# salesforce/LayoutDETR

Hardware: AMD Instinct MI355X
Metric: images/sec G+D fwd-bwd, 256x256 bg x9 elems (higher is better)
Workload: dtype f32

## Files before the change

include/ldetr_hip.h:

```cpp
#ifndef LDETR_HIP_H
#define LDETR_HIP_H

#include <stdint.h>

#ifdef __cplusplus
extern "C" {
#endif

const char* ldetr_last_error(void);
int ldetr_abi_version(void);

int ldetr_debug_trace_tiles(int64_t* buffer);

int ldetr_set_split_bf16(int tiles);

int ldetr_engine_launch_counts(int64_t* f32_pipe, int64_t* bf16_split_pipe);

int ldetr_set_workspace(void* ptr, int64_t bytes);

typedef struct ldetr_tensor4 {
    int N, C, H, W;
    int64_t sn, sc, sh, sw;
} ldetr_tensor4;

typedef struct ldetr_epilogue {
    float alpha;
    const float* col_scale;
    const float* col_bias;
    const float* samp_scale;
    int64_t samp_ld;
    const float* residual;
    int64_t ldr;
    int act;
    float act_alpha;
    float act_gain;
    const float* mask_src;
    int64_t ldm;
    int mask_mode;
    float out_scale;
    float p_drop;
    uint64_t seed;
    const uint64_t* seed_ptr;
    int accumulate;
    float* a_rowsum;
} ldetr_epilogue;

int ldetr_bias_act_f32(const float* x, const float* b, const float* xref, const float* yref, const float* dy, float* y,
                       int64_t sizeX, int sizeB, int64_t stepB, int grad, int act, float alpha, float gain, float clamp,
                       void* stream);

int ldetr_upfirdn2d_f32(const float* x, const float* f, float* y, int N, int C, int inH, int inW,
                        const int64_t* x_strides_nchw, int fh, int fw, int64_t f_stride_h, int64_t f_stride_w,
                        int upx, int upy, int downx, int downy, int padx0, int padx1, int pady0, int pady1, int flip,
                        float gain, int outH, int outW, const int64_t* y_strides_nchw,
                        const float* act_bias, int has_act, float act_alpha, float act_gain, void* stream);

int ldetr_gemm_f32(const float* A, int64_t lda, int ta, const float* B, int64_t ldb, int tb, float* C, int64_t ldc,
                   int M, int N, int K, int splitk, const ldetr_epilogue* ep, int pix_per_sample, void* stream);

typedef struct ldetr_gemm_desc {
    const float* A; int64_t lda; int ta;
    const float* B; int64_t ldb; int tb;
    float* C; int64_t ldc;
    int M, N, K, splitk;
    const ldetr_epilogue* ep;
    int pix_per_sample;
} ldetr_gemm_desc;
int ldetr_gemm_pair_f32(const ldetr_gemm_desc* g0, const ldetr_gemm_desc* g1, void* stream);
int ldetr_gemm_pair_is_single_launch(const ldetr_gemm_desc* g0, const ldetr_gemm_desc* g1);

int ldetr_conv2d_fwd_f32(const float* x, const ldetr_tensor4* xt, const float* w, int Cout, int KH, int KW, int stride,
                         int pad, float* y, int64_t ldy, int OH, int OW, const float* in_scale, int64_t in_scale_ld,
                         const ldetr_epilogue* ep, void* stream);
int ldetr_conv2d_bwd_data_f32(const float* dy, const ldetr_tensor4* dyt, const float* w, int Cin, int KH, int KW,
                              int stride, int pad, float* dx, int64_t lddx, int IH, int IW, const float* dy_scale,
                              int64_t dy_scale_ld, const ldetr_epilogue* ep, void* stream);
int ldetr_conv2d_bwd_weight_f32(const float* x, const ldetr_tensor4* xt, const float* dy, const ldetr_tensor4* dyt,
                                float* dw, int KH, int KW, int stride, int pad, int splitk, const float* x_scale,
                                int64_t x_scale_ld, const float* dy_scale, int64_t dy_scale_ld, int accumulate, void* stream);

int ldetr_conv_transpose2d_fwd_f32(const float* x, const ldetr_tensor4* xt, const float* w, int Cout, int KH, int KW,
                                   int stride, int pad, float* y, int64_t ldy, int OH, int OW, const float* in_scale,
                                   int64_t in_scale_ld, const ldetr_epilogue* ep, void* stream);
int ldetr_conv_transpose2d_bwd_data_f32(const float* dy, const ldetr_tensor4* dyt, const float* w, int Cin, int KH,
                                        int KW, int stride, int pad, float* dx, int64_t lddx, int IH, int IW,
                                        const float* dy_scale, int64_t dy_scale_ld, const ldetr_epilogue* ep,
                                        void* stream);
int ldetr_conv_transpose2d_bwd_weight_f32(const float* x, const ldetr_tensor4* xt, const float* dy,
                                          const ldetr_tensor4* dyt, float* dw, int KH, int KW, int stride, int pad,
                                          int splitk, const float* x_scale, int64_t x_scale_ld, const float* dy_scale,
                                          int64_t dy_scale_ld, int accumulate, void* stream);

int ldetr_attention_fwd_f32(const float* q, int64_t ldq, const float* k, int64_t ldk, const float* v, int64_t ldv,
                            const unsigned char* key_padding_mask, float* out, int64_t ldo, float* lse, int B, int H,
                            int Lq, int Lk, int head_dim, float scale, float p_drop, uint64_t seed, const uint64_t* seed_ptr,
                            int causal, void* stream);
int ldetr_attention_bwd_f32(const float* q, int64_t ldq, const float* k, int64_t ldk, const float* v, int64_t ldv,
                            const unsigned char* key_padding_mask, const float* out, int64_t ldo, const float* lse,
                            const float* dout, int64_t lddo, float* dq, int64_t lddq, float* dk, int64_t lddk,
                            float* dv, int64_t lddv, int B, int H, int Lq, int Lk, int head_dim, float scale,
                            float p_drop, uint64_t seed, const uint64_t* seed_ptr, int causal, void* stream);

int ldetr_torgb_bwd_finish_f32(const float* dws, const float* s, const float* w, int B, int C, float* dw, float* ds, void* stream);

int ldetr_loss_combine_fwd_f32(const float* const* x, const float* w, const int* n, const int* fn, const int* red, int K, int ld,
                               float* vals, float* sums, float* total, void* stream);
int ldetr_loss_combine_bwd_f32(const float* const* x, const float* w, const int* n, const int* fn, const int* red, int K, int ld,
                               const float* g, float* grads, void* stream);
int ldetr_masked_mse_fwd_f32(const float* a, const float* b, const uint8_t* valid, int64_t rows, int D, int bdiv, float* out2, void* stream);
int ldetr_masked_mse_bwd_f32(const float* a, const float* b, const uint8_t* valid, int64_t rows, int D, int bdiv, const float* out2,
                             const float* g, float* da, void* stream);

typedef struct ldetr_ln_args {
    const float* x; const float* r; const float* gamma; const float* beta;
    float* y; float* z; float* mean; float* rstd;
    const float* dy; float* dx; float* dr; float* dgamma; float* dbeta;
    int64_t rows; int D; float eps, p_drop; uint64_t seed; const uint64_t* seed_ptr;
    const float* pos; int64_t pos_rows; float* ypos; const float* dy2;
    int r_parts; int64_t r_part_stride; const float* r_bias;
    const float* dy_parts; int dy_nparts; int64_t dy_part_stride;
} ldetr_ln_args;
int ldetr_layernorm_fwd_group_f32(const ldetr_ln_args* a, int n, void* stream);
int ldetr_layernorm_bwd_group_f32(const ldetr_ln_args* a, int n, void* stream);
int ldetr_sum_parts_f32(const float* base, const float* parts, int n_parts, int64_t part_stride, float* out, int64_t n, void* stream);

typedef struct ldetr_ffn_args {
    const float* x; int64_t ldx;
    const float* w1; const float* b1;
    const float* w2;
    float* h;
    float* ypart;
    int M, F;
    float p_drop; uint64_t seed; const uint64_t* seed_ptr;
    const float* dy;
    float* dxpart;
    float* dh;
} ldetr_ffn_args;
int ldetr_ffn_fwd_group_f32(const ldetr_ffn_args* a, int n, void* stream);
int ldetr_ffn_bwd_group_f32(const ldetr_ffn_args* a, int n, void* stream);

typedef struct ldetr_mha_small_args {
    const float* x; int64_t ldx;
    const float* w_in; const float* b_in; const float* w_out;
    const unsigned char* kpm;
    float* qkv; float* o; float* lse; float* ypart;
    int B, L;
    float scale, p_drop; uint64_t seed; const uint64_t* seed_ptr;
    const float* dr;
    float* dqkv; float* dxpart;
} ldetr_mha_small_args;
int ldetr_mha_small_fwd_group_f32(const ldetr_mha_small_args* a, int n, void* stream);
int ldetr_mha_small_bwd_group_f32(const ldetr_mha_small_args* a, int n, void* stream);

typedef struct ldetr_mha_cross_args {
    const float* x; int64_t ldx;
    const float* w_q; const float* b_q;
    const float* k; int64_t ldk; const float* v; int64_t ldv;
    const float* w_out;
    const unsigned char* kpm;
    float* q; float* o; float* lse; float* ypart;
    int B, Lq, Lk;
    float scale, p_drop; uint64_t seed; const uint64_t* seed_ptr;
    const float* dr;
    float* dq; float* dk; int64_t lddk; float* dv; int64_t lddv; float* dxpart;
} ldetr_mha_cross_args;
int ldetr_mha_cross_fwd_f32(const ldetr_mha_cross_args* a, void* stream);
int ldetr_mha_cross_bwd_f32(const ldetr_mha_cross_args* a, void* stream);

typedef struct ldetr_wgrad_desc {
    const float* A; int64_t lda; const float* B; int64_t ldb;
    float* dW; int64_t ldw; float* db;
    int M, rows, cols;
} ldetr_wgrad_desc;
int ldetr_wgrad_multi_f32(const ldetr_wgrad_desc* d, int n, void* stream);

int ldetr_colsum_f32(const float* a, float* red, int B, int64_t P, int C, void* stream);
int ldetr_act_bwd_reduce_f32(const float* dy, const float* y, float* dv, const float* bias, const float* demod,
                             float* dbias, float* ddemod, int B, int64_t P, int C, int act, float alpha, float gain,
                             void* stream);
int ldetr_mul_reduce_f32(const float* a, const float* x, const float* scale, float* out, float* red, int B, int64_t P,
                         int C, void* stream);
int ldetr_torgb_fwd_f32(const float* x, const float* w, const float* styles, const float* bias, float* y,
                        int B, int64_t P, int C, void* stream);
int ldetr_torgb_bwd_f32(const float* x, const float* dy, const float* w, const float* styles, float* dx, float* dws,
                        float* dbias, int B, int64_t P, int C, void* stream);
int ldetr_sg2_handoff_f32(const float* dxs, const float* x, const float* dy_rgb, float* dv, const float* s_conv, const float* s_rgb,
                          const float* w_rgb, const float* bias, const float* demod, float* ds_conv, float* dws_rgb, float* dbias_rgb,
                          float* dbias, float* ddemod, int B, int64_t P, int C, float alpha, float gain, void* stream);

int ldetr_maxpool3x3s2_fwd_f32(const float* x, float* y, unsigned char* idx, int N, int H, int W, int C, void* stream);
int ldetr_maxpool3x3s2_bwd_f32(const float* dy, const unsigned char* idx, float* dx, int N, int H, int W, int C,
                               void* stream);

int ldetr_grad_sanitize_f32(float* g, int64_t n, float scale, float nan_value, float posinf, float neginf,
                            void* stream);
int ldetr_adam_step_f32(float* p, const float* g, float* m, float* v, int64_t n, int64_t step, float lr, float beta1,
                        float beta2, float eps, int fuse_sanitize, float gscale, float nan_value, float posinf,
                        float neginf, void* stream);
int ldetr_adam_ema_step_f32(float* p, const float* g, float* m, float* v, int64_t n, int64_t step, float lr, float beta1, float beta2,
                            float eps, int fuse_sanitize, float gscale, float nan_value, float posinf, float neginf,
                            float* p_ema, float ema_beta, void* stream);
int ldetr_ema_lerp_f32(float* p_ema, const float* p, int64_t n, float beta, void* stream);

int ldetr_softmax_xent_fwd_f32(const float* logits, int64_t ld, const int64_t* targets, float* row_lse, float* loss_sum, float* count,
                               int64_t rows, int V, int64_t ignore_index, float label_smoothing, void* stream);
int ldetr_softmax_xent_bwd_f32(const float* logits, int64_t ld, const int64_t* targets, const float* row_lse, const float* count,
                               const float* grad_out, float* dlogits, int64_t ldd, int64_t rows, int V, int64_t ignore_index,
                               float label_smoothing, void* stream);

int ldetr_embedding_fwd_f32(const float* weight, const float* pos, const int64_t* ids, float* out, int64_t n, int d, int V, int T,
                            void* stream);
int ldetr_embedding_bwd_f32(const float* dy, const int64_t* ids, float* dweight, int64_t n, int d, int V, int64_t padding_idx,
                            void* stream);

int ldetr_resample_coeffs(int in_size, int out_size, int32_t* bounds, int32_t* weights, int64_t weights_capacity, int* ksize_out);
int ldetr_resize_normalize_u8(const uint8_t* src, int64_t images, int H, int W, int out_h, int out_w, const int32_t* hbounds,
                              const int32_t* hweights, int hksize, const int32_t* vbounds, const int32_t* vweights, int vksize,
                              uint8_t* tmp, uint8_t* out_u8, float* out_chw, float mean0, float mean1, float mean2, float std0,
                              float std1, float std2, void* stream);

#define LDETR_PAGE_FILTER_BLUR 1
#define LDETR_PAGE_FILTER_EDGE 2
int ldetr_page_filter_u8(const uint8_t* src, uint8_t* dst, int64_t images, int H, int W, int kind, float radius, void* stream);

int ldetr_demod_fwd_f32(const float* weight, int64_t so, int64_t si, int64_t sh, int64_t sw, const float* styles, float* dcoefs,
                        float* w2, int B, int O, int I, int KH, int KW, float eps, void* stream);
int ldetr_demod_bwd_f32(const float* weight, int64_t so, int64_t si, int64_t sh, int64_t sw, const float* styles, const float* dcoefs,
                        const float* w2, const float* grad_dcoefs, float* dweight, int accumulate_dweight, float* dstyles, int B, int O,
                        int I, int KH, int KW, void* stream);

int ldetr_layout_losses_f32(const float* bbox, const float* bbox_ref, const uint8_t* valid, int B, int N, float* losses,
                            float* grads, void* stream);
int ldetr_layout_losses_bwd_f32(const float* grads, const float* grad_losses, int B, int N, float* dbbox, void* stream);

int ldetr_layout_finish_f32(const float* bbox_in, const int* num, const float* factors, const unsigned char* jitter, const unsigned char* mode,
                            float* bbox_out, float* overlap, float* alignment, int* order, int C, int K, int N, void* stream);

#define LDETR_FILTER_BILINEAR 0
#define LDETR_FILTER_LANCZOS 1
typedef struct ldetr_layout_raster_args {
    int struct_bytes;
    int B, N, S, nrow, n_colors, n_pages;
    const float* bbox;
    const uint8_t* valid;
    const int32_t* labels;
    const uint8_t* palette;
    const int32_t* page_wh;
    const uint8_t* pages;
    int64_t pages_bytes;
    const int64_t* page_table;
    const int32_t* page_index;
    const int32_t* coeffs;
    int64_t coeffs_len;
    const int64_t* cell_coeffs;
    int32_t* cells_dev;
    uint8_t* out;
} ldetr_layout_raster_args;
int ldetr_resample_coeffs_filter(int filter, int in_size, int out_size, int32_t* bounds, int32_t* weights, int64_t weights_capacity, int* ksize_out);
int ldetr_layout_raster_cell_size(int W, int H, int S, int* wn_out, int* hn_out);
int ldetr_layout_raster_u8(const ldetr_layout_raster_args* a, void* stream);

typedef struct ldetr_patch_resize_args {
    int struct_bytes;
    int n_jobs;
    const uint8_t* src0;
    int64_t src0_bytes;
    const uint8_t* src1;
    int64_t src1_bytes;
    uint8_t* dst;
    int64_t dst_bytes;
    const int64_t* jobs;
    const int32_t* tables;
    const int32_t* tables_host;
    int64_t tables_len;
    int32_t* jobs_dev;
} ldetr_patch_resize_args;
typedef struct ldetr_image_raster_args {
    int struct_bytes;
    int B, N, S, nrow;
    const float* bbox;
    const uint8_t* valid;
    const int32_t* rects;
    const int64_t* patch_off;
    const int64_t* page_off;
    const int32_t* page_wh;
    const uint8_t* pixels;
    int64_t pixels_bytes;
    const int32_t* coeffs;
    int64_t coeffs_len;
    const int64_t* cell_coeffs;
    int32_t* cells_dev;
    uint8_t* out;
} ldetr_image_raster_args;
int ldetr_patch_resize_u8(const ldetr_patch_resize_args* a, void* stream);
int ldetr_image_raster_u8(const ldetr_image_raster_args* a, void* stream);

#define LDETR_PNG_NOT_ELIGIBLE 3
#define LDETR_PNG_MALFORMED 4
typedef struct ldetr_png_decode_args {
    int struct_bytes;
    int n, H, W;
    int phases;
    int reserved;
    const uint8_t* files;
    int64_t files_bytes;
    const int64_t* file_off;
    const int64_t* file_off_dev;
    const int64_t* segments;
    const int64_t* segments_dev;
    int64_t n_segments;
    const int32_t* jobs;
    const int32_t* jobs_dev;
    int64_t n_jobs;
    uint8_t* scratch;
    int64_t scratch_bytes;
    uint8_t* dst;
} ldetr_png_decode_args;
int ldetr_png_scan(const uint8_t* file, int64_t file_bytes, int* width, int* height, int* channels, int64_t* segments, int64_t segments_capacity,
                   int64_t* segments_count, int32_t* row_starts, int64_t row_starts_capacity, int64_t* row_starts_count);
int ldetr_png_decode_u8(const ldetr_png_decode_args* a, void* stream);

typedef struct ldetr_png_encode_args {
    int struct_bytes;
    int H, W;
    int blocks;
    int filter;
    int reserved;
    const uint8_t* src;
    uint8_t* out;
    int64_t out_capacity;
    int64_t* total_bytes;
    uint8_t* workspace;
    int64_t workspace_bytes;
    int64_t* seg_table;
    int64_t seg_table_rows;
} ldetr_png_encode_args;
int ldetr_png_encode_bound(int H, int W, int64_t* out_bytes, int64_t* workspace_bytes);
int ldetr_png_encode_u8(const ldetr_png_encode_args* a, void* stream);
int ldetr_png_index_bytes(int H, int W, int64_t* bytes);

#define LDETR_PNG_INFLATE_CODE 1
#define LDETR_PNG_INFLATE_COUNT 2
#define LDETR_PNG_INFLATE_HEADER 4
#define LDETR_PNG_INFLATE_DISTANCE 8
#define LDETR_PNG_INFLATE_TRAILER 16
#define LDETR_PNG_INFLATE_FILTER 32
#define LDETR_PNG_INFLATE_STUCK 64
#define LDETR_PNG_INFLATE_TABLE 128
typedef struct ldetr_png_inflate_args {
    int struct_bytes;
    int n, H, W;
    int phases;
    int reserved;
    const uint8_t* files;
    int64_t files_bytes;
    const int64_t* file_off;
    const int64_t* file_off_dev;
    const int64_t* segments;
    const int64_t* segments_dev;
    const int64_t* index_off;
    const int64_t* index_off_dev;
    const int32_t* jobs;
    const int32_t* jobs_dev;
    int64_t n_jobs;
    uint8_t* scratch;
    int64_t scratch_bytes;
    uint8_t* dst;
    int32_t* status;
} ldetr_png_inflate_args;
int ldetr_png_scan_packed(const uint8_t* file, int64_t file_bytes, int* width, int* height, int64_t* segments, int64_t segments_capacity, int64_t* segments_count,
                          int64_t* index_offset, int32_t* row_starts, int64_t row_starts_capacity, int64_t* row_starts_count);
int ldetr_png_inflate_u8(const ldetr_png_inflate_args* a, void* stream);

int ldetr_lsap_f64(const double* cost, int batch, int n, int maximize, int* row_ind, int* col_ind, void* stream);

int ldetr_layoutnet_features_f32(const float* bbox, const int64_t* label, const uint8_t* padding_mask, const int* label_map, int map_len,
                                 const float* weights, int64_t weights_len, int num_label, int B, int N, float* out, void* stream);

int ldetr_layoutnet_forward_f32(const float* bbox, const int64_t* label, const uint8_t* padding_mask, const float* enc_weights,
                                int64_t enc_len, const float* dec_weights, int64_t dec_len, int num_label, int B, int N,
                                float* logit_disc, float* logit_cls, float* bbox_pred, float* features, void* stream);

// ... 48 lines not shown
```

layoutdetr_amd/_lib.py:

```python
import ctypes
import os
from ctypes import (POINTER, Structure, c_char_p, c_double, c_float, c_int, c_int64, c_ubyte, c_uint64, c_void_p)

_HERE = os.path.dirname(os.path.abspath(__file__))
ABI_VERSION = 25
LIB_PATH = os.environ.get('LDETR_LIB') or os.path.join(_HERE, 'lib', 'libldetr_hip.so')


class Tensor4(Structure):
    _fields_ = [('N', c_int), ('C', c_int), ('H', c_int), ('W', c_int),
                ('sn', c_int64), ('sc', c_int64), ('sh', c_int64), ('sw', c_int64)]


class GemmDesc(Structure):
    _fields_ = [('A', c_void_p), ('lda', c_int64), ('ta', c_int), ('B', c_void_p), ('ldb', c_int64), ('tb', c_int),
                ('C', c_void_p), ('ldc', c_int64), ('M', c_int), ('N', c_int), ('K', c_int), ('splitk', c_int),
                ('ep', c_void_p), ('pix_per_sample', c_int)]


class P3Epilogue(Structure):
    _fields_ = [('alpha', c_float), ('col_scale', c_void_p), ('col_bias', c_void_p), ('residual_p3', c_void_p),
                ('residual_f32', c_void_p), ('relu_mask_p3', c_void_p), ('relu', c_int)]


class Epilogue(Structure):
    _fields_ = [('alpha', c_float), ('col_scale', c_void_p), ('col_bias', c_void_p), ('samp_scale', c_void_p),
                ('samp_ld', c_int64), ('residual', c_void_p), ('ldr', c_int64), ('act', c_int),
                ('act_alpha', c_float), ('act_gain', c_float), ('mask_src', c_void_p), ('ldm', c_int64),
                ('mask_mode', c_int), ('out_scale', c_float), ('p_drop', c_float), ('seed', c_uint64),
                ('seed_ptr', c_void_p), ('accumulate', c_int), ('a_rowsum', c_void_p)]


class LnArgs(Structure):
    _fields_ = [('x', c_void_p), ('r', c_void_p), ('gamma', c_void_p), ('beta', c_void_p),
                ('y', c_void_p), ('z', c_void_p), ('mean', c_void_p), ('rstd', c_void_p),
                ('dy', c_void_p), ('dx', c_void_p), ('dr', c_void_p), ('dgamma', c_void_p), ('dbeta', c_void_p),
                ('rows', c_int64), ('D', c_int), ('eps', c_float), ('p_drop', c_float), ('seed', c_uint64), ('seed_ptr', c_void_p),
                ('pos', c_void_p), ('pos_rows', c_int64), ('ypos', c_void_p), ('dy2', c_void_p),
                ('r_parts', c_int), ('r_part_stride', c_int64), ('r_bias', c_void_p),
                ('dy_parts', c_void_p), ('dy_nparts', c_int), ('dy_part_stride', c_int64)]


class FfnArgs(Structure):
    _fields_ = [('x', c_void_p), ('ldx', c_int64), ('w1', c_void_p), ('b1', c_void_p), ('w2', c_void_p), ('h', c_void_p), ('ypart', c_void_p),
                ('M', c_int), ('F', c_int), ('p_drop', c_float), ('seed', c_uint64), ('seed_ptr', c_void_p),
                ('dy', c_void_p), ('dxpart', c_void_p), ('dh', c_void_p)]


class MhaSmallArgs(Structure):
    _fields_ = [('x', c_void_p), ('ldx', c_int64), ('w_in', c_void_p), ('b_in', c_void_p), ('w_out', c_void_p), ('kpm', c_void_p),
                ('qkv', c_void_p), ('o', c_void_p), ('lse', c_void_p), ('ypart', c_void_p), ('B', c_int), ('L', c_int),
                ('scale', c_float), ('p_drop', c_float), ('seed', c_uint64), ('seed_ptr', c_void_p),
                ('dr', c_void_p), ('dqkv', c_void_p), ('dxpart', c_void_p)]


class MhaCrossArgs(Structure):
    _fields_ = [('x', c_void_p), ('ldx', c_int64), ('w_q', c_void_p), ('b_q', c_void_p), ('k', c_void_p), ('ldk', c_int64), ('v', c_void_p), ('ldv', c_int64),
                ('w_out', c_void_p), ('kpm', c_void_p), ('q', c_void_p), ('o', c_void_p), ('lse', c_void_p), ('ypart', c_void_p),
                ('B', c_int), ('Lq', c_int), ('Lk', c_int), ('scale', c_float), ('p_drop', c_float), ('seed', c_uint64), ('seed_ptr', c_void_p),
                ('dr', c_void_p), ('dq', c_void_p), ('dk', c_void_p), ('lddk', c_int64), ('dv', c_void_p), ('lddv', c_int64), ('dxpart', c_void_p)]


class WgradDesc(Structure):
    _fields_ = [('A', c_void_p), ('lda', c_int64), ('B', c_void_p), ('ldb', c_int64), ('dW', c_void_p), ('ldw', c_int64), ('db', c_void_p),
                ('M', c_int), ('rows', c_int), ('cols', c_int)]


class LayoutRasterArgs(Structure):
    _fields_ = [('struct_bytes', c_int), ('B', c_int), ('N', c_int), ('S', c_int), ('nrow', c_int), ('n_colors', c_int), ('n_pages', c_int),
                ('bbox', c_void_p), ('valid', c_void_p), ('labels', c_void_p), ('palette', c_void_p), ('page_wh', c_void_p),
                ('pages', c_void_p), ('pages_bytes', c_int64), ('page_table', c_void_p), ('page_index', c_void_p),
                ('coeffs', c_void_p), ('coeffs_len', c_int64), ('cell_coeffs', c_void_p), ('cells_dev', c_void_p), ('out', c_void_p)]


class PatchResizeArgs(Structure):
    _fields_ = [('struct_bytes', c_int), ('n_jobs', c_int), ('src0', c_void_p), ('src0_bytes', c_int64), ('src1', c_void_p), ('src1_bytes', c_int64),
                ('dst', c_void_p), ('dst_bytes', c_int64), ('jobs', c_void_p), ('tables', c_void_p), ('tables_host', c_void_p), ('tables_len', c_int64),
                ('jobs_dev', c_void_p)]


class ImageRasterArgs(Structure):
    _fields_ = [('struct_bytes', c_int), ('B', c_int), ('N', c_int), ('S', c_int), ('nrow', c_int),
                ('bbox', c_void_p), ('valid', c_void_p), ('rects', c_void_p), ('patch_off', c_void_p), ('page_off', c_void_p), ('page_wh', c_void_p),
                ('pixels', c_void_p), ('pixels_bytes', c_int64), ('coeffs', c_void_p), ('coeffs_len', c_int64), ('cell_coeffs', c_void_p),
                ('cells_dev', c_void_p), ('out', c_void_p)]


class PngDecodeArgs(Structure):
    _fields_ = [('struct_bytes', c_int), ('n', c_int), ('H', c_int), ('W', c_int), ('phases', c_int), ('reserved', c_int),
                ('files', c_void_p), ('files_bytes', c_int64), ('file_off', c_void_p), ('file_off_dev', c_void_p),
                ('segments', c_void_p), ('segments_dev', c_void_p), ('n_segments', c_int64),
                ('jobs', c_void_p), ('jobs_dev', c_void_p), ('n_jobs', c_int64),
                ('scratch', c_void_p), ('scratch_bytes', c_int64), ('dst', c_void_p)]


class PngEncodeArgs(Structure):
    _fields_ = [('struct_bytes', c_int), ('H', c_int), ('W', c_int), ('blocks', c_int), ('filter', c_int), ('reserved', c_int),
                ('src', c_void_p), ('out', c_void_p), ('out_capacity', c_int64), ('total_bytes', c_void_p),
                ('workspace', c_void_p), ('workspace_bytes', c_int64), ('seg_table', c_void_p), ('seg_table_rows', c_int64)]


class PngInflateArgs(Structure):
    _fields_ = [('struct_bytes', c_int), ('n', c_int), ('H', c_int), ('W', c_int), ('phases', c_int), ('reserved', c_int),
                ('files', c_void_p), ('files_bytes', c_int64), ('file_off', c_void_p), ('file_off_dev', c_void_p),
                ('segments', c_void_p), ('segments_dev', c_void_p), ('index_off', c_void_p), ('index_off_dev', c_void_p),
                ('jobs', c_void_p), ('jobs_dev', c_void_p), ('n_jobs', c_int64),
                ('scratch', c_void_p), ('scratch_bytes', c_int64), ('dst', c_void_p), ('status', c_void_p)]


_P = c_void_p
_I = c_int
_L = c_int64
_F = c_float
_T4 = POINTER(Tensor4)
_EP = POINTER(Epilogue)

SIGNATURES = {
    'ldetr_set_workspace': [_P, _L],
    'ldetr_bias_act_f32': [_P, _P, _P, _P, _P, _P, _L, _I, _L, _I, _I, _F, _F, _F, _P],
    'ldetr_upfirdn2d_f32': [_P, _P, _P, _I, _I, _I, _I, POINTER(c_int64), _I, _I, _L, _L, _I, _I, _I, _I, _I, _I, _I, _I,
                            _I, _F, _I, _I, POINTER(c_int64), _P, _I, _F, _F, _P],
    'ldetr_gemm_f32': [_P, _L, _I, _P, _L, _I, _P, _L, _I, _I, _I, _I, _EP, _I, _P],
    'ldetr_conv2d_fwd_f32': [_P, _T4, _P, _I, _I, _I, _I, _I, _P, _L, _I, _I, _P, _L, _EP, _P],
    'ldetr_conv2d_bwd_data_f32': [_P, _T4, _P, _I, _I, _I, _I, _I, _P, _L, _I, _I, _P, _L, _EP, _P],
    'ldetr_conv2d_bwd_weight_f32': [_P, _T4, _P, _T4, _P, _I, _I, _I, _I, _I, _P, _L, _P, _L, _I, _P],
    'ldetr_conv_transpose2d_fwd_f32': [_P, _T4, _P, _I, _I, _I, _I, _I, _P, _L, _I, _I, _P, _L, _EP, _P],
    'ldetr_conv_transpose2d_bwd_data_f32': [_P, _T4, _P, _I, _I, _I, _I, _I, _P, _L, _I, _I, _P, _L, _EP, _P],
    'ldetr_conv_transpose2d_bwd_weight_f32': [_P, _T4, _P, _T4, _P, _I, _I, _I, _I, _I, _P, _L, _P, _L, _I, _P],
    'ldetr_attention_fwd_f32': [_P, _L, _P, _L, _P, _L, _P, _P, _L, _P, _I, _I, _I, _I, _I, _F, _F, c_uint64, _P, _I, _P],
    'ldetr_attention_bwd_f32': [_P, _L, _P, _L, _P, _L, _P, _P, _L, _P, _P, _L, _P, _L, _P, _L, _P, _L,
                                _I, _I, _I, _I, _I, _F, _F, c_uint64, _P, _I, _P],
    'ldetr_colsum_f32': [_P, _P, _I, _L, _I, _P],
    'ldetr_act_bwd_reduce_f32': [_P, _P, _P, _P, _P, _P, _P, _I, _L, _I, _I, _F, _F, _P],
    'ldetr_mul_reduce_f32': [_P, _P, _P, _P, _P, _I, _L, _I, _P],
    'ldetr_torgb_fwd_f32': [_P, _P, _P, _P, _P, _I, _L, _I, _P],
    'ldetr_torgb_bwd_f32': [_P, _P, _P, _P, _P, _P, _P, _I, _L, _I, _P],
    'ldetr_maxpool3x3s2_fwd_f32': [_P, _P, _P, _I, _I, _I, _I, _P],
    'ldetr_maxpool3x3s2_bwd_f32': [_P, _P, _P, _I, _I, _I, _I, _P],
    'ldetr_grad_sanitize_f32': [_P, _L, _F, _F, _F, _F, _P],
    'ldetr_adam_step_f32': [_P, _P, _P, _P, _L, _L, _F, _F, _F, _F, _I, _F, _F, _F, _F, _P],
    'ldetr_adam_ema_step_f32': [_P, _P, _P, _P, _L, _L, _F, _F, _F, _F, _I, _F, _F, _F, _F, _P, _F, _P],
    'ldetr_ema_lerp_f32': [_P, _P, _L, _F, _P],
    'ldetr_lsap_f64': [_P, _I, _I, _I, _P, _P, _P],
    'ldetr_layoutnet_features_f32': [_P, _P, _P, POINTER(c_int), _I, _P, _L, _I, _I, _I, _P, _P],
    'ldetr_layoutnet_forward_f32': [_P, _P, _P, _P, _L, _P, _L, _I, _I, _I, _P, _P, _P, _P, _P],
    'ldetr_feature_stats_f64': [_P, _L, _I, _P, _P, _P],
    'ldetr_box_giou_pairwise_f32': [_P, _P, _I, _I, _I, _I, _P, _P, _P, _P, c_double, _P],
    'ldetr_bmm_strided_f32': [_P, _P, _P, _P, _P, _P, _I, _I, _I, _I, _I, _F, _P],
    'ldetr_softmax_xent_fwd_f32': [_P, _L, _P, _P, _P, _P, _L, _I, _L, _F, _P],
    'ldetr_softmax_xent_bwd_f32': [_P, _L, _P, _P, _P, _P, _P, _L, _L, _I, _L, _F, _P],
    'ldetr_embedding_fwd_f32': [_P, _P, _P, _P, _L, _I, _I, _I, _P],
    'ldetr_embedding_bwd_f32': [_P, _P, _P, _L, _I, _I, _L, _P],
    'ldetr_debug_trace_tiles': [_P],
    'ldetr_set_split_bf16': [c_int],
    'ldetr_engine_launch_counts': [POINTER(c_int64), POINTER(c_int64)],
    'ldetr_layernorm_fwd_group_f32': [_P, _I, _P],
    'ldetr_layernorm_bwd_group_f32': [_P, _I, _P],
    'ldetr_sum_parts_f32': [_P, _P, _I, _L, _P, _L, _P],
    'ldetr_ffn_fwd_group_f32': [_P, _I, _P],
    'ldetr_ffn_bwd_group_f32': [_P, _I, _P],
    'ldetr_mha_small_fwd_group_f32': [_P, _I, _P],
    'ldetr_mha_small_bwd_group_f32': [_P, _I, _P],
    'ldetr_mha_cross_fwd_f32': [_P, _P],
    'ldetr_mha_cross_bwd_f32': [_P, _P],
    'ldetr_wgrad_multi_f32': [_P, _I, _P],
    'ldetr_loss_combine_fwd_f32': [_P, _P, _P, _P, _P, _I, _I, _P, _P, _P, _P],
    'ldetr_loss_combine_bwd_f32': [_P, _P, _P, _P, _P, _I, _I, _P, _P, _P],
    'ldetr_masked_mse_fwd_f32': [_P, _P, _P, _L, _I, _I, _P, _P],
    'ldetr_masked_mse_bwd_f32': [_P, _P, _P, _L, _I, _I, _P, _P, _P, _P],
    'ldetr_torgb_bwd_finish_f32': [_P, _P, _P, _I, _I, _P, _P, _P],
    'ldetr_sg2_handoff_f32': [_P, _P, _P, _P, _P, _P, _P, _P, _P, _P, _P, _P, _P, _P, _I, _L, _I, _F, _F, _P],
    'ldetr_gemm_pair_f32': [_P, _P, _P],
    'ldetr_gemm_pair_is_single_launch': [_P, _P],
    'ldetr_demod_fwd_f32': [_P, _L, _L, _L, _L, _P, _P, _P, _I, _I, _I, _I, _I, _F, _P],
    'ldetr_demod_bwd_f32': [_P, _L, _L, _L, _L, _P, _P, _P, _P, _P, _I, _P, _I, _I, _I, _I, _I, _P],
    'ldetr_layout_losses_f32': [_P, _P, _P, _I, _I, _P, _P, _P],
    'ldetr_layout_losses_bwd_f32': [_P, _P, _I, _I, _P, _P],
    'ldetr_layout_finish_f32': [_P, _P, _P, _P, _P, _P, _P, _P, _P, _I, _I, _I, _P],
    'ldetr_resample_coeffs': [_I, _I, _P, _P, _L, _P],
    'ldetr_resample_coeffs_filter': [_I, _I, _I, _P, _P, _L, _P],
    'ldetr_layout_raster_cell_size': [_I, _I, _I, _P, _P],
    'ldetr_layout_raster_u8': [_P, _P],
    'ldetr_patch_resize_u8': [_P, _P],
    'ldetr_image_raster_u8': [_P, _P],
    'ldetr_p3_split_f32': [_P, _L, _P, _L, _I, _P],
    'ldetr_p3_merge_f32': [_P, _P, _L, _L, _I, _P],
    'ldetr_p3_weight_bwd': [_P, _P, _P, _I, _I, _I, _I, _P],
    'ldetr_p3_conv2d_bwd_data': [_P, _I, _I, _I, _I, _P, _I, _I, _I, _I, _I, _I, _I, _P, _P, _P, _P],
    'ldetr_p3_conv2d_fwd': [_P, _I, _I, _I, _I, _P, _I, _I, _I, _I, _I, _P, _P, _P, _P],
    'ldetr_p3_conv2d_bwd_weight': [_P, _I, _I, _I, _I, _P, _I, _I, _I, _I, _I, _P, _P, _P],
    'ldetr_p3_weight_prep': [_P, _I, _I, _P],
    'ldetr_p3_conv2d_fwd_dual': [_P, _P, _I, _I, _I, _I, _P, _P, _I, _I, _I, _I, _I, _P, _P, _P, _P, _P, _P, _P],
    'ldetr_p3_conv2d_bwd_pair': [_P, _I, _I, _I, _I, _P, _P, _I, _I, _I, _I, _I, _I, _I, _P, _P, _P, _P, _P, _P, _P],
    'ldetr_p3_last_launch': [_P],
    'ldetr_engine_last_launch': [_P],
    'ldetr_struct_sizes': [_P],
    'ldetr_resize_normalize_u8': [_P, _L, _I, _I, _I, _I, _P, _P, _I, _P, _P, _I, _P, _P, _P, _F, _F, _F, _F, _F, _F, _P],
    'ldetr_page_filter_u8': [_P, _P, _L, _I, _I, _I, _F, _P],
    'ldetr_png_scan': [_P, _L, _P, _P, _P, _P, _L, _P, _P, _L, _P],
    'ldetr_png_decode_u8': [_P, _P],
    'ldetr_png_encode_bound': [_I, _I, _P, _P],
    'ldetr_png_encode_u8': [_P, _P],
    'ldetr_png_index_bytes': [_I, _I, _P],
    'ldetr_png_scan_packed': [_P, _L, _P, _P, _P, _L, _P, _P, _P, _L, _P],
    'ldetr_png_inflate_u8': [_P, _P],
}

_lib = None


def load():
    global _lib
    if _lib is not None:
        return _lib
    if not os.path.exists(LIB_PATH):
        raise RuntimeError(
            f'{LIB_PATH} not found: build the gfx950 kernels first (python -m layoutdetr_amd.build or '
            f'__graft_entry__.build()).  layoutdetr_amd has no CPU/PyTorch fallback path.')
    import torch
    lib = ctypes.CDLL(LIB_PATH)
    lib.ldetr_last_error.restype = c_char_p
    lib.ldetr_last_error.argtypes = []
    lib.ldetr_abi_version.restype = c_int
    lib.ldetr_abi_version.argtypes = []
    for name, argtypes in SIGNATURES.items():
        fn = getattr(lib, name)
        fn.restype = c_int
        fn.argtypes = argtypes
    if lib.ldetr_abi_version() != ABI_VERSION:
        raise RuntimeError('libldetr_hip.so ABI version mismatch; rebuild it')
    sizes = (ctypes.c_int32 * 6)()
    lib.ldetr_struct_sizes(sizes)
    mirror = [ctypes.sizeof(t) for t in (LnArgs, FfnArgs, MhaSmallArgs, MhaCrossArgs, WgradDesc, P3Epilogue)]
    if list(sizes) != mirror:
        raise RuntimeError(f'libldetr_hip.so argument blocks {list(sizes)} do not match the ctypes mirror {mirror}; rebuild')
    _lib = lib
    return lib


def check(rc, what=''):
    if rc != 0:
        msg = load().ldetr_last_error().decode('utf-8', 'replace')
        raise RuntimeError(f'{what}: {msg}' if what else msg)
```

layoutdetr_amd/build.py:

```python
import hashlib
import os
import shutil
import subprocess
import sys
from concurrent.futures import ThreadPoolExecutor

HERE = os.path.dirname(os.path.abspath(__file__))
CSRC = os.path.join(HERE, 'csrc')
LIBDIR = os.path.join(HERE, 'lib')
OBJDIR = os.path.join(LIBDIR, 'obj')
LIBNAME = 'libldetr_hip.so'
ARCH = 'gfx950'

SOURCES = ['ldetr_core.cpp', 'bias_act.hip', 'upfirdn2d.hip', 'gemm_conv.hip', 'attention.hip', 'layernorm.hip',
           'misc_ops.hip', 'optim.hip', 'lsap.hip', 'xent.hip', 'resample.hip', 'layout_loss.hip', 'demod.hip', 'wgrad_smallc.hip', 'stem_conv.hip', 'box_ops.hip', 'ffn_fused.hip', 'conv_c32.hip', 'mha_small.hip', 'p3_engine.hip', 'bmm_strided.hip', 'layoutnet.hip', 'layoutnet_train.hip', 'layout_finish.hip', 'layout_raster.hip', 'page_filter.hip', 'patch_resize.hip', 'png_decode.hip', 'png_encode.hip', 'png_inflate.hip']
HEADERS = ['ldetr_common.hpp', 'layoutnet_layers.hpp', 'pil_resample.hpp', 'png_pages.hpp', 'png_inflate_kernel.hpp', os.path.join('..', '..', 'include', 'ldetr_hip.h')]

FLAGS = ([] if os.environ.get('LDETR_TILE_TRACE') else ['-DLDETR_TILE_TRACE=0']) + (['-DP3_TRACE'] if os.environ.get('LDETR_P3_TRACE') else []) + ['-O3', '-std=c++17', '-fPIC', f'--offload-arch={ARCH}', '-munsafe-fp-atomics', '-fno-gpu-rdc',
         '-Wno-unused-result', '-Rpass-analysis=kernel-resource-usage']
NO_SCRATCH = ('wgrad_c32_3x3_kernel', 'gemm_f32_kernel', 'gemm_small_kernel', 'attn_fwd_kernel', 'attn_fwd_wide_kernel', 'attn_bwd_kernel', 'ffn_fwd_kernel', 'ffn_bwd_kernel', 'conv3x3_c32_kernel', 'mha_small_fwd_kernel', 'mha_cross_fwd_kernel', 'mha_small_bwd_kernel', 'mha_cross_bwd_kernel', 'wgrad_multi_kernel', 'ln_fwd_kernel', 'ln_bwd_kernel', 'p3_nt_kernel', 'p3_tn_kernel', 'p3_c3_kernel', 'p3_bwd_pair', 'layoutnet_features_kernel', 'layoutnet_forward_kernel', 'feature_stats_f64_kernel', 'layout_finish_kernel', 'layout_raster_kernel', 'page_blur_kernel', 'page_edge_kernel', 'patch_resize_kernel', 'sg2_handoff_kernel', 'png_gather_kernel', 'png_unfilter_kernel', 'png_enc_filter_kernel', 'png_enc_deflate_kernel', 'png_enc_assemble_kernel', 'png_inflate_kernel')


def _hipcc():
    for cand in (os.environ.get('HIPCC'), shutil.which('hipcc'), '/opt/rocm/bin/hipcc'):
        if cand and os.path.exists(cand):
            return cand
    raise RuntimeError('hipcc not found: the gfx950 kernel library cannot be built')


def _digest(paths):
    h = hashlib.sha256()
    for p in paths:
        with open(p, 'rb') as f:
            h.update(f.read())
    h.update(' '.join(FLAGS).encode())
    return h.hexdigest()


def _kernel_resources(remarks):
    out, cur = {}, None
    for line in remarks.splitlines():
        if 'remark:' not in line:
            continue
        body = line.split('remark:', 1)[1].split('[-Rpass-analysis', 1)[0].strip()
        if body.startswith('Function Name:'):
            cur = body.split(':', 1)[1].strip()
            out[cur] = {}
        elif cur is not None and ':' in body:
            k, v = body.rsplit(':', 1)
            out[cur][k.strip()] = v.strip()
    return out


def source_digest():
    return _digest(sorted(os.path.join(CSRC, f) for f in os.listdir(CSRC) if f.endswith(('.hip', '.cpp', '.hpp')) and not f.startswith('.'))
                   + [os.path.normpath(os.path.join(CSRC, HEADERS[-1]))])


def lib_path():
    return os.path.join(LIBDIR, LIBNAME)


def build(force=False, verbose=True):
    os.makedirs(OBJDIR, exist_ok=True)
    hipcc = _hipcc()
    hdrs = [os.path.normpath(os.path.join(CSRC, h)) for h in HEADERS]
    objs, jobs = [], []
    for src in SOURCES:
        sp = os.path.join(CSRC, src)
        obj = os.path.join(OBJDIR, src + '.o')
        stamp = obj + '.sha'
        dig = _digest([sp] + hdrs)
        objs.append(obj)
        if not force and os.path.exists(obj) and os.path.exists(stamp) and open(stamp).read() == dig:
            continue
        jobs.append((sp, obj, stamp, dig))

    def compile_one(job):
        sp, obj, stamp, dig = job
        cmd = [hipcc] + FLAGS + ['-x', 'hip', '-c', sp, '-o', obj]
        if verbose:
            print('[ldetr build]', os.path.basename(sp), flush=True)
        r = subprocess.run(cmd, capture_output=True, text=True)
        if r.returncode != 0:
            raise RuntimeError(f'hipcc failed for {sp}:\n{r.stdout}\n{r.stderr}')
        res = _kernel_resources(r.stderr)
        with open(obj + '.resources.txt', 'w') as f:
            for name, d in res.items():
                f.write(f"{name} vgprs={d.get('VGPRs', '?')} agprs={d.get('AGPRs', '?')} scratch={d.get('ScratchSize [bytes/lane]', '?')} "
                        f"occupancy={d.get('Occupancy [waves/SIMD]', '?')} lds={d.get('LDS Size [bytes/block]', '?')}\n")
        bad = [n for n, d in res.items() if any(k in n for k in NO_SCRATCH) and d.get('ScratchSize [bytes/lane]', '0') != '0']
        if bad:
            raise RuntimeError(f'{os.path.basename(sp)}: scratch memory in register-budgeted kernels: ' + ', '.join(bad[:4]))
        with open(stamp, 'w') as f:
            f.write(dig)

    if jobs:
        with ThreadPoolExecutor(max_workers=min(8, len(jobs))) as ex:
            list(ex.map(compile_one, jobs))
    out = lib_path()
    if jobs or not os.path.exists(out):
        cmd = [hipcc, '-shared', '-fPIC', f'--offload-arch={ARCH}', '-fno-gpu-rdc', '-o', out] + objs
        r = subprocess.run(cmd, capture_output=True, text=True)
        if r.returncode != 0:
            raise RuntimeError(f'link failed:\n{r.stdout}\n{r.stderr}')
        if verbose:
            print('[ldetr build] linked', out, flush=True)
    return out


if __name__ == '__main__':
    build(force='--force' in sys.argv)
```

layoutdetr_amd/csrc/demod.hip:

```cpp
#include "ldetr_common.hpp"
#include "../../include/ldetr_hip.h"

namespace ldetr {

struct DemodParams {
    const float* w; long so, si, sh, sw;
    const float* s;
    float* d;
    float* w2;
    const float* g;
    float* dw; int dw_accumulate;
    float* ds;
    int B, O, I, KH, KW;
    float eps;
};

constexpr int DEMOD_MAXB = 64;

__global__ __launch_bounds__(256) void demod_fwd_kernel(DemodParams p) {
    extern __shared__ float w2row[];
    const int o = blockIdx.x;
    for (int i = threadIdx.x; i < p.I; i += 256) {
        const float* wp = p.w + (long)o * p.so + (long)i * p.si;
        float acc = 0.f;
        for (int kh = 0; kh < p.KH; kh++)
            for (int kw = 0; kw < p.KW; kw++) { const float v = wp[kh * p.sh + kw * p.sw]; acc += v * v; }
        w2row[i] = acc;
        p.w2[(long)o * p.I + i] = acc;
    }
    __syncthreads();
    __shared__ float red16[4][16];
    for (int b0 = 0; b0 < p.B; b0 += 16) {
        float part[16];
#pragma unroll
        for (int u = 0; u < 16; u++) part[u] = 0.f;
        for (int i = threadIdx.x; i < p.I; i += 256) {
            const float wv = w2row[i];
#pragma unroll
            for (int u = 0; u < 16; u++)
                if (b0 + u < p.B) { const float sv = p.s[(long)(b0 + u) * p.I + i]; part[u] += sv * sv * wv; }
        }
#pragma unroll
        for (int u = 0; u < 16; u++) part[u] = wave_sum(part[u]);
        __syncthreads();
        if ((threadIdx.x & 63) == 0) {
#pragma unroll
            for (int u = 0; u < 16; u++) red16[threadIdx.x >> 6][u] = part[u];
        }
        __syncthreads();
        if (threadIdx.x < 16 && b0 + threadIdx.x < p.B) {
            const float tot = red16[0][threadIdx.x] + red16[1][threadIdx.x] + red16[2][threadIdx.x] + red16[3][threadIdx.x];
            p.d[(long)(b0 + threadIdx.x) * p.O + o] = rsqrtf(tot + p.eps);
        }
    }
}

__global__ __launch_bounds__(256) void demod_bwd_w_kernel(DemodParams p) {
    __shared__ float t[DEMOD_MAXB];
    const int o = blockIdx.x;
    if (threadIdx.x < p.B) {
        const float dv = p.d[(long)threadIdx.x * p.O + o];
        t[threadIdx.x] = -0.5f * p.g[(long)threadIdx.x * p.O + o] * dv * dv * dv;
    }
    __syncthreads();
    for (int i = threadIdx.x; i < p.I; i += 256) {
        float dw2 = 0.f;
        for (int b = 0; b < p.B; b++) { const float sv = p.s[(long)b * p.I + i]; dw2 += t[b] * sv * sv; }
        dw2 *= 2.f;
        const long base = (long)o * p.so + (long)i * p.si;
        for (int kh = 0; kh < p.KH; kh++)
            for (int kw = 0; kw < p.KW; kw++) {
                const long off = base + kh * p.sh + kw * p.sw;
                const float v = p.w[off] * dw2;
                if (p.dw_accumulate) p.dw[off] += v; else p.dw[off] = v;
            }
    }
}

__global__ __launch_bounds__(256) void demod_bwd_s_kernel(DemodParams p) {
    extern __shared__ float tb[];
    const int b = blockIdx.y, i = blockIdx.x * 64 + (threadIdx.x & 63), lane = threadIdx.x >> 6;
    for (int o = threadIdx.x; o < p.O; o += 256) {
        const float dv = p.d[(long)b * p.O + o];
        tb[o] = -0.5f * p.g[(long)b * p.O + o] * dv * dv * dv;
    }
    __syncthreads();
    float acc = 0.f;
    if (i < p.I) {
#pragma unroll 8
        for (int o = lane; o < p.O; o += 4) acc += tb[o] * p.w2[(long)o * p.I + i];
    }
    float* part = tb + p.O;
    part[threadIdx.x] = acc;
    __syncthreads();
    if (lane == 0 && i < p.I) {
        acc += part[threadIdx.x + 64] + part[threadIdx.x + 128] + part[threadIdx.x + 192];
        p.ds[(long)b * p.I + i] = 2.f * p.s[(long)b * p.I + i] * acc;
    }
}

}

using namespace ldetr;

static int demod_check(const DemodParams& p, const char* what) {
    LDETR_CHECK(p.w && p.s && p.d && p.w2, "%s: null pointer", what);
    LDETR_CHECK(p.B > 0 && p.B <= DEMOD_MAXB && p.O > 0 && p.I > 0 && p.KH > 0 && p.KW > 0, "%s: bad shape (batch <= %d)", what, DEMOD_MAXB);
    LDETR_CHECK((size_t)(p.I > p.O ? p.I : p.O) * sizeof(float) <= 48 * 1024, "%s: more than 12288 channels", what);
    return LDETR_OK;
}

extern "C" int ldetr_demod_fwd_f32(const float* weight, int64_t so, int64_t si, int64_t sh, int64_t sw, const float* styles, float* dcoefs,
                                   float* w2, int B, int O, int I, int KH, int KW, float eps, void* stream) {
    DemodParams p; memset(&p, 0, sizeof(p));
    p.w = weight; p.so = so; p.si = si; p.sh = sh; p.sw = sw; p.s = styles; p.d = dcoefs; p.w2 = w2;
    p.B = B; p.O = O; p.I = I; p.KH = KH; p.KW = KW; p.eps = eps;
    int rc = demod_check(p, "demod_fwd"); if (rc) return rc;
    hipLaunchKernelGGL(demod_fwd_kernel, dim3(O), 256, (size_t)I * sizeof(float), (hipStream_t)stream, p);
    return check_launch("demod_fwd");
}

extern "C" int ldetr_demod_bwd_f32(const float* weight, int64_t so, int64_t si, int64_t sh, int64_t sw, const float* styles, const float* dcoefs,
                                   const float* w2, const float* grad_dcoefs, float* dweight, int accumulate_dweight, float* dstyles, int B,
                                   int O, int I, int KH, int KW, void* stream) {
    DemodParams p; memset(&p, 0, sizeof(p));
    p.w = weight; p.so = so; p.si = si; p.sh = sh; p.sw = sw; p.s = styles; p.d = const_cast<float*>(dcoefs); p.w2 = const_cast<float*>(w2);
    p.g = grad_dcoefs; p.dw = dweight; p.dw_accumulate = accumulate_dweight; p.ds = dstyles;
    p.B = B; p.O = O; p.I = I; p.KH = KH; p.KW = KW;
    int rc = demod_check(p, "demod_bwd"); if (rc) return rc;
    LDETR_CHECK(grad_dcoefs && (dweight || dstyles), "demod_bwd: null pointer");
    hipStream_t st = (hipStream_t)stream;
    if (dweight) {
        hipLaunchKernelGGL(demod_bwd_w_kernel, dim3(O), 256, 0, st, p);
        rc = check_launch("demod_bwd_w"); if (rc) return rc;
    }
    if (dstyles) {
        hipLaunchKernelGGL(demod_bwd_s_kernel, dim3(cdiv(I, 64), B), 256, (size_t)(O + 256) * sizeof(float), st, p);
        rc = check_launch("demod_bwd_s");
    }
    return rc;
}
```

layoutdetr_amd/csrc/gemm_conv.hip:

```cpp
#include <cstdlib>
#include <type_traits>
#include <atomic>
#include "ldetr_common.hpp"
#include "../../include/ldetr_hip.h"

namespace ldetr {
static thread_local int64_t t_launches_f32 = 0, t_launches_split = 0;
void count_engine_launch(bool bf16_split_pipe) { (bf16_split_pipe ? t_launches_split : t_launches_f32)++; }

enum {
    OP_KC_DENSE = 0,
    OP_KC_CONV = 1,
    OP_KC_CONVT = 2,
    OP_KC_WTAP = 3,
    OP_RC_DENSE = 4,
    OP_RC_PIX = 5,
    OP_RC_WT = 6,
    OP_RC_CONVK = 7,
};

struct Operand {
    const float* p;
    long ld;
    int vec;
// ... 892 lines not shown
        if (!s_last) { trace_out(); return; }
#pragma unroll
        for (int i = 0; i < TM; i++)
#pragma unroll
            for (int j = 0; j < TN; j++)
#pragma unroll
                for (int r = 0; r < 16; r++) acc[i][j][r] = 0.f;
        for (int sl = 0; sl < p.splitk; sl++) {
            const float* src = slot0 + (long)sl * (BM * BN);
#pragma unroll
            for (int i = 0; i < TM; i++)
#pragma unroll
                for (int j = 0; j < TN; j++)
#pragma unroll
                    for (int r = 0; r < 16; r++)
                        acc[i][j][r] += __hip_atomic_load(src + ((i * TN + j) * 16 + r) * NT + tid, __ATOMIC_RELAXED, __HIP_MEMORY_SCOPE_AGENT);
        }
        direct = true;
    }

    const GemmEpilogue& ep = p.ep;
    const float inv_keep = ep.p_drop > 0.f ? 1.f / (1.f - ep.p_drop) : 1.f;
    if (direct && p.ep_vec) {
        constexpr int CP = BN + 4;
        constexpr int LDSF = 2 * BKT * (LDA + LDB);
        constexpr int PASSES = (BM * CP + LDSF - 1) / LDSF, RP = BM / PASSES;
        static_assert(BM % PASSES == 0 && RP * CP <= LDSF && (RP % 32) == 0, "epilogue staging does not fit");
        static_assert(!SPLIT || RP * CP * 4 <= 3 * (BKT / 8) * (PLA + PLB), "epilogue staging does not fit the split path's LDS image");
        float* Cs = ldetr_smem;
#pragma unroll
        for (int ps = 0; ps < PASSES; ps++) {
            if (ps > 0) __syncthreads();
#pragma unroll
            for (int i = 0; i < TM; i++) {
                const int rb = wm * WM + i * 32 - ps * RP;
                if (rb < 0 || rb >= RP) continue;
#pragma unroll
                for (int j = 0; j < TN; j++)
#pragma unroll
                    for (int r = 0; r < 16; r++)
                        Cs[(rb + (r & 3) + 8 * (r >> 2) + 4 * kl) * CP + wn * WN + j * 32 + cl] = acc[i][j][r];
            }
            __syncthreads();
            for (int u = tid; u < RP * (BN / 4); u += NT) {
                const int rl = u / (BN / 4), c4 = (u - rl * (BN / 4)) * 4;
                const int m = m0 + ps * RP + rl, n = n0 + c4;
                if (m >= z.M || n >= p.N) continue;
                long orow = m;
                if (p.zmode == 1 && p.pstep > 1) {
                    int per = z.DH2 * z.DW2;
                    int nn = m / per; int rem = m - nn * per;
                    int y2 = rem / z.DW2; int x2 = rem - y2 * z.DW2;
                    orow = ((long)nn * p.A.DH + (y2 * p.pstep + z.py)) * p.A.DW + (x2 * p.pstep + z.px);
                }
                const int samp = (ep.samp_scale && p.pix_per_sample > 0) ? (int)((unsigned)orow / (unsigned)p.pix_per_sample) : 0;
                const float4 a4 = *reinterpret_cast<const float4*>(Cs + rl * CP + c4);
                float4 cs4 = make_float4(1.f, 1.f, 1.f, 1.f), cb4 = make_float4(0.f, 0.f, 0.f, 0.f), rs4 = make_float4(0.f, 0.f, 0.f, 0.f);
                if (ep.col_scale) cs4 = *reinterpret_cast<const float4*>(ep.col_scale + n);
                if (ep.col_bias) cb4 = *reinterpret_cast<const float4*>(ep.col_bias + n);
                if (ep.residual) rs4 = *reinterpret_cast<const float4*>(ep.residual + orow * ep.ldr + n);
                float4 mk4 = make_float4(0.f, 0.f, 0.f, 0.f);
                if (ep.mask_mode) mk4 = *reinterpret_cast<const float4*>(ep.mask_src + orow * ep.ldm + n);
                float* dst = p.C + z.c_off + orow * p.ldc + n;
                float4 o;
                o.x = apply_epilogue(ep, a4.x, orow, n + 0, samp, p.ldc, inv_keep, cs4.x, cb4.x, rs4.x, mk4.x);
                o.y = apply_epilogue(ep, a4.y, orow, n + 1, samp, p.ldc, inv_keep, cs4.y, cb4.y, rs4.y, mk4.y);
                o.z = apply_epilogue(ep, a4.z, orow, n + 2, samp, p.ldc, inv_keep, cs4.z, cb4.z, rs4.z, mk4.z);
                o.w = apply_epilogue(ep, a4.w, orow, n + 3, samp, p.ldc, inv_keep, cs4.w, cb4.w, rs4.w, mk4.w);
                if (ep.accumulate) { const float4 c = *reinterpret_cast<const float4*>(dst); o.x += c.x; o.y += c.y; o.z += c.z; o.w += c.w; }
                *reinterpret_cast<float4*>(dst) = o;
            }
        }
        trace_out(); return;
    }
    float cs[TN], cb[TN], sfc[TN];
#pragma unroll
    for (int j = 0; j < TN; j++) {
        int n = n0 + wn * WN + j * 32 + cl;
        cs[j] = (ep.col_scale && n < p.N) ? ep.col_scale[n] : 1.f;
        cb[j] = (ep.col_bias && n < p.N) ? ep.col_bias[n] : 0.f;
        sfc[j] = (p.scol && n < p.N) ? p.scol[(long)z.samp * p.scol_ld + n] : 1.f;
    }
#pragma unroll
    for (int i = 0; i < TM; i++) {
#pragma unroll
        for (int r = 0; r < 16; r++) {
            int m = m0 + wm * WM + i * 32 + (r & 3) + 8 * (r >> 2) + 4 * kl;
            if (m >= z.M) continue;
            long orow = m;
            if (p.zmode == 1 && p.pstep > 1) {
                int per = z.DH2 * z.DW2;
                int n = m / per; int rem = m - n * per;
                int y2 = rem / z.DW2; int x2 = rem - y2 * z.DW2;
                orow = ((long)n * p.A.DH + (y2 * p.pstep + z.py)) * p.A.DW + (x2 * p.pstep + z.px);
            }
            int samp = (ep.samp_scale && p.pix_per_sample > 0) ? (int)((unsigned)orow / (unsigned)p.pix_per_sample) : 0;
            const float sfr = p.srow ? p.srow[(long)z.samp * p.srow_ld + m] : 1.f;
#pragma unroll
            for (int j = 0; j < TN; j++) {
                int n = n0 + wn * WN + j * 32 + cl;
                if (n >= p.N) continue;
                float* dst = p.C + z.c_off + orow * p.ldc + n;
                const float a = acc[i][j][r] * sfr * sfc[j];
                if (!direct) {
                    atomicAdd(dst, a * (ep.row_scale ? ep.alpha * ep.row_scale[orow] : ep.alpha));
                } else {
                    float v = apply_epilogue(ep, a, orow, n, samp, p.ldc, inv_keep, cs[j], cb[j], ep.residual ? ep.residual[orow * ep.ldr + n] : 0.f,
                                           ep.mask_mode ? ep.mask_src[orow * ep.ldm + n] : 0.f);
                    if (ep.accumulate) *dst += v; else *dst = v;
                }
            }
        }
    }
    trace_out();
}

template <int T>
__device__ __forceinline__ void small_load(const Operand& o, int row, int R, int k0, int kl, int kend, float (&f)[16]) {
    const int kb = k0 + 16 * kl;
    if (T == 0) {
        const float* src = o.p + (long)row * o.ld + kb;
        if (row < R && o.vec) {
#pragma unroll
            for (int j = 0; j < 4; j++) {
                float4 v = make_float4(0.f, 0.f, 0.f, 0.f);
                if (kb + 4 * j < kend) v = *reinterpret_cast<const float4*>(src + 4 * j);
                f[4 * j] = v.x; f[4 * j + 1] = v.y; f[4 * j + 2] = v.z; f[4 * j + 3] = v.w;
            }
        } else {
#pragma unroll
            for (int t = 0; t < 16; t++) f[t] = (row < R && kb + t < kend) ? src[t] : 0.f;
        }
    } else {
        const float* src = o.p + (long)kb * o.ld + row;
#pragma unroll
        for (int t = 0; t < 16; t++) f[t] = (row < R && kb + t < kend) ? src[(long)t * o.ld] : 0.f;
    }
}

template <int T>
__device__ __forceinline__ void small_load_fast(const __amdgpu_buffer_rsrc_t& rs, int voff, int k0, int ld, float (&f)[16]) {
    if (T == 0) {
#pragma unroll
        for (int j = 0; j < 4; j++) {
            const auto v = __builtin_amdgcn_raw_buffer_load_b128(rs, voff + 16 * j, k0 * 4, 0);
            f[4 * j] = __int_as_float(v[0]); f[4 * j + 1] = __int_as_float(v[1]); f[4 * j + 2] = __int_as_float(v[2]); f[4 * j + 3] = __int_as_float(v[3]);
        }
    } else {
#pragma unroll
        for (int t = 0; t < 16; t++) f[t] = __int_as_float(__builtin_amdgcn_raw_buffer_load_b32(rs, voff, (k0 + t) * ld * 4, 0));
    }
}

template <int TA, int TB, int NW, bool FAST = false>
__device__ __forceinline__ void gemm_small_body(const GemmParams& p, const int bx, const int by, const int bz, const int sk, const int gx) {
    using f32x16 = __attribute__((__vector_size__(16 * sizeof(float)))) float;
    __shared__ float red[NW][32][33];
    const int tid = threadIdx.x, lane = tid & 63, wave = tid >> 6;
    const int cl = lane & 31, kl = lane >> 5;
    const int m0 = by * 32, n0 = bx * 32;
    const int chunks_all = (p.K + 31) / 32;
    const int cper = (chunks_all + sk - 1) / sk;
    const int kblk0 = bz * cper * 32, kblk1 = min(p.K, kblk0 + cper * 32);
    const int chunks = kblk1 > kblk0 ? (kblk1 - kblk0 + 31) / 32 : 0, per = (chunks + NW - 1) / NW;
    const int kbeg = kblk0 + wave * per * 32, kend = min(kblk1, kbeg + per * 32);
    __amdgpu_buffer_rsrc_t rsA = __builtin_amdgcn_make_buffer_rsrc(const_cast<float*>(p.A.p), 0, FAST ? 0x7fffffff : 0, 0x00020000);
    __amdgpu_buffer_rsrc_t rsB = __builtin_amdgcn_make_buffer_rsrc(const_cast<float*>(p.B.p), 0, FAST ? 0x7fffffff : 0, 0x00020000);
    const int voffA = (m0 + cl < p.M) ? (TA == 0 ? ((m0 + cl) * (int)p.A.ld + 16 * kl) * 4 : (16 * kl * (int)p.A.ld + m0 + cl) * 4) : (int)0x80000000;
    const int voffB = (n0 + cl < p.N) ? (TB == 0 ? ((n0 + cl) * (int)p.B.ld + 16 * kl) * 4 : (16 * kl * (int)p.B.ld + n0 + cl) * 4) : (int)0x80000000;
    auto loadA = [&](int k0, float (&f)[16]) {
        if constexpr (FAST) small_load_fast<TA>(rsA, voffA, k0, (int)p.A.ld, f); else small_load<TA>(p.A, m0 + cl, p.M, k0, kl, kend, f);
        if constexpr (TA == 0) {
            if (p.A.scale) {
                const int kb = k0 + 16 * kl;
#pragma unroll
                for (int j = 0; j < 4; j++) {
                    if (kb + 4 * j < kend) {
                        const float4 s4 = *reinterpret_cast<const float4*>(p.A.scale + kb + 4 * j);
                        f[4 * j] *= s4.x; f[4 * j + 1] *= s4.y; f[4 * j + 2] *= s4.z; f[4 * j + 3] *= s4.w;
                    }
                }
            }
        }
    };
    auto loadB = [&](int k0, float (&f)[16]) {
        if constexpr (FAST) small_load_fast<TB>(rsB, voffB, k0, (int)p.B.ld, f); else small_load<TB>(p.B, n0 + cl, p.N, k0, kl, kend, f);
    };
    f32x16 acc;
#pragma unroll
    for (int r = 0; r < 16; r++) acc[r] = 0.f;
    float a0[16], b0[16], a1[16], b1[16];
    const bool want_rs = TA == 1 && p.ep.a_rowsum != nullptr && bx == 0;
    float rs = 0.f;
    if (kbeg < kend) {
        loadA(kbeg, a0);
        loadB(kbeg, b0);
    }
    for (int k = kbeg; k < kend; k += 64) {
        if (k + 32 < kend) {
            loadA(k + 32, a1);
            loadB(k + 32, b1);
        }
#pragma unroll
        for (int t = 0; t < 16; t++) acc = __builtin_amdgcn_mfma_f32_32x32x2f32(a0[t], b0[t], acc, 0, 0, 0);
        if (want_rs) {
#pragma unroll
            for (int t = 0; t < 16; t++) rs += a0[t];
        }
        if (k + 32 >= kend) break;
        if (k + 64 < kend) {
            loadA(k + 64, a0);
            loadB(k + 64, b0);
        }
#pragma unroll
        for (int t = 0; t < 16; t++) acc = __builtin_amdgcn_mfma_f32_32x32x2f32(a1[t], b1[t], acc, 0, 0, 0);
        if (want_rs) {
#pragma unroll
            for (int t = 0; t < 16; t++) rs += a1[t];
        }
    }
    __shared__ float rsum[NW][32];
    if (want_rs) {
        rs += __shfl_xor(rs, 32);
        if (kl == 0) rsum[wave][cl] = rs;
    }
#pragma unroll
    for (int r = 0; r < 16; r++) red[wave][(r & 3) + 8 * (r >> 2) + 4 * kl][cl] = acc[r];
    __syncthreads();
    if (want_rs && tid < 32 && m0 + tid < p.M) {
        float tot = 0.f;
#pragma unroll
        for (int w = 0; w < NW; w++) tot += rsum[w][tid];
        if (sk > 1) atomicAdd(p.ep.a_rowsum + m0 + tid, tot);
        else p.ep.a_rowsum[m0 + tid] += tot;
    }
    const GemmEpilogue& ep = p.ep;
    const float inv_keep = ep.p_drop > 0.f ? 1.f / (1.f - ep.p_drop) : 1.f;
    float* slot0 = nullptr;
    if (sk > 1) {
        const long tile = (long)by * gx + bx;
        slot0 = p.ws + tile * sk * 1024;
        float* mine = slot0 + (long)bz * 1024;
        for (int q = tid; q < 256; q += NW * 64) {
            const int row = q >> 3, c4 = (q & 7) * 4;
#pragma unroll
            for (int e = 0; e < 4; e++) {
                float sum = 0.f;
#pragma unroll
                for (int w = 0; w < NW; w++) sum += red[w][row][c4 + e];
                __hip_atomic_store(mine + q * 4 + e, sum, __ATOMIC_RELAXED, __HIP_MEMORY_SCOPE_AGENT);
            }
        }
        asm volatile("s_waitcnt vmcnt(0)" ::: "memory");
        __shared__ int s_last_small;
        __syncthreads();
        if (tid == 0) {
            const int old = atomicAdd(p.ws_count + tile, 1);
            s_last_small = (old == sk - 1);
            if (s_last_small) __hip_atomic_store(p.ws_count + tile, 0, __ATOMIC_RELAXED, __HIP_MEMORY_SCOPE_AGENT);
        }
        __syncthreads();
        if (!s_last_small) return;
    }
    for (int q = tid; q < 256; q += NW * 64) {
        const int row = q >> 3, c4 = (q & 7) * 4;
        const int m = m0 + row;
        if (m >= p.M) continue;
        float v[4];
        if (sk > 1) {
#pragma unroll
            for (int e = 0; e < 4; e++) v[e] = 0.f;
            float part[8][4];
#pragma unroll
            for (int z = 0; z < 8; z++)
#pragma unroll
                for (int e = 0; e < 4; e++)
                    part[z][e] = z < sk ? __hip_atomic_load(slot0 + (long)z * 1024 + q * 4 + e, __ATOMIC_RELAXED, __HIP_MEMORY_SCOPE_AGENT) : 0.f;
#pragma unroll
            for (int z = 0; z < 8; z++)
#pragma unroll
                for (int e = 0; e < 4; e++) v[e] += part[z][e];
        } else {
#pragma unroll
            for (int e = 0; e < 4; e++) {
                float sum = 0.f;
#pragma unroll
                for (int w = 0; w < NW; w++) sum += red[w][row][c4 + e];
                v[e] = sum;
            }
        }
        const int samp = (ep.samp_scale && p.pix_per_sample > 0) ? m / p.pix_per_sample : 0;
        float* dst = p.C + (long)m * p.ldc + n0 + c4;
#pragma unroll
        for (int e = 0; e < 4; e++)
            if (n0 + c4 + e < p.N) v[e] = apply_epilogue(ep, v[e], m, n0 + c4 + e, samp, p.ldc, inv_keep, ep.col_scale ? ep.col_scale[n0 + c4 + e] : 1.f, ep.col_bias ? ep.col_bias[n0 + c4 + e] : 0.f,
                                                             ep.residual ? ep.residual[(long)m * ep.ldr + n0 + c4 + e] : 0.f,
                                                             ep.mask_mode ? ep.mask_src[(long)m * ep.ldm + n0 + c4 + e] : 0.f);
        if (n0 + c4 + 3 < p.N && (p.ldc & 3) == 0 && ((((uintptr_t)p.C) & 15) == 0)) {
            float4 o = make_float4(v[0], v[1], v[2], v[3]);
            if (ep.accumulate) { float4 c = *reinterpret_cast<float4*>(dst); o.x += c.x; o.y += c.y; o.z += c.z; o.w += c.w; }
            *reinterpret_cast<float4*>(dst) = o;
        } else {
#pragma unroll
            for (int e = 0; e < 4; e++)
                if (n0 + c4 + e < p.N) { if (ep.accumulate) dst[e] += v[e]; else dst[e] = v[e]; }
        }
    }
}

template <int TA, int TB, int NW, bool FAST = false>
__global__ __launch_bounds__(NW * 64) void gemm_small_kernel(GemmParams p) {
    gemm_small_body<TA, TB, NW, FAST>(p, blockIdx.x, blockIdx.y, blockIdx.z, gridDim.z, gridDim.x);
}

template <int TA0, int TB0, int TA1, int TB1, int NW, bool FAST = false>
__global__ __launch_bounds__(NW * 64) void gemm_small_pair_kernel(GemmParams p0, GemmParams p1, int gx0, int nt0, int sk0, int gx1, int nt1, int sk1) {
    const int b = blockIdx.x;
    if (b < nt0 * sk0) { const int t = b % nt0; gemm_small_body<TA0, TB0, NW, FAST>(p0, t % gx0, t / gx0, b / nt0, sk0, gx0); }
    else { const int c = b - nt0 * sk0, t = c % nt1; gemm_small_body<TA1, TB1, NW, FAST>(p1, t % gx1, t / gx1, c / nt1, sk1, gx1); }
}

static inline bool al16(const void* p) { return (((uintptr_t)p) & 15) == 0; }


constexpr long WS_COUNTERS = 262144;
struct Workspace { void* ptr; size_t bytes; size_t counter_cursor; size_t partial_cursor; };
static Workspace g_workspace[64];
static Workspace& workspace_for_current_device() {
    static Workspace none = {nullptr, 0, 0, 0};
    int dev = 0;
    if (hipGetDevice(&dev) != hipSuccess || dev < 0 || dev >= 64) return none;
    return g_workspace[dev];
}

static bool ring_alloc(long tiles, size_t bytes, int** counters, float** partials) {
    Workspace& w = workspace_for_current_device();
    const size_t need = (bytes + 255) & ~(size_t)255;
    const size_t pbytes = w.bytes > WS_COUNTERS * sizeof(int) ? w.bytes - WS_COUNTERS * sizeof(int) : 0;
    if (!w.ptr || need > pbytes || tiles > WS_COUNTERS) return false;
    if (w.counter_cursor + tiles > (size_t)WS_COUNTERS) w.counter_cursor = 0;
    if (w.partial_cursor + need > pbytes) w.partial_cursor = 0;
    *counters = reinterpret_cast<int*>(w.ptr) + w.counter_cursor;
    *partials = reinterpret_cast<float*>(reinterpret_cast<char*>(w.ptr) + WS_COUNTERS * sizeof(int) + w.partial_cursor);
    w.counter_cursor += tiles; w.partial_cursor += need;
    return true;
}

bool splitk_ws_alloc(long tiles, size_t partial_bytes, float** ws, int** counters) { return ring_alloc(tiles, partial_bytes, counters, ws); }

float* scratch_alloc(size_t bytes) {
    int* counters; float* r;
    return ring_alloc(0, bytes, &counters, &r) ? r : nullptr;
}

static int plan_small_split(GemmParams& p, long blocks) {
    int sk = 1;
    if (blocks <= 128 && p.K >= 1024) {
        sk = p.K / 256; if (sk > 8) sk = 8;
        while (sk > 1 && blocks * sk > 640) sk--;
        if (sk > 1 && !ring_alloc(blocks, (size_t)blocks * sk * 1024 * sizeof(float), &p.ws_count, &p.ws)) sk = 1;
    }
    return sk;
}

static bool small_fast_ok(const GemmParams& p, int ta, int tb) {
    static const int on = (int)knob("SMALL_FAST", 1);
    const long a_bytes = (ta ? (long)p.K * p.A.ld : (long)p.M * p.A.ld) * 4, b_bytes = (tb ? (long)p.K * p.B.ld : (long)p.N * p.B.ld) * 4;
    return on && (p.K % 32) == 0 && a_bytes < 0x7fffffffL && b_bytes < 0x7fffffffL && (ta || (p.A.ld % 4) == 0) && (tb || (p.B.ld % 4) == 0) &&
           ((((uintptr_t)p.A.p) | ((uintptr_t)p.B.p)) & 15) == 0;
}

static bool small_wants8(long blocks, int sk, int K) { return blocks * sk <= 256 && (K + sk - 1) / sk >= 512; }

template <int NW, bool FAST, int TA, int TB>
static auto small_kernel() { return gemm_small_kernel<TA, TB, NW, FAST>; }
template <int NW, bool FAST, int TA0, int TB0, int TA1, int TB1>
static auto small_kernel() { return gemm_small_pair_kernel<TA0, TB0, TA1, TB1, NW, FAST>; }

template <int... MODES, typename... Args>
static void launch_small_kernel(bool fast, bool w8, dim3 grid, hipStream_t st, const Args&... args) {
    if (fast) {
        if (w8) hipLaunchKernelGGL((small_kernel<8, true, MODES...>()), grid, 512, 0, st, args...);
        else hipLaunchKernelGGL((small_kernel<4, true, MODES...>()), grid, 256, 0, st, args...);
    } else {
        if (w8) hipLaunchKernelGGL((small_kernel<8, false, MODES...>()), grid, 512, 0, st, args...);
        else hipLaunchKernelGGL((small_kernel<4, false, MODES...>()), grid, 256, 0, st, args...);
    }
    t_launches_f32++;
}

template <int TA, int TB>
static int launch_small(GemmParams& p, hipStream_t st) {
    dim3 grid(cdiv(p.N, 32), cdiv(p.M, 32), 1);
    const long blocks = (long)grid.x * grid.y;
    const int sk = plan_small_split(p, blocks);
    grid.z = sk;
    const bool fast = small_fast_ok(p, TA, TB);
    const bool w8 = small_wants8(blocks, sk, p.K);
    launch_small_kernel<TA, TB>(fast, w8, grid, st, p);
    note_engine_launch(2, 32, 32, 0, w8 ? 8 : 4, fast ? 1 : 0, 0, sk, blocks * sk, TA * 2 + TB);
    return check_launch("gemm_small");
}

template <int TA0>
static int launch_small_pair(GemmParams& p0, GemmParams& p1, hipStream_t st) {
    const int gx0 = cdiv(p0.N, 32), nt0 = gx0 * cdiv(p0.M, 32), gx1 = cdiv(p1.N, 32), nt1 = gx1 * cdiv(p1.M, 32);
    const int sk0 = plan_small_split(p0, nt0), sk1 = plan_small_split(p1, nt1);
    const bool w8 = small_wants8(nt0, sk0, p0.K) && small_wants8(nt1, sk1, p1.K);
    const bool fast = small_fast_ok(p0, TA0, 1) && small_fast_ok(p1, 1, 1);
    const dim3 grid((unsigned)(nt0 * sk0 + nt1 * sk1));
    launch_small_kernel<TA0, 1, 1, 1>(fast, w8, grid, st, p0, p1, gx0, nt0, sk0, gx1, nt1, sk1);
    note_engine_launch(3, 32, 32, 0, w8 ? 8 : 4, fast ? 1 : 0, 0, sk0 * 256 + sk1, (long)grid.x, (TA0 * 2 + 1) * 4 + 3);
    return check_launch("gemm_small_pair");
}

struct EpiParams { GemmEpilogue ep; float* C; long ldc; long rows; int N; int pix_per_sample; };

__global__ __launch_bounds__(256) void gemm_epilogue_kernel(EpiParams q) {
    const float inv_keep = q.ep.p_drop > 0.f ? 1.f / (1.f - q.ep.p_drop) : 1.f;
    const long total = q.rows * q.N;
    for (long i = (long)blockIdx.x * blockDim.x + threadIdx.x; i < total; i += (long)gridDim.x * blockDim.x) {
        long row = i / q.N; int n = (int)(i - row * q.N);
        int samp = (q.ep.samp_scale && q.pix_per_sample > 0) ? (int)(row / q.pix_per_sample) : 0;
        float* dst = q.C + row * q.ldc + n;
        *dst = apply_epilogue(q.ep, *dst, row, n, samp, q.ldc, inv_keep, q.ep.col_scale ? q.ep.col_scale[n] : 1.f, q.ep.col_bias ? q.ep.col_bias[n] : 0.f,
                              q.ep.residual ? q.ep.residual[row * q.ep.ldr + n] : 0.f,
                              q.ep.mask_mode ? q.ep.mask_src[row * q.ep.ldm + n] : 0.f);
    }
}

static bool epilogue_is_linear(const GemmEpilogue& ep) {
    return !ep.col_scale && !ep.samp_scale && !ep.col_bias && !ep.residual && !ep.act && !ep.mask_mode && ep.p_drop == 0.f &&
           ep.out_scale == 1.f;
}


#ifndef T128_BK
#define T128_BK 32
#endif
#ifndef T128_WAVES
#define T128_WAVES 8
#endif
#ifndef LDETR_EPILOGUE_VEC
#define LDETR_EPILOGUE_VEC 1
#endif
#ifndef T12864_SPLIT_MIN_TILES
#define T12864_SPLIT_MIN_TILES 64
#endif
#ifndef T12864_WAVES
#define T12864_WAVES 8
#define T12864_BK 32
#endif

static const long SMALL_GEMM_TILES = 256;
constexpr long SMALL_GEMM_MNK = 1l << 30;
static bool small_class(long M, long N, long K) { return (long)cdiv(M, 64) * cdiv(N, 64) < SMALL_GEMM_TILES && M * N * K <= SMALL_GEMM_MNK; }
#ifndef WGRAD_MIN_K
#define WGRAD_MIN_K 512
#endif

__global__ void __launch_bounds__(256) zero_fill_kernel(float* __restrict__ dst, long pitch, long width, long rows) {
    const long total = rows * width;
    for (long i = (long)blockIdx.x * 256 + threadIdx.x; i < total; i += (long)gridDim.x * 256) {
        const long r = i / width;
        dst[r * pitch + (i - r * width)] = 0.f;
    }
}
static int zero_fill(float* dst, long pitch, long width, long rows, hipStream_t st) {
    if (rows <= 0 || width <= 0) return LDETR_OK;
    if (pitch == width) { width *= rows; pitch = width; rows = 1; }
    long total = rows * width;
    int g = (int)((total + 255) / 256); if (g > 2048) g = 2048;
// ... 215 lines not shown
}

static void set_sample_slices(GemmParams& p, int nsamp, int pix_per_samp, int want, const float* srow, long srow_ld,
                              const float* scol, long scol_ld) {
    int q = (want + nsamp / 2) / nsamp;
    if (q < 1) q = 1;
    while (q > 1 && pix_per_samp / q < 64) q--;
    p.samp_pix = pix_per_samp; p.samp_q = q;
    p.srow = srow; p.srow_ld = srow_ld; p.scol = scol; p.scol_ld = scol_ld;
    p.splitk = nsamp * q;
    if (p.splitk > 1) p.ep.accumulate = 0;
}

static void fill_epilogue(GemmEpilogue& ep, const ldetr_epilogue* e) {
    memset(&ep, 0, sizeof(ep));
    ep.out_scale = 1.f; ep.act_gain = 1.f; ep.alpha = 1.f;
    if (!e) return;
    ep.alpha = e->alpha;
    ep.col_scale = e->col_scale; ep.col_bias = e->col_bias;
    ep.samp_scale = e->samp_scale; ep.samp_ld = e->samp_ld;
    ep.residual = e->residual; ep.ldr = e->ldr;
    ep.act = e->act; ep.act_alpha = e->act_alpha; ep.act_gain = e->act_gain;
    ep.mask_src = e->mask_src; ep.ldm = e->ldm; ep.mask_mode = e->mask_mode;
    ep.out_scale = e->out_scale; ep.p_drop = e->p_drop; ep.seed = e->seed; ep.seed_ptr = (const unsigned long long*)e->seed_ptr; ep.accumulate = e->accumulate;
    ep.a_rowsum = e->a_rowsum;
}

static void init_operand(Operand& o) { memset(&o, 0, sizeof(o)); o.KW = 1; o.KH = 1; o.stride = 1; o.C = 1; o.Cr = 1; }

static GemmParams new_params() {
    GemmParams p; memset(&p, 0, sizeof(p));
    init_operand(p.A); init_operand(p.B);
    return p;
}

static void set_conv_src(Operand& o, const float* x, const ldetr_tensor4* t) {
    o.p = x; o.SH = t->H; o.SW = t->W; o.sn = t->sn; o.sh = t->sh; o.sw = t->sw; o.sc = t->sc;
}

static void set_conv_operand(Operand& o, const float* x, const ldetr_tensor4* t, const float* scale, long scale_ld, int DH, int DW,
                             int stride, int pad, int KH, int KW) {
    set_conv_src(o, x, t);
    o.DH = DH; o.DW = DW; o.stride = stride; o.pad = pad; o.KH = KH; o.KW = KW;
    o.scale = scale; o.scale_ld = scale_ld;
    o.vec = al16(x) && (t->sn % 4 == 0) && (t->sh % 4 == 0) && (t->sw % 4 == 0) && (!scale || (al16(scale) && scale_ld % 4 == 0));
}

static bool packed_nhwc(const ldetr_tensor4* t) { return t->sw == t->C && t->sh == (long)t->W * t->C && t->sn == (long)t->H * t->W * t->C; }

}

using namespace ldetr;

extern "C" int ldetr_debug_trace_tiles(int64_t* buffer) {
    g_trace_buffer = reinterpret_cast<long long*>(buffer);
    return LDETR_OK;
}

extern "C" int ldetr_engine_launch_counts(int64_t* f32_pipe, int64_t* bf16_split_pipe) {
    if (f32_pipe) *f32_pipe = t_launches_f32;
    if (bf16_split_pipe) *bf16_split_pipe = t_launches_split;
    return LDETR_OK;
}

extern "C" int ldetr_set_split_bf16(int tiles) {
    const int prev = g_split_bf16_override.exchange(tiles);
    return prev;
}

extern "C" int ldetr_set_workspace(void* ptr, int64_t bytes) {
    int dev = 0;
    LDETR_CHECK(hipGetDevice(&dev) == hipSuccess && dev >= 0 && dev < 64, "set_workspace: no current device");
    LDETR_CHECK(bytes >= 0, "set_workspace: negative size");
    LDETR_CHECK(!ptr || (((uintptr_t)ptr) & 15) == 0, "set_workspace: pointer must be 16-byte aligned");
    LDETR_CHECK(!ptr || bytes > (int64_t)(WS_COUNTERS * sizeof(int)), "set_workspace: too small");
    g_workspace[dev].ptr = ptr; g_workspace[dev].bytes = ptr ? (size_t)bytes : 0;
    g_workspace[dev].counter_cursor = 0; g_workspace[dev].partial_cursor = 0;
    return LDETR_OK;
}

static GemmParams fill_dense(const ldetr_gemm_desc& g) {
    GemmParams p = new_params();
    p.A.p = g.A; p.A.ld = g.lda; p.B.p = g.B; p.B.ld = g.ldb;
    p.A.vec = al16(g.A) && (g.lda % 4 == 0) && (g.ta ? (g.M % 4 == 0) : (g.K % 4 == 0));
    p.B.vec = al16(g.B) && (g.ldb % 4 == 0) && (g.tb ? (g.N % 4 == 0) : (g.K % 4 == 0));
    p.M = g.M; p.N = g.N; p.K = g.K; p.C = g.C; p.ldc = g.ldc;
    p.zmode = 0; p.splitk = 1; p.pstep = 1; p.nsamp = 1; p.pix_per_sample = g.pix_per_sample;
    fill_epilogue(p.ep, g.ep);
    return p;
}

static int gemm_dense(const ldetr_gemm_desc& g, void* stream) {
    const int M = g.M, N = g.N, K = g.K, ta = g.ta, tb = g.tb;
    LDETR_CHECK(g.A && g.B && g.C, "gemm: null pointer");
    LDETR_CHECK(M >= 0 && N >= 0 && K >= 0, "gemm: negative dimension");
    if (M == 0 || N == 0) return LDETR_OK;
    GemmParams p = fill_dense(g);
    p.splitk = g.splitk < 1 ? 1 : g.splitk;
    LDETR_CHECK(!(p.splitk > 1 && p.ep.accumulate && !epilogue_is_linear(p.ep)), "gemm: split-K + accumulate needs a linear epilogue");
    hipStream_t st = (hipStream_t)stream;
    const bool auto_split = (g.splitk == 0);
    const bool small = auto_split && small_class(M, N, K);
    if (p.ep.a_rowsum) {
        LDETR_CHECK(ta == 1 && g.lda == M, "gemm: a_rowsum needs ta == 1 and a packed A (lda == M)");
        if (!(small && tb)) {
            int rc = ldetr_colsum_f32(g.A, p.ep.a_rowsum, 1, K, M, stream);
            if (rc) return rc;
            p.ep.a_rowsum = nullptr;
        }
    }
    if (small) {
        if (!ta && !tb) return launch_small<0, 0>(p, st);
        if (!ta && tb) return launch_small<0, 1>(p, st);
        if (ta && tb) return launch_small<1, 1>(p, st);
    }
    if (!ta && !tb) return launch_gemm<OP_KC_DENSE, OP_KC_DENSE>(p, M, M, 1, auto_split, false, st);
    if (!ta && tb) return launch_gemm<OP_KC_DENSE, OP_RC_DENSE>(p, M, M, 1, auto_split, false, st);
    if (ta && tb) return launch_gemm<OP_RC_DENSE, OP_RC_DENSE>(p, M, M, 1, auto_split, false, st);
    set_error("gemm: (ta=1, tb=0) is not instantiated");
    return LDETR_ERR_UNSUPPORTED;
}

extern "C" int ldetr_gemm_f32(const float* A, int64_t lda, int ta, const float* B, int64_t ldb, int tb,
                              float* C, int64_t ldc, int M, int N, int K, int splitk,
                              const ldetr_epilogue* ep, int pix_per_sample, void* stream) {
    const ldetr_gemm_desc g = {A, lda, ta, B, ldb, tb, C, ldc, M, N, K, splitk, ep, pix_per_sample};
    return gemm_dense(g, stream);
}

static bool small_class(const ldetr_gemm_desc& g) {
    return g.splitk == 0 && g.M > 0 && g.N > 0 && g.K > 0 && small_class(g.M, g.N, g.K);
}

static bool pair_single_launch(const ldetr_gemm_desc* g0, const ldetr_gemm_desc* g1) {
    static const int pair_on = (int)knob("GEMM_PAIR", 1);
    const bool nn_tn = g0->ta == 0 && g0->tb == 1 && g1->ta == 1 && g1->tb == 1, tn_tn = g0->ta == 1 && g0->tb == 1 && g1->ta == 1 && g1->tb == 1;
    return pair_on && (nn_tn || tn_tn) && g0->A && g0->B && g0->C && g1->A && g1->B && g1->C && small_class(*g0) && small_class(*g1) &&
           (!g1->ep || !g1->ep->a_rowsum || g1->lda == g1->M) && (!(g0->ep && g0->ep->a_rowsum) || (tn_tn && g0->lda == g0->M));
}

extern "C" int ldetr_gemm_pair_is_single_launch(const ldetr_gemm_desc* g0, const ldetr_gemm_desc* g1) {
    return (g0 && g1 && pair_single_launch(g0, g1)) ? 1 : 0;
}

extern "C" int ldetr_gemm_pair_f32(const ldetr_gemm_desc* g0, const ldetr_gemm_desc* g1, void* stream) {
    LDETR_CHECK(g0 && g1, "gemm_pair: null descriptor");
    if (pair_single_launch(g0, g1)) {
        GemmParams p0 = fill_dense(*g0), p1 = fill_dense(*g1);
        return g0->ta == 1 ? launch_small_pair<1>(p0, p1, (hipStream_t)stream) : launch_small_pair<0>(p0, p1, (hipStream_t)stream);
    }
    int rc = gemm_dense(*g0, stream);
    if (rc) return rc;
    return gemm_dense(*g1, stream);
}

extern "C" int ldetr_conv2d_fwd_f32(const float* x, const ldetr_tensor4* xt, const float* w, int Cout, int KH, int KW,
                                    int stride, int pad, float* y, int64_t ldy, int OH, int OW,
                                    const float* in_scale, int64_t in_scale_ld,
                                    const ldetr_epilogue* ep, void* stream) {
    LDETR_CHECK(x && w && y && xt, "conv2d_fwd: null pointer");
    int eOH = (xt->H + 2 * pad - KH) / stride + 1, eOW = (xt->W + 2 * pad - KW) / stride + 1;
    LDETR_CHECK(eOH == OH && eOW == OW, "conv2d_fwd: output size mismatch (expected %dx%d)", eOH, eOW);
    {
        const int took = try_launch_stem_conv(x, xt, w, Cout, KH, KW, stride, pad, y, ldy, OH, OW, in_scale, ep, (hipStream_t)stream);
        if (took >= 0) return took;
    }
    {
        const int took = try_launch_conv_c32(x, xt, w, Cout, KH, KW, stride, pad, y, ldy, OH, OW, in_scale, in_scale_ld, ep, 0, (hipStream_t)stream);
        if (took > 0) t_launches_f32++;
        if (took != 0) return took > 0 ? LDETR_OK : LDETR_ERR_LAUNCH;
    }
    GemmParams p = new_params();
    set_conv_operand(p.A, x, xt, in_scale, in_scale_ld, OH, OW, stride, pad, KH, KW);
    p.A.C = xt->C;
    p.A.vec = p.A.vec && (xt->sc == 1) && (xt->C % 4 == 0);
    long K = (long)KH * KW * xt->C;
    p.B.p = w; p.B.ld = K; p.B.vec = al16(w) && (K % 4 == 0);
    p.M = xt->N * OH * OW; p.N = Cout; p.K = (int)K; p.C = y; p.ldc = ldy;
    p.zmode = 0; p.splitk = 1; p.pstep = 1; p.nsamp = xt->N; p.pix_per_sample = OH * OW;
    fill_epilogue(p.ep, ep);
    hipStream_t st = (hipStream_t)stream;
    if (KH == 1 && KW == 1 && stride == 1 && pad == 0 && p.A.vec && !in_scale && packed_nhwc(xt)) {
        p.A.ld = xt->C;
        if (!p.ep.samp_scale && small_class(p.M, p.N, p.K)) return launch_small<0, 0>(p, st);
        return launch_gemm<OP_KC_DENSE, OP_KC_DENSE>(p, p.M, p.M, 1, true, false, st);
    }
    return launch_gemm<OP_KC_CONV, OP_KC_DENSE>(p, p.M, p.M, 1, true, false, st);
}

extern "C" int ldetr_conv2d_bwd_data_f32(const float* dy, const ldetr_tensor4* dyt, const float* w, int Cin, int KH, int KW,
                                         int stride, int pad, float* dx, int64_t lddx, int IH, int IW,
                                         const float* dy_scale, int64_t dy_scale_ld,
                                         const ldetr_epilogue* ep, void* stream) {
    LDETR_CHECK(dy && w && dx && dyt, "conv2d_bwd_data: null pointer");
    LDETR_CHECK(dyt->sc == 1 && dyt->C % 4 == 0 && Cin % 4 == 0, "conv2d_bwd_data: channels must be NHWC-contiguous multiples of 4");
    {
        const int took = try_launch_conv_c32(dy, dyt, w, Cin, KH, KW, stride, pad, dx, lddx, IH, IW, dy_scale, dy_scale_ld, ep, 1, (hipStream_t)stream);
        if (took > 0) t_launches_f32++;
        if (took != 0) return took > 0 ? LDETR_OK : LDETR_ERR_LAUNCH;
    }
    GemmParams p = new_params();
    set_conv_operand(p.A, dy, dyt, dy_scale, dy_scale_ld, IH, IW, stride, pad, KH, KW);
    p.A.C = dyt->C;
    LDETR_CHECK(p.A.vec, "conv2d_bwd_data: dy must be 16-byte aligned NHWC");
    p.B.p = w; p.B.ld = (long)KH * KW * Cin; p.B.C = dyt->C; p.B.Cr = Cin; p.B.KH = KH; p.B.KW = KW;
    p.B.vec = al16(w);
    p.N = Cin; p.C = dx; p.ldc = lddx;
    p.zmode = 1; p.splitk = 1; p.pstep = stride; p.nsamp = dyt->N; p.pix_per_sample = IH * IW;
    p.M = dyt->N * IH * IW; p.K = KH * KW * dyt->C;
    fill_epilogue(p.ep, ep);
    if (KH == 1 && KW == 1 && stride == 1 && pad == 0 && packed_nhwc(dyt) && (!dy_scale || dy_scale_ld == 0) && dyt->C % 4 == 0 &&
        !p.ep.samp_scale && small_class(p.M, p.N, p.K)) {
        GemmParams g = p;
        g.zmode = 0; g.pstep = 1; g.A.ld = dyt->C; g.B.ld = Cin; g.B.vec = al16(w) && (Cin % 4 == 0);
        return launch_small<0, 1>(g, (hipStream_t)stream);
    }
    int Mmax = dyt->N * cdiv(IH, stride) * cdiv(IW, stride);
    return launch_gemm<OP_KC_CONVT, OP_RC_WT>(p, Mmax, (long)p.M, stride * stride, true, false, (hipStream_t)stream);
}

static int wgrad_begin(GemmParams& p, int splitk, int nsamp, float* dw, long wsz, int accumulate, hipStream_t st) {
    p = new_params();
    fill_epilogue(p.ep, nullptr);
    p.splitk = splitk; p.pstep = 1; p.nsamp = nsamp; p.pix_per_sample = 0;
    if (!accumulate) { if (int zrc = zero_fill(dw, wsz, wsz, 1, st)) return zrc; }
    if (splitk == 1 && accumulate) p.ep.accumulate = 1;
    return LDETR_OK;
}

static void wgrad_factor_sample_scales(GemmParams& p, int nsamp, int pix_per_samp, int accumulate, const float*& dy_scale, long dy_scale_ld,
                                       const float*& x_scale, long x_scale_ld) {
    if (!((dy_scale || x_scale) && (!dy_scale || dy_scale_ld != 0) && (!x_scale || x_scale_ld != 0) && pix_per_samp >= 64)) return;
    set_sample_slices(p, nsamp, pix_per_samp, p.splitk, dy_scale, dy_scale_ld, x_scale, x_scale_ld);
    if (p.splitk == 1 && accumulate) p.ep.accumulate = 1;
    dy_scale = nullptr; x_scale = nullptr;
}

extern "C" int ldetr_conv2d_bwd_weight_f32(const float* x, const ldetr_tensor4* xt, const float* dy, const ldetr_tensor4* dyt,
                                           float* dw, int KH, int KW, int stride, int pad, int splitk,
                                           const float* x_scale, int64_t x_scale_ld,
                                           const float* dy_scale, int64_t dy_scale_ld, int accumulate, void* stream) {
    LDETR_CHECK(x && dy && dw && xt && dyt, "conv2d_bwd_weight: null pointer");
    LDETR_CHECK(dyt->sc == 1, "conv2d_bwd_weight: dy must be NHWC");
    int Cin = xt->C, Cout = dyt->C, OH = dyt->H, OW = dyt->W;
    hipStream_t st = (hipStream_t)stream;
    int Kpix = dyt->N * OH * OW;
    const bool gather = (xt->sc != 1 || Cin % 4 != 0);
    if (splitk < 1)
        splitk = gather ? wgrad_auto_split(Cout, KH * KW * Cin, Kpix, 1) : wgrad_auto_split(Cout, Cin, Kpix, KH * KW);
    GemmParams p;
    if (int rc = wgrad_begin(p, splitk, xt->N, dw, (long)Cout * KH * KW * Cin, accumulate, st)) return rc;
    if (!gather) {
        const int took = try_launch_wgrad_smallc(x, xt, dy, dyt, dw, KH, KW, stride, pad, x_scale, x_scale_ld, dy_scale, dy_scale_ld, st);
        if (took > 0) t_launches_f32++;
        if (took != 0) return took > 0 ? LDETR_OK : LDETR_ERR_LAUNCH;
    }
    p.M = Cout; p.K = Kpix; p.C = dw; p.ldc = (long)KH * KW * Cin;
    if (gather) {
        LDETR_CHECK(packed_nhwc(dyt), "conv2d_bwd_weight: dy must be packed NHWC");
        LDETR_CHECK(!x_scale && !dy_scale, "conv2d_bwd_weight: scales unsupported on the scalar-gather path");
        p.A.p = dy; p.A.ld = Cout; p.A.vec = al16(dy) && (Cout % 4 == 0);
        set_conv_src(p.B, x, xt);
        p.B.DH = OH; p.B.DW = OW; p.B.C = Cin; p.B.stride = stride; p.B.pad = pad; p.B.KH = KH; p.B.KW = KW;
        p.N = KH * KW * Cin; p.zmode = 0;
        return launch_gemm<OP_RC_DENSE, OP_RC_CONVK>(p, p.M, p.M, 1, false, true, st);
    }
    if (dy_scale && dy_scale_ld == 0) { p.ep.row_scale = dy_scale; dy_scale = nullptr; }
    p.N = Cin; p.zmode = 2; p.ntaps = KH * KW; p.c_tap_stride = Cin;
    wgrad_factor_sample_scales(p, dyt->N, OH * OW, accumulate, dy_scale, dy_scale_ld, x_scale, x_scale_ld);
    if (!dy_scale && packed_nhwc(dyt)) {
        p.A.p = dy; p.A.ld = Cout; p.A.vec = al16(dy) && (Cout % 4 == 0);
        if (!x_scale && KH == 1 && KW == 1 && stride == 1 && pad == 0 && packed_nhwc(xt)) {
            p.B.p = x; p.B.ld = Cin; p.B.vec = al16(x);
            if (small_class(p.M, p.N, p.K) && Kpix <= 8192) {
                p.zmode = 0; p.ntaps = 1; p.c_tap_stride = 0; p.splitk = 1; p.ep.accumulate = 1;
                return launch_small<1, 1>(p, st);
            }
            return launch_gemm<OP_RC_DENSE, OP_RC_DENSE>(p, p.M, p.M, 1, false, true, st);
        }
        set_conv_operand(p.B, x, xt, x_scale, x_scale_ld, OH, OW, stride, pad, KH, KW);
        p.B.tapped = 1;
        return launch_gemm<OP_RC_DENSE, OP_RC_PIX>(p, p.M, p.M, p.ntaps, false, true, st);
    }
    set_conv_operand(p.A, dy, dyt, dy_scale, dy_scale_ld, OH, OW, 1, 0, 1, 1);
    p.A.vec = p.A.vec && (Cout % 4 == 0);
    set_conv_operand(p.B, x, xt, x_scale, x_scale_ld, OH, OW, stride, pad, KH, KW);
    p.B.tapped = 1;
    return launch_gemm<OP_RC_PIX, OP_RC_PIX>(p, p.M, p.M, p.ntaps, false, true, st);
}

extern "C" int ldetr_conv_transpose2d_fwd_f32(const float* x, const ldetr_tensor4* xt, const float* w, int Cout, int KH, int KW,
                                              int stride, int pad, float* y, int64_t ldy, int OH, int OW,
                                              const float* in_scale, int64_t in_scale_ld,
                                              const ldetr_epilogue* ep, void* stream) {
    LDETR_CHECK(x && w && y && xt, "conv_transpose2d_fwd: null pointer");
    LDETR_CHECK(xt->sc == 1 && xt->C % 4 == 0, "conv_transpose2d_fwd: x must be NHWC with C % 4 == 0");
    int eOH = (xt->H - 1) * stride - 2 * pad + KH, eOW = (xt->W - 1) * stride - 2 * pad + KW;
    LDETR_CHECK(eOH == OH && eOW == OW, "conv_transpose2d_fwd: output size mismatch (expected %dx%d)", eOH, eOW);
    GemmParams p = new_params();
    set_conv_operand(p.A, x, xt, in_scale, in_scale_ld, OH, OW, stride, pad, KH, KW);
    p.A.C = xt->C;
    LDETR_CHECK(p.A.vec, "conv_transpose2d_fwd: x must be 16-byte aligned NHWC");
    p.B.p = w; p.B.ld = (long)KH * KW * xt->C; p.B.C = xt->C; p.B.KH = KH; p.B.KW = KW; p.B.vec = al16(w);
    LDETR_CHECK(p.B.vec, "conv_transpose2d_fwd: w must be 16-byte aligned");
    p.N = Cout; p.C = y; p.ldc = ldy;
    p.zmode = 1; p.splitk = 1; p.pstep = stride; p.nsamp = xt->N; p.pix_per_sample = OH * OW;
// ... 47 lines not shown
```

layoutdetr_amd/csrc/misc_ops.hip:

```cpp
#include "ldetr_common.hpp"
#include "../../include/ldetr_hip.h"
#include <type_traits>

namespace ldetr {

enum { RR_COLSUM = 0, RR_ACTGRAD = 1, RR_MULRED = 2 };

struct RRParams {
    const float* a; const float* b; float* out;
    const float* colv;
    const float* sampv;
    float* red1; long red1_bs;
    float* red2; long red2_bs;
    float* part;
    long P; int B, C, mode, act, rows_pb;
    float alpha, gain;
};

template <int MODE>
__global__ __launch_bounds__(256) void rowreduce_kernel(RRParams p) {
    __shared__ float4 sh1[256];
    __shared__ float4 sh2[256];
    const int C4 = p.C >> 2;
    const int TQ = C4 < 256 ? C4 : 256;
// ... 381 lines not shown
                    db0 += d0[u]; db1 += d1[u]; db2 += d2[u];
                }
                if (CONV) {
                    const float4& a = av[u];
                    g.x += a.x * sc.x; g.y += a.y * sc.y; g.z += a.z * sc.z; g.w += a.w * sc.w;
                    rs.x += a.x * x.x; rs.y += a.y * x.y; rs.z += a.z * x.z; rs.w += a.w * x.w;
                }
                float4 dv;
                dv.x = x.x > 0.f ? g.x * gp : g.x * gn; dv.y = x.y > 0.f ? g.y * gp : g.y * gn;
                dv.z = x.z > 0.f ? g.z * gp : g.z * gn; dv.w = x.w > 0.f ? g.w * gp : g.w * gn;
                *reinterpret_cast<float4*>(ob + (size_t)(u * RL) * rowb + ((unsigned)r * rowb + cb)) = dv;
                f4_add(rb, dv);
                rd.x += dv.x * (x.x > 0.f ? x.x * ip : x.x * in); rd.y += dv.y * (x.y > 0.f ? x.y * ip : x.y * in);
                rd.z += dv.z * (x.z > 0.f ? x.z * ip : x.z * in); rd.w += dv.w * (x.w > 0.f ? x.w * ip : x.w * in);
            }
        };
        int r = ty;
#pragma nounroll
        for (; r + 3 * RL < nrows; r += 4 * RL) trip(r, std::integral_constant<int, 4>());
#pragma nounroll
        for (; r < nrows; r += RL) trip(r, std::integral_constant<int, 1>());
    }
    const bool lead = active && ty == 0;
    const int c = cq << 2;
    const long nblk = (long)gridDim.x * gridDim.y, blk = (long)blockIdx.y * gridDim.x + blockIdx.x;
    auto emit = [&](const float4& v, int plane, float* red, long bs) {
        if (p.part) { *reinterpret_cast<float4*>(p.part + ((long)plane * nblk + blk) * p.C + c) = v; return; }
        float* d = red + (long)b * bs + c;
        atomicAdd(d, v.x); atomicAdd(d + 1, v.y); atomicAdd(d + 2, v.z); atomicAdd(d + 3, v.w);
    };
    if (RGB) {
        sh[0][threadIdx.x] = a0; sh[1][threadIdx.x] = a1; sh[2][threadIdx.x] = a2;
        __syncthreads();
        if (lead) {
            for (int j = 1; j < RL; j++) { f4_add(a0, sh[0][j * TQ + tx]); f4_add(a1, sh[1][j * TQ + tx]); f4_add(a2, sh[2][j * TQ + tx]); }
            const int pl = CONV ? 1 : 0;
            emit(a0, pl, p.dws, 3L * p.C); emit(a1, pl + 1, p.dws + p.C, 3L * p.C); emit(a2, pl + 2, p.dws + 2 * p.C, 3L * p.C);
        }
        __syncthreads();
    }
    sh[0][threadIdx.x] = rs; sh[1][threadIdx.x] = rb; sh[2][threadIdx.x] = rd;
    __syncthreads();
    if (lead) {
        for (int j = 1; j < RL; j++) { f4_add(rs, sh[0][j * TQ + tx]); f4_add(rb, sh[1][j * TQ + tx]); f4_add(rd, sh[2][j * TQ + tx]); }
        const int pl = (CONV ? 1 : 0) + (RGB ? 3 : 0);
        if (CONV) emit(rs, 0, p.ds_conv, p.C);
        emit(rb, pl, p.dbias, 0);
        if (dd) {
            const float4 dmv = *reinterpret_cast<const float4*>(p.demod + (long)b * p.C + c);
            const float4 cv = p.bias ? *reinterpret_cast<const float4*>(p.bias + c) : make_float4(0.f, 0.f, 0.f, 0.f);
            rd.x = (rd.x - cv.x * rb.x) / dmv.x; rd.y = (rd.y - cv.y * rb.y) / dmv.y;
            rd.z = (rd.z - cv.z * rb.z) / dmv.z; rd.w = (rd.w - cv.w * rb.w) / dmv.w;
            emit(rd, pl + 1, p.ddemod, p.C);
        }
    }
    if (RGB && blockIdx.z == 0) {
        __syncthreads();
        float* f = reinterpret_cast<float*>(&sh[0][0]);
        if (tx == 0 && ty < RL) { f[ty * 3] = db0; f[ty * 3 + 1] = db1; f[ty * 3 + 2] = db2; }
        __syncthreads();
        if (threadIdx.x < 3) {
            float t = 0.f;
            for (int j = 0; j < RL; j++) t += f[j * 3 + threadIdx.x];
            atomicAdd(p.dbias_rgb + threadIdx.x, t);
        }
    }
}

template <bool CONV, bool RGB>
static int launch_handoff(HandoffParams& p, hipStream_t st) {
    const dim3 grid = rr_grid(p.B, p.P, p.C, &p.rows_pb);
    LDETR_CHECK((long)p.rows_pb * p.C < (1L << 30), "sg2_handoff: a row chunk of %d x %d floats exceeds the kernel's 32-bit offsets", p.rows_pb, p.C);
    const long nblk = (long)grid.x * grid.y;
    const int planes = (CONV ? 1 : 0) + (RGB ? 3 : 0) + 1 + (p.ddemod ? 1 : 0);
    p.part = nblk > 32 ? scratch_alloc((size_t)planes * nblk * p.C * sizeof(float)) : nullptr;
    hipLaunchKernelGGL((sg2_handoff_kernel<CONV, RGB>), grid, 256, 0, st, p);
    int rc = check_launch("sg2_handoff"); if (rc || !p.part) return rc;
    RRFinish f; memset(&f, 0, sizeof(f));
    int i = 0;
    if (CONV) { f.red[i] = p.ds_conv; f.bs[i++] = p.C; }
    if (RGB) for (int k = 0; k < 3; k++) { f.red[i] = p.dws + (long)k * p.C; f.bs[i++] = 3L * p.C; }
    f.red[i] = p.dbias; f.bs[i++] = 0;
    if (p.ddemod) { f.red[i] = p.ddemod; f.bs[i++] = p.C; }
    f.part = p.part; f.B = p.B; f.C = p.C;
    return launch_rr_finish(f, planes, (int)grid.x, nblk, st);
}

}

using namespace ldetr;

static int rr_common(RRParams& p, const char* what) {
    LDETR_CHECK(p.a, "%s: null pointer", what);
    LDETR_CHECK(p.C % 4 == 0 && p.C > 0, "%s: C must be a positive multiple of 4", what);
    LDETR_CHECK(p.B > 0 && p.P >= 0, "%s: bad shape", what);
    return LDETR_OK;
}

extern "C" int ldetr_colsum_f32(const float* a, float* red, int B, int64_t P, int C, void* stream) {
    RRParams p; memset(&p, 0, sizeof(p));
    p.a = a; p.red1 = red; p.red1_bs = C; p.B = B; p.P = P; p.C = C; p.mode = RR_COLSUM;
    int rc = rr_common(p, "colsum"); if (rc) return rc;
    if (P == 0) return LDETR_OK;
    return launch_rr(p, (hipStream_t)stream);
}

extern "C" int ldetr_act_bwd_reduce_f32(const float* dy, const float* y, float* dv, const float* bias, const float* demod,
                                        float* dbias, float* ddemod, int B, int64_t P, int C, int act, float alpha, float gain,
                                        void* stream) {
    RRParams p; memset(&p, 0, sizeof(p));
    p.a = dy; p.b = y; p.out = dv; p.colv = bias; p.sampv = demod; p.red1 = dbias; p.red1_bs = 0;
    p.red2 = ddemod; p.red2_bs = C; p.B = B; p.P = P; p.C = C; p.mode = RR_ACTGRAD; p.act = act; p.alpha = alpha; p.gain = gain;
    int rc = rr_common(p, "act_bwd_reduce"); if (rc) return rc;
    LDETR_CHECK(y, "act_bwd_reduce: y is required");
    LDETR_CHECK(!ddemod || demod, "act_bwd_reduce: ddemod needs demod");
    if (P == 0) return LDETR_OK;
    return launch_rr(p, (hipStream_t)stream);
}

extern "C" int ldetr_mul_reduce_f32(const float* a, const float* x, const float* scale, float* out, float* red,
                                    int B, int64_t P, int C, void* stream) {
    RRParams p; memset(&p, 0, sizeof(p));
    p.a = a; p.b = x; p.out = out; p.sampv = scale; p.red1 = red; p.red1_bs = C; p.B = B; p.P = P; p.C = C; p.mode = RR_MULRED;
    int rc = rr_common(p, "mul_reduce"); if (rc) return rc;
    LDETR_CHECK(x, "mul_reduce: x is required");
    if (P == 0) return LDETR_OK;
    return launch_rr(p, (hipStream_t)stream);
}

extern "C" int ldetr_maxpool3x3s2_fwd_f32(const float* x, float* y, unsigned char* idx, int N, int H, int W, int C, void* stream) {
    LDETR_CHECK(x && y, "maxpool_fwd: null pointer");
    LDETR_CHECK(C % 4 == 0, "maxpool_fwd: C must be a multiple of 4");
    PoolParams p; memset(&p, 0, sizeof(p));
    p.x = x; p.y = y; p.idx = idx; p.N = N; p.H = H; p.W = W; p.C = C; p.OH = (H + 2 - 3) / 2 + 1; p.OW = (W + 2 - 3) / 2 + 1;
    long total = (long)N * p.OH * p.OW * (C / 4);
    int grid = (int)((total + 255) / 256); if (grid > 8192) grid = 8192; if (grid < 1) grid = 1;
    hipLaunchKernelGGL(maxpool_fwd_kernel, grid, 256, 0, (hipStream_t)stream, p);
    return check_launch("maxpool_fwd");
}

extern "C" int ldetr_maxpool3x3s2_bwd_f32(const float* dy, const unsigned char* idx, float* dx, int N, int H, int W, int C, void* stream) {
    LDETR_CHECK(dy && idx && dx, "maxpool_bwd: null pointer");
    LDETR_CHECK(C % 4 == 0, "maxpool_bwd: C must be a multiple of 4");
    PoolParams p; memset(&p, 0, sizeof(p));
    p.dy = dy; p.idx = const_cast<unsigned char*>(idx); p.dx = dx; p.N = N; p.H = H; p.W = W; p.C = C;
    p.OH = (H + 2 - 3) / 2 + 1; p.OW = (W + 2 - 3) / 2 + 1;
    long total = (long)N * H * W * (C / 4);
    int grid = (int)((total + 255) / 256); if (grid > 8192) grid = 8192; if (grid < 1) grid = 1;
    hipLaunchKernelGGL(maxpool_bwd_kernel, grid, 256, 0, (hipStream_t)stream, p);
    return check_launch("maxpool_bwd");
}

namespace ldetr {
struct RgbFwdParams { const float* x; const float* w; const float* s; const float* bias; float* y; long P; int B, C; };

template <int LPP>
__global__ __launch_bounds__(256) void torgb_fwd_kernel(RgbFwdParams p) {
    const int lane_in = threadIdx.x % LPP;
    const long pix_per_block = 256 / LPP;
    const int C4 = p.C >> 2;
    const int b = blockIdx.y;
    const float* sb = p.s + (long)b * p.C;
    float4 w0[2], w1[2], w2[2];
#pragma unroll
    for (int t = 0; t < 2; t++) {
        const int cq = lane_in + t * LPP;
        if (cq < C4) {
            const float4 sv = *reinterpret_cast<const float4*>(sb + 4 * cq);
            float4 a = *reinterpret_cast<const float4*>(p.w + 4 * cq), bq = *reinterpret_cast<const float4*>(p.w + p.C + 4 * cq), c = *reinterpret_cast<const float4*>(p.w + 2 * p.C + 4 * cq);
            w0[t] = make_float4(a.x * sv.x, a.y * sv.y, a.z * sv.z, a.w * sv.w);
            w1[t] = make_float4(bq.x * sv.x, bq.y * sv.y, bq.z * sv.z, bq.w * sv.w);
            w2[t] = make_float4(c.x * sv.x, c.y * sv.y, c.z * sv.z, c.w * sv.w);
        } else { w0[t] = w1[t] = w2[t] = make_float4(0.f, 0.f, 0.f, 0.f); }
    }
    const float b0 = p.bias ? p.bias[0] : 0.f, b1 = p.bias ? p.bias[1] : 0.f, b2 = p.bias ? p.bias[2] : 0.f;
    const long stride = (long)gridDim.x * pix_per_block;
    for (long r = (long)blockIdx.x * pix_per_block + threadIdx.x / LPP; r < p.P; r += stride) {
        const float* xr = p.x + ((long)b * p.P + r) * p.C;
        float d0 = 0.f, d1 = 0.f, d2 = 0.f;
#pragma unroll
        for (int t = 0; t < 2; t++) {
            const int cq = lane_in + t * LPP;
            if (cq < C4) {
                const float4 xv = *reinterpret_cast<const float4*>(xr + 4 * cq);
                d0 += xv.x * w0[t].x + xv.y * w0[t].y + xv.z * w0[t].z + xv.w * w0[t].w;
                d1 += xv.x * w1[t].x + xv.y * w1[t].y + xv.z * w1[t].z + xv.w * w1[t].w;
                d2 += xv.x * w2[t].x + xv.y * w2[t].y + xv.z * w2[t].z + xv.w * w2[t].w;
            }
        }
#pragma unroll
        for (int o = LPP / 2; o > 0; o >>= 1) { d0 += __shfl_xor(d0, o, 64); d1 += __shfl_xor(d1, o, 64); d2 += __shfl_xor(d2, o, 64); }
        if (lane_in == 0) {
            float* yr = p.y + ((long)b * p.P + r) * 3;
            yr[0] = d0 + b0; yr[1] = d1 + b1; yr[2] = d2 + b2;
        }
    }
}
}

extern "C" int ldetr_torgb_fwd_f32(const float* x, const float* w, const float* styles, const float* bias, float* y,
                                   int B, int64_t P, int C, void* stream) {
    LDETR_CHECK(x && w && styles && y, "torgb_fwd: null pointer");
    const int C4 = C / 4;
    LDETR_CHECK(C % 4 == 0 && C4 >= 1 && C <= 512 && (C4 & (C4 - 1)) == 0, "torgb_fwd: C must be 4 x a power of two, at most 512 (got %d)", C);
    LDETR_CHECK((((uintptr_t)x | (uintptr_t)w | (uintptr_t)styles) & 15) == 0, "torgb_fwd: buffers must be 16-byte aligned");
    if (B == 0 || P == 0) return LDETR_OK;
    RgbFwdParams p; p.x = x; p.w = w; p.s = styles; p.bias = bias; p.y = y; p.P = P; p.B = B; p.C = C;
    const int lpp = C4 < 64 ? C4 : 64;
    const long ppb = 256 / lpp;
    long gx = (P + ppb - 1) / ppb; if (gx > 4096) gx = 4096;
    const dim3 grid((unsigned)gx, (unsigned)B);
    hipStream_t st = (hipStream_t)stream;
    switch (lpp) {
        case 1: hipLaunchKernelGGL(torgb_fwd_kernel<1>, grid, 256, 0, st, p); break;
        case 2: hipLaunchKernelGGL(torgb_fwd_kernel<2>, grid, 256, 0, st, p); break;
        case 4: hipLaunchKernelGGL(torgb_fwd_kernel<4>, grid, 256, 0, st, p); break;
        case 8: hipLaunchKernelGGL(torgb_fwd_kernel<8>, grid, 256, 0, st, p); break;
        case 16: hipLaunchKernelGGL(torgb_fwd_kernel<16>, grid, 256, 0, st, p); break;
        case 32: hipLaunchKernelGGL(torgb_fwd_kernel<32>, grid, 256, 0, st, p); break;
        default: hipLaunchKernelGGL(torgb_fwd_kernel<64>, grid, 256, 0, st, p); break;
    }
    return check_launch("torgb_fwd");
}

extern "C" int ldetr_torgb_bwd_f32(const float* x, const float* dy, const float* w, const float* styles,
                                   float* dx, float* dws, float* dbias, int B, int64_t P, int C, void* stream) {
    LDETR_CHECK(x && dy && w && styles && dx && dws, "torgb_bwd: null pointer");
    LDETR_CHECK(C % 4 == 0, "torgb_bwd: C must be a multiple of 4");
    RgbParams p; memset(&p, 0, sizeof(p));
    p.x = x; p.dy = dy; p.w = w; p.s = styles; p.dx = dx; p.dws = dws; p.dbias = dbias; p.B = B; p.P = P; p.C = C;
    const int C4 = C / 4; const int TQ = C4 < 256 ? C4 : 256; const int RL = 256 / TQ;
    long rows_pb = (long)RL * 16;
    long nb = ((P + rows_pb - 1) / rows_pb) * B * cdiv(C4, TQ);
    while (nb > 2048) { rows_pb *= 2; nb = ((P + rows_pb - 1) / rows_pb) * B * cdiv(C4, TQ); }
    p.rows_pb = (int)rows_pb;
    dim3 grid((unsigned)((P + rows_pb - 1) / rows_pb), B, cdiv(C4, TQ));
    hipLaunchKernelGGL(torgb_bwd_kernel, grid, 256, 0, (hipStream_t)stream, p);
    return check_launch("torgb_bwd");
}

extern "C" int ldetr_sg2_handoff_f32(const float* dxs, const float* x, const float* dy_rgb, float* dv, const float* s_conv, const float* s_rgb,
                                     const float* w_rgb, const float* bias, const float* demod, float* ds_conv, float* dws_rgb,
                                     float* dbias_rgb, float* dbias, float* ddemod, int B, int64_t P, int C, float alpha, float gain,
                                     void* stream) {
    LDETR_CHECK(x && dv && dbias, "sg2_handoff: x, dv and dbias are required");
    LDETR_CHECK(dxs || dy_rgb, "sg2_handoff: neither a conv gradient nor an rgb gradient");
    LDETR_CHECK(!dxs || (s_conv && ds_conv), "sg2_handoff: dxs needs s_conv and ds_conv");
    LDETR_CHECK(!dy_rgb || (s_rgb && w_rgb && dws_rgb && dbias_rgb), "sg2_handoff: dy_rgb needs s_rgb, w_rgb, dws_rgb and dbias_rgb");
    LDETR_CHECK(!ddemod || demod, "sg2_handoff: ddemod needs demod");
    LDETR_CHECK(C % 4 == 0 && C > 0 && B > 0 && P >= 0, "sg2_handoff: C must be a positive multiple of 4, B > 0 (got B %d, C %d)", B, C);
    LDETR_CHECK((((uintptr_t)dxs | (uintptr_t)x | (uintptr_t)dv | (uintptr_t)s_conv | (uintptr_t)s_rgb | (uintptr_t)w_rgb | (uintptr_t)bias |
                  (uintptr_t)demod) & 15) == 0, "sg2_handoff: buffers must be 16-byte aligned");
    if (P == 0) return LDETR_OK;
    HandoffParams p; memset(&p, 0, sizeof(p));
    p.dxs = dxs; p.x = x; p.dy = dy_rgb; p.dv = dv; p.s_conv = s_conv; p.s_rgb = s_rgb; p.w_rgb = w_rgb; p.bias = bias; p.demod = demod;
    p.ds_conv = ds_conv; p.dws = dws_rgb; p.dbias_rgb = dbias_rgb; p.dbias = dbias; p.ddemod = ddemod;
    p.B = B; p.P = P; p.C = C; p.gp = gain; p.gn = gain * alpha;
    hipStream_t st = (hipStream_t)stream;
    if (dxs && dy_rgb) return launch_handoff<true, true>(p, st);
    if (dxs) return launch_handoff<true, false>(p, st);
    return launch_handoff<false, true>(p, st);
}

extern "C" int ldetr_torgb_bwd_finish_f32(const float* dws, const float* s, const float* w, int B, int C, float* dw, float* ds, void* stream) {
    LDETR_CHECK(dws && s && w && dw && ds && B > 0 && C > 0, "torgb_bwd_finish: bad arguments");
    const int n = (B > 3 ? B : 3) * C;
    hipLaunchKernelGGL(torgb_finish_kernel, dim3((unsigned)((n + 255) / 256)), 256, 0, (hipStream_t)stream, dws, s, w, dw, ds, B, C);
    return check_launch("torgb_bwd_finish");
}
```

layoutdetr_amd/hip/core.py:

```python
import ctypes
import os

import torch

from .. import _lib
from .._lib import Epilogue, Tensor4

ACT_NONE, ACT_RELU, ACT_LRELU = 0, 1, 2

_seed_counter = [0x5EED]

WEIGHT_GRADIENTS_DISABLED = [False]


class _EngineProfile(object):

    def __init__(self):
        self.enabled = False
        self.records = []

    def reset(self):
        self.records = []

    def summary(self):
        fl = sum(r[1] for r in self.records)
        ms = sum(r[2].elapsed_time(r[3]) for r in self.records)
        return fl, ms * 1e-3, len(self.records)


PROF = _EngineProfile()


_LEGACY_ENV = ('LDETR_PAIR_D', 'LDETR_DUAL_TRUNK', 'LDETR_FUSED_LAYOUT_LOSSES', 'LDETR_FFN_FUSED', 'LDETR_FFN_FUSED_LARGE', 'LDETR_GROUP_KV', 'LDETR_NO_WORKSPACE',
               'LDETR_TOKEN_STACKS', 'LDETR_SPLIT_BF16', 'LDETR_GEMM_PAIR', 'LDETR_P3_PAIR')
_legacy_warned = [False]


def _warn_legacy_env():
    if _legacy_warned[0]:
        return
    _legacy_warned[0] = True
    old = [k for k in _LEGACY_ENV if k in os.environ]
    if old:
        import warnings
        warnings.warn(f'{", ".join(old)}: these switch variables are IGNORED; the switches that remain are keys of LDETR_DEBUG="KEY=value,..."; see DESIGN.md, '
                      '"Diagnostic switches"')


def knob(key, default):
    _warn_legacy_env()
    for kv in os.environ.get('LDETR_DEBUG', '').split(','):
        k, _, v = kv.partition('=')
        if k.strip() == key and v.strip():
            try:
                return int(v)
            except ValueError:
                return int(float(v))
    return default


def engine_call(tag, flops, thunk, operands=(), nbytes=None):
    if not PROF.enabled:
        return thunk()
    s = torch.cuda.Event(enable_timing=True)
    e = torch.cuda.Event(enable_timing=True)
    c0 = engine_launch_counts()
    s.record()
    r = thunk()
    e.record()
    c1 = engine_launch_counts()
    if nbytes is None:
        nbytes = 4.0 * sum(t.numel() for t in operands if t is not None)
    PROF.records.append((tag, float(flops), s, e, nbytes, (c1[0] - c0[0], c1[1] - c0[1]), launched_kernel(tag)))
    return r


_P3_KINDS = {1: 'p3_nt_kernel', 2: 'p3_c3_kernel', 3: 'p3_tn_kernel', 4: 'p3_bwd_pair_nt_kernel', 5: 'p3_bwd_pair_c3_kernel'}
_ENGINE_KINDS = {1: 'gemm_f32_kernel', 2: 'gemm_small_kernel', 3: 'gemm_small_pair_kernel', 4: 'conv3x3_c32_kernel', 5: 'wgrad_c32_3x3_kernel', 6: 'stem_conv7x7_kernel'}


def launched_kernel(tag):
    info = (ctypes.c_int32 * 10)()
    if tag.startswith('ldetr_p3'):
        check(lib().ldetr_p3_last_launch(info), 'p3_last_launch')
        kind, bm, bn, nw, sk = info[0], info[1], info[2], info[3], info[4]
        name = _P3_KINDS.get(kind, 'p3_?')
        if kind in (2, 5):
            return name
        return f'{name}<{bm},{bn},{nw}w>' + (f' splitK={sk}' if sk > 1 else '')
    if tag == 'ldetr_token_stack':
        return 'token-stack kernels (mha_small / mha_cross / ffn / wgrad_multi)'
    check(lib().ldetr_engine_last_launch(info), 'engine_last_launch')
    kind, bm, bn, bk, nw, fast, split, sk = [info[i] for i in range(8)]
    name = _ENGINE_KINDS.get(kind, 'engine_?')
    if kind == 1:
        return f'{name}<{bm},{bn},{bk},{nw}w' + (',FAST' if fast else '') + (',SPLIT' if split else '') + '>' + (f' splitK={sk}' if sk > 1 else '')
    if kind in (2, 3):
        return f'{name}<{nw}w' + (',FAST' if fast else '') + '>'
    if kind == 4:
        return 'conv3x3_c32_split_kernel' if split else name
    return name


def engine_launch_counts():
    a, b = ctypes.c_int64(0), ctypes.c_int64(0)
    lib().ldetr_engine_launch_counts(ctypes.byref(a), ctypes.byref(b))
    return a.value, b.value



_workspace = {}
WORKSPACE_BYTES = int(os.environ.get('LDETR_WORKSPACE_MIB', '256')) << 20


def disable_splitk_workspace():
    l = _lib.load()
    dev = torch.cuda.current_device()
    _workspace[dev] = None
    check(l.ldetr_set_workspace(None, 0), 'set_workspace')


def enable_splitk_workspace():
    _workspace.pop(torch.cuda.current_device(), None)
    lib()


def lib():
    l = _lib.load()
    if torch.cuda.is_available():
        dev = torch.cuda.current_device()
        if dev not in _workspace:
            ws = torch.zeros(WORKSPACE_BYTES // 4, dtype=torch.float32, device=torch.device('cuda', dev))
            _workspace[dev] = ws
            check_rc = l.ldetr_set_workspace(ctypes.c_void_p(ws.data_ptr()), ws.numel() * 4)
            if check_rc != 0:
                raise RuntimeError('ldetr_set_workspace failed: ' + l.ldetr_last_error().decode())
    return l


def check(rc, what=''):
    _lib.check(rc, what)


def require_gpu(*tensors):
    for t in tensors:
        if t is not None and t.device.type != 'cuda':
            raise RuntimeError('layoutdetr_amd ops require tensors in GPU memory (no CPU fallback); got device '
                               f'{t.device}')


def stream():
    return ctypes.c_void_p(torch.cuda.current_stream().cuda_stream)


def ptr(t):
    if t is None:
        return None
    return ctypes.c_void_p(t.data_ptr())


def f32c(t):
    if t is None:
        return None
    if t.dtype != torch.float32:
        t = t.float()
    return t.contiguous()


def next_seed():
    _seed_counter[0] += 1
    base = int(torch.initial_seed()) & 0xFFFFFFFF
    return ((base << 32) ^ (_seed_counter[0] * 0x9E3779B1)) & 0xFFFFFFFFFFFFFFFF


_iter_seed = {}


def iter_seed(device=None):
    device = torch.device('cuda', torch.cuda.current_device()) if device is None else torch.device(device)
    key = (device.type, device.index)
    if key not in _iter_seed:
        _iter_seed[key] = torch.zeros(1, dtype=torch.int64, device=device)
    return _iter_seed[key]


def reseed(device=None):
    iter_seed(device).random_()


def seed_ptr():
    return ctypes.c_void_p(iter_seed().data_ptr())


def tensor4_nhwc(x):
    N, H, W, C = x.shape
    sn, sh, sw, sc = x.stride()
    return Tensor4(N, C, H, W, sn, sc, sh, sw)


def tensor4_nchw(x):
    N, C, H, W = x.shape
    sn, sc, sh, sw = x.stride()
    return Tensor4(N, C, H, W, sn, sc, sh, sw)


def epilogue(alpha=1.0, col_scale=None, col_bias=None, samp_scale=None, residual=None, act=ACT_NONE, act_alpha=0.0,
             act_gain=1.0, mask_src=None, mask_mode=0, out_scale=1.0, p_drop=0.0, seed=0, accumulate=False, a_rowsum=None):
    ep = Epilogue()
    ep.alpha = alpha
    ep.col_scale = col_scale.data_ptr() if col_scale is not None else None
    ep.col_bias = col_bias.data_ptr() if col_bias is not None else None
    if samp_scale is not None:
        ep.samp_scale = samp_scale.data_ptr()
        ep.samp_ld = samp_scale.stride(0)
    if residual is not None:
        ep.residual = residual.data_ptr()
        ep.ldr = residual.shape[-1]
    ep.act = act
    ep.act_alpha = act_alpha
    ep.act_gain = act_gain
    if mask_src is not None:
        ep.mask_src = mask_src.data_ptr()
        ep.ldm = mask_src.shape[-1]
    ep.mask_mode = mask_mode
    ep.out_scale = out_scale
    ep.p_drop = p_drop
    ep.seed = seed
    ep.seed_ptr = iter_seed().data_ptr() if p_drop > 0 else None
    ep.accumulate = 1 if accumulate else 0
    ep.a_rowsum = a_rowsum.data_ptr() if a_rowsum is not None else None
    return ep


def gemm(A, B, ta, tb, M, N, K, out=None, ep=None, splitk=0, pix_per_sample=0, lda=None, ldb=None):
    require_gpu(A, B)
    if out is None:
        out = torch.empty((M, N), device=A.device, dtype=torch.float32)
    lda = A.stride(0) if lda is None else lda
    ldb = B.stride(0) if ldb is None else ldb
    engine_call('gemm', 2.0 * M * N * K, lambda: check(lib().ldetr_gemm_f32(
        ptr(A), lda, int(ta), ptr(B), ldb, int(tb), ptr(out), out.stride(0), M, N, K, splitk,
        ctypes.byref(ep) if ep is not None else None, pix_per_sample, stream()), 'gemm'), nbytes=4.0 * (M * K + N * K + M * N))
    return out


def _pair_descs(g0, g1):
    descs = []
    flops = 0.0
    for g in (g0, g1):
        require_gpu(g['A'], g['B'], g['out'])
        d = _lib.GemmDesc()
        d.A = g['A'].data_ptr(); d.lda = g['A'].stride(0); d.ta = int(g['ta'])
        d.B = g['B'].data_ptr(); d.ldb = g['B'].stride(0); d.tb = int(g['tb'])
        d.C = g['out'].data_ptr(); d.ldc = g['out'].stride(0)
        d.M, d.N, d.K, d.splitk = int(g['M']), int(g['N']), int(g['K']), 0
        d.ep = ctypes.addressof(g['ep']) if g.get('ep') is not None else None
        d.pix_per_sample = 0
        descs.append(d)
        flops += 2.0 * d.M * d.N * d.K
    return descs, flops


def gemm_pair_is_single_launch(g0, g1):
    descs, _ = _pair_descs(g0, g1)
    return lib().ldetr_gemm_pair_is_single_launch(ctypes.byref(descs[0]), ctypes.byref(descs[1])) == 1


def gemm_pair(g0, g1):
    descs, flops = _pair_descs(g0, g1)
    engine_call('gemm', flops, lambda: check(lib().ldetr_gemm_pair_f32(ctypes.byref(descs[0]), ctypes.byref(descs[1]), stream()), 'gemm_pair'),
                nbytes=4.0 * sum(d.M * d.K + d.N * d.K + d.M * d.N for d in descs))


def colsum(a2d, B=1):
    require_gpu(a2d)
    R, C = a2d.shape
    if C % 4 != 0:
        return a2d.reshape(B, R // B, C).sum(1)
    red = torch.zeros((B, C), device=a2d.device, dtype=torch.float32)
    check(lib().ldetr_colsum_f32(ptr(a2d), ptr(red), B, R // B, C, stream()), 'colsum')
    return red


def flat_grad(p):
    if isinstance(p, torch.nn.Parameter) and getattr(p, '_ldetr_flat', False) and p.grad is not None and not torch.is_grad_enabled():
        return p.grad
    return None


class _ZeroArena(object):

    def __init__(self):
        self.buf = {}
        self.cursor = 0
        self.high = {}
        self.open = None

    def begin(self, device):
        dev = device.index if device.index is not None else torch.cuda.current_device()
        self.open = None
        if dev not in self.buf:
            if torch.cuda.is_current_stream_capturing():
                return
            cap = 1 << 22
            self.buf[dev] = (torch.zeros(cap, device=torch.device('cuda', dev), dtype=torch.float32), cap)
            self.high[dev] = 0
        buf, cap = self.buf[dev]
        n = min(cap, max(self.high[dev] * 2, 1 << 16))
        buf[:n].zero_()
        self.limit, self.cursor, self.open = n, 0, dev

    def take(self, shape, device):
        dev = device.index if device.index is not None else torch.cuda.current_device()
        if self.open != dev:
            return None
        n = 1
        for d in shape:
            n *= int(d)
        pad = (n + 3) // 4 * 4
        if self.cursor + pad > self.limit:
            self.high[dev] = max(self.high[dev], self.cursor + pad)
            return None
        out = self.buf[dev][0][self.cursor:self.cursor + n].view(shape)
        self.cursor += pad
        self.high[dev] = max(self.high[dev], self.cursor)
        return out

    def end(self):
        if self.open is not None and self.cursor and knob('ARENA_GUARD', 0) and not torch.cuda.is_current_stream_capturing():
            self.buf[self.open][0][:self.cursor].fill_(float('nan'))
        self.open = None


ZERO_ARENA = _ZeroArena()
_ZERO_ARENA_ON = True


def zero_arena_begin(device):
    if _ZERO_ARENA_ON:
        ZERO_ARENA.begin(torch.device(device))


def zero_arena_end():
    ZERO_ARENA.end()


def zeros(shape, device):
    device = torch.device(device)
    t = ZERO_ARENA.take(tuple(shape), device) if device.type == 'cuda' else None
    return t if t is not None else torch.zeros(shape, device=device, dtype=torch.float32)


def pick_splitk(tiles, K, target=512, min_k=256):
    s = 1
    while tiles * s < target and K // (s * 2) >= min_k and s < 256:
        s *= 2
    return s
```

layoutdetr_amd/hip/sg2_chain.py:

```python
import torch

from . import core, modconv
from .conv import weight_ohwi
from ..torch_utils.ops import upfirdn2d as _up

ENABLED = core.knob('SG2_CHAIN', 1) != 0
ACT_ALPHA = 0.2
NODE_RUNS = [0]


class Block(object):

    def __init__(self, has_conv0, gains, params):
        self.has_conv0 = has_conv0
        self.gains = gains
        self.params = params


def _handoff(dxs, x, dy_rgb, s_conv, rgb, bias, demod, dbias, gain):
    B, H, W, C = x.shape
    dev = x.device
    dv = dxs if dxs is not None else torch.empty_like(x)
    ds_conv = core.zeros((B, C), dev) if dxs is not None else None
    dws = core.zeros((B, 3, C), dev) if dy_rgb is not None else None
    ddemod = core.zeros((B, C), dev)
    s_rgb, w_rgb, dbias_rgb = rgb if dy_rgb is not None else (None, None, None)
    core.check(core.lib().ldetr_sg2_handoff_f32(core.ptr(dxs), core.ptr(x), core.ptr(dy_rgb), core.ptr(dv), core.ptr(s_conv), core.ptr(s_rgb), core.ptr(w_rgb),
                                                core.ptr(bias), core.ptr(demod), core.ptr(ds_conv), core.ptr(dws), core.ptr(dbias_rgb), core.ptr(dbias),
                                                core.ptr(ddemod), B, H * W, C, ACT_ALPHA, gain, core.stream()), 'sg2_handoff')
    return dv, ds_conv, dws, ddemod


def _bias_target(bparam, C, device):
    gb = core.flat_grad(bparam)
    if gb is not None:
        return gb, True
    return torch.zeros(C, device=device, dtype=torch.float32), False


class _SynthesisFn(torch.autograd.Function):

    @staticmethod
    def forward(ctx, blocks, const, f, *tensors):
        core.require_gpu(const, f, *tensors)
        keep = any(ctx.needs_input_grad)
        it = iter(tensors)
        saved, layout = [const, f], []
        x = img = None
        B = tensors[2].shape[0]
        for blk in blocks:
            entry = {}
            if blk.has_conv0:
                w, b, s, d = [next(it) for _ in range(4)]
                w = core.f32c(weight_ohwi(w)); b = core.f32c(b); s = core.f32c(s); d = core.f32c(d)
                _, x0 = modconv.up_fwd(x, w, s, d, b, f, ACT_ALPHA, blk.gains[0])
                entry['conv0'] = (w, b, s, d, x0)
                x = x0
            else:
                x = core.f32c(const).permute(1, 2, 0).unsqueeze(0).repeat([B, 1, 1, 1])
                entry['xin'] = (x,)
            w, b, s, d = [next(it) for _ in range(4)]
            w = core.f32c(weight_ohwi(w)); b = core.f32c(b); s = core.f32c(s); d = core.f32c(d)
            x = modconv.conv_fwd(x, w, s, d, b, w.shape[1] // 2, ACT_ALPHA, blk.gains[1])
            entry['conv1'] = (w, b, s, d, x)
            if img is not None:
                img = _up._kernel_call(img.permute(0, 3, 1, 2), f, 2, 2, 1, 1, 2, 1, 2, 1, False, 4.0).permute(0, 2, 3, 1)
            w, b, s = [next(it) for _ in range(3)]
            ctx_wshape = w.shape
            w = core.f32c(w.reshape(w.shape[0], -1)); b = core.f32c(b); s = core.f32c(s)
            if w.shape[0] != 3:
                raise NotImplementedError('the synthesis node is specialised for 3 colour channels')
            y = modconv.torgb_fwd(x, w, s, b)
            img = img + y if img is not None else y
            entry['torgb'] = (w, s)
            entry['rgb_wshape'] = ctx_wshape
            if keep:
                rec = {}
                for k in ('conv0', 'xin', 'conv1', 'torgb'):
                    if k in entry:
                        rec[k] = (len(saved), len(entry[k]))
                        saved += list(entry[k])
                rec['rgb_wshape'] = ctx_wshape
                layout.append(rec)
        if keep:
            ctx.save_for_backward(*saved)
            ctx.blocks, ctx.layout = blocks, layout
        return img

    @staticmethod
    def backward(ctx, dimg):
        saved = ctx.saved_tensors
        const, f = saved[0], saved[1]
        blocks, layout = ctx.blocks, ctx.layout
        need = ctx.needs_input_grad[3:]
        get = lambda rec, k: saved[rec[k][0]:rec[k][0] + rec[k][1]]
        dimg = core.f32c(dimg)
        dev = dimg.device
        grads = [None] * len(need)
        first, n = [], 0
        for blk in blocks:
            first.append(n)
            n += 11 if blk.has_conv0 else 7
        dxs_next = s_next = dconst = None
        for i in reversed(range(len(blocks))):
            blk, rec = blocks[i], layout[i]
            o = first[i] + (4 if blk.has_conv0 else 0)
            w1, b1, s1, d1, x1 = get(rec, 'conv1')
            wr, sr = get(rec, 'torgb')
            B, H, W, C = x1.shape
            (w1p, b1p), (wrp, brp) = blk.params['conv1'], blk.params['torgb']
            dw_rgb, dbias_rgb, wr_flat, br_flat = modconv.torgb_grad_targets(wrp, brp, 3, C, dev)
            db1, b1_flat = _bias_target(b1p, C, dev)
            dv1, ds_next, dws, dd1 = _handoff(dxs_next, x1, dimg, s_next, (sr, wr, dbias_rgb), b1, d1, db1, blk.gains[1])
            ds_rgb = torch.empty((B, C), device=dev, dtype=torch.float32)
            core.check(core.lib().ldetr_torgb_bwd_finish_f32(core.ptr(dws), core.ptr(sr), core.ptr(wr), B, C, core.ptr(dw_rgb), core.ptr(ds_rgb), core.stream()),
                       'torgb_bwd_finish')
            if i + 1 < len(blocks):
                grads[first[i + 1] + 2] = ds_next
            grads[o + 4] = None if wr_flat else dw_rgb.reshape(rec['rgb_wshape'])
            grads[o + 5] = None if br_flat else dbias_rgb
            grads[o + 6] = ds_rgb
            grads[o + 1] = None if b1_flat else db1
            grads[o + 3] = dd1
            xin = get(rec, 'conv0')[4] if blk.has_conv0 else get(rec, 'xin')[0]
            pad = w1.shape[1] // 2
            dxs1 = modconv.conv_bwd_data(dv1, w1, d1, B, xin.shape[1], xin.shape[2], pad)
            if need[o]:
                grads[o] = modconv.conv_bwd_weight(xin, dv1, w1, s1, d1, w1p, pad)
            if not blk.has_conv0:
                dx, ds1 = modconv._mul_reduce(dxs1, xin, s1, B, xin.shape[1] * xin.shape[2], xin.shape[3])
                grads[o + 2] = ds1
                if ctx.needs_input_grad[1]:
                    dconst = dx.sum(0).permute(2, 0, 1)
                break
            w0, b0, s0, d0, x0 = get(rec, 'conv0')
            w0p, b0p = blk.params['conv0']
            db0, b0_flat = _bias_target(b0p, C, dev)
            dv0, ds1, _, dd0 = _handoff(dxs1, x0, None, s1, None, b0, d0, db0, blk.gains[0])
            grads[o + 2] = ds1
            grads[first[i] + 1] = None if b0_flat else db0
            grads[first[i] + 3] = dd0
            dud = modconv.up_fir_adjoint(dv0, f)
            xprev = get(layout[i - 1], 'conv1')[4]
            dxs_next = modconv.up_bwd_data(dud, w0, d0, B, xprev.shape[1], xprev.shape[2])
            s_next = s0
            if need[first[i]]:
                grads[first[i]] = modconv.up_bwd_weight(xprev, dud, w0, s0, d0, w0p)
            dimg = _up._kernel_call(dimg.permute(0, 3, 1, 2), f, 1, 1, 2, 2, 1, 1, 1, 1, True, 4.0).permute(0, 2, 3, 1)
        return (None, dconst, None) + tuple(grads)


def run(blocks, const, f, tensors):
    NODE_RUNS[0] += 1
    return _SynthesisFn.apply(blocks, const, f, *tensors)
```

layoutdetr_amd/training/networks_stylegan2.py:

```python
import math

import numpy as np
import torch

from ..hip import core, modconv, sg2_chain
from ..hip.linear import linear
from ..torch_utils.ops import bias_act, upfirdn2d


def normalize_2nd_moment(x, dim=1, eps=1e-8):
    return x * (x.square().mean(dim=dim, keepdim=True) + eps).rsqrt()


class FullyConnectedLayer(torch.nn.Module):
    def __init__(self, in_features, out_features, bias=True, activation='linear', lr_multiplier=1, bias_init=0):
        super().__init__()
        self.in_features = in_features
        self.out_features = out_features
        self.activation = activation
        self.weight = torch.nn.Parameter(torch.randn([out_features, in_features]) / lr_multiplier)
        self.bias = torch.nn.Parameter(torch.full([out_features], np.float32(bias_init))) if bias else None
        self.weight_gain = lr_multiplier / np.sqrt(in_features)
        self.bias_gain = lr_multiplier

    def forward(self, x):
        b = self.bias
        spec = bias_act.activation_funcs[self.activation]
        if self.activation == 'lrelu' and b is not None and self.bias_gain != 1 and self.bias_gain > 0:
            return linear(x, self.weight, b, act=core.ACT_LRELU, act_alpha=float(spec.def_alpha), act_gain=float(spec.def_gain * self.bias_gain),
                          wscale=float(self.weight_gain / self.bias_gain))
        if b is not None and self.bias_gain != 1:
            b = b * self.bias_gain
        if self.activation == 'linear':
            return linear(x, self.weight, b, wscale=float(self.weight_gain))
        if self.activation in ('relu', 'lrelu'):
            act = core.ACT_RELU if self.activation == 'relu' else core.ACT_LRELU
            return linear(x, self.weight, b, act=act, act_alpha=float(spec.def_alpha), act_gain=float(spec.def_gain),
                          wscale=float(self.weight_gain))
        y = linear(x, self.weight, None, wscale=float(self.weight_gain))
        return bias_act.bias_act(y, b, act=self.activation)



class SynthesisLayer(torch.nn.Module):
    def __init__(self, in_channels, out_channels, w_dim, resolution, kernel_size=3, up=1, use_noise=True, activation='lrelu',
                 resample_filter=[1, 3, 3, 1], conv_clamp=None, channels_last=False):
        super().__init__()
        if use_noise or conv_clamp is not None or activation != 'lrelu' or kernel_size != 3 or up not in (1, 2):
            raise NotImplementedError('SynthesisLayer: only use_noise=False, conv_clamp=None, lrelu, 3x3, up in {1,2}')
        self.in_channels = in_channels
        self.out_channels = out_channels
        self.w_dim = w_dim
        self.resolution = resolution
        self.up = up
        self.use_noise = use_noise
        self.activation = activation
        self.conv_clamp = conv_clamp
        self.register_buffer('resample_filter', upfirdn2d.setup_filter(resample_filter))
        self.padding = kernel_size // 2
        self.act_gain = bias_act.activation_funcs[activation].def_gain
        self.affine = FullyConnectedLayer(w_dim, in_channels, bias_init=1)
        self.weight = torch.nn.Parameter(torch.randn([out_channels, in_channels, kernel_size, kernel_size]).to(memory_format=torch.channels_last))
        self.bias = torch.nn.Parameter(torch.zeros([out_channels]))

    def forward(self, x, w, noise_mode='none', fused_modconv=False, gain=1):
        if fused_modconv:
            raise NotImplementedError('fused_modconv=True is not used by LayoutDETR (networks_detr.py:261)')
        styles = self.affine(w)
        g = float(self.act_gain * gain)
        if self.up == 1:
            return modconv.modconv3x3(x, self.weight, styles, self.bias, 0.2, g)
        return modconv.modconv3x3_up2(x, self.weight, styles, self.bias, self.resample_filter, 0.2, g)

    def extra_repr(self):
        return (f'in_channels={self.in_channels:d}, out_channels={self.out_channels:d}, w_dim={self.w_dim:d}, '
                f'resolution={self.resolution:d}, up={self.up}, activation={self.activation:s}')


class ToRGBLayer(torch.nn.Module):
    def __init__(self, in_channels, out_channels, w_dim, kernel_size=1, conv_clamp=None, channels_last=False):
        super().__init__()
        if kernel_size != 1 or conv_clamp is not None:
            raise NotImplementedError('ToRGBLayer: only 1x1 without clamping')
        self.in_channels = in_channels
        self.out_channels = out_channels
        self.w_dim = w_dim
        self.conv_clamp = conv_clamp
        self.affine = FullyConnectedLayer(w_dim, in_channels, bias_init=1)
        self.weight = torch.nn.Parameter(torch.randn([out_channels, in_channels, kernel_size, kernel_size]))
        self.bias = torch.nn.Parameter(torch.zeros([out_channels]))
        self.weight_gain = 1 / np.sqrt(in_channels * (kernel_size ** 2))

    def forward(self, x, w, fused_modconv=False):
        styles = self.affine(w) * float(self.weight_gain)
        return modconv.torgb(x, self.weight, styles, self.bias)



class SynthesisBlock(torch.nn.Module):
    def __init__(self, in_channels, out_channels, w_dim, resolution, img_channels, is_last, architecture='skip',
                 resample_filter=[1, 3, 3, 1], conv_clamp=256, use_fp16=False, fp16_channels_last=False,
                 fused_modconv_default=True, **layer_kwargs):
        super().__init__()
        if architecture != 'skip' or use_fp16:
            raise NotImplementedError("SynthesisBlock: only architecture='skip' in fp32")
        self.in_channels = in_channels
        self.w_dim = w_dim
        self.resolution = resolution
        self.img_channels = img_channels
        self.is_last = is_last
        self.architecture = architecture
        self.use_fp16 = use_fp16
        self.channels_last = False
        self.fused_modconv_default = fused_modconv_default
        self.register_buffer('resample_filter', upfirdn2d.setup_filter(resample_filter))
        self.num_conv = 0
        self.num_torgb = 0
        if in_channels == 0:
            self.const = torch.nn.Parameter(torch.randn([out_channels, resolution, resolution]))
        if in_channels != 0:
            self.conv0 = SynthesisLayer(in_channels, out_channels, w_dim=w_dim, resolution=resolution, up=2,
                                        resample_filter=resample_filter, conv_clamp=conv_clamp, **layer_kwargs)
            self.num_conv += 1
        self.conv1 = SynthesisLayer(out_channels, out_channels, w_dim=w_dim, resolution=resolution, conv_clamp=conv_clamp, **layer_kwargs)
        self.num_conv += 1
        self.torgb = ToRGBLayer(out_channels, img_channels, w_dim=w_dim, conv_clamp=conv_clamp)
        self.num_torgb += 1

    def forward(self, x, img, ws, force_fp32=False, fused_modconv=None, update_emas=False, **layer_kwargs):
        w_iter = iter(ws.unbind(dim=1))
        if fused_modconv is None:
            fused_modconv = self.fused_modconv_default
        if fused_modconv == 'inference_only':
            fused_modconv = not self.training
        if self.in_channels == 0:
            x = self.const.permute(1, 2, 0).unsqueeze(0).repeat([ws.shape[0], 1, 1, 1])
            x = self.conv1(x, next(w_iter), fused_modconv=fused_modconv, **layer_kwargs)
        else:
            x = self.conv0(x, next(w_iter), fused_modconv=fused_modconv, **layer_kwargs)
            x = self.conv1(x, next(w_iter), fused_modconv=fused_modconv, **layer_kwargs)
        if img is not None:
            img = upfirdn2d.upsample2d(img.permute(0, 3, 1, 2), self.resample_filter).permute(0, 2, 3, 1)
        y = self.torgb(x, next(w_iter), fused_modconv=fused_modconv)
        img = img + y if img is not None else y
        return x, img



class SynthesisNetwork(torch.nn.Module):
    def __init__(self, w_dim, img_resolution, img_channels, channel_base=32768, channel_max=512, num_fp16_res=4, **block_kwargs):
        assert img_resolution >= 4 and img_resolution & (img_resolution - 1) == 0
        super().__init__()
        if num_fp16_res != 0:
            raise NotImplementedError('fp16 blocks are not used by LayoutDETR (num_fp16_res=0)')
        self.w_dim = w_dim
        self.img_resolution = img_resolution
        self.img_resolution_log2 = int(np.log2(img_resolution))
        self.img_channels = img_channels
        self.num_fp16_res = num_fp16_res
        self.block_resolutions = [2 ** i for i in range(2, self.img_resolution_log2 + 1)]
        channels_dict = {res: min(channel_base // res, channel_max) for res in self.block_resolutions}
        self.num_ws = 0
        for res in self.block_resolutions:
            in_channels = channels_dict[res // 2] if res > 4 else 0
            out_channels = channels_dict[res]
            is_last = (res == self.img_resolution)
            block = SynthesisBlock(in_channels, out_channels, w_dim=w_dim, resolution=res, img_channels=img_channels,
                                   is_last=is_last, use_fp16=False, **block_kwargs)
            self.num_ws += block.num_conv
            if is_last:
                self.num_ws += block.num_torgb
            setattr(self, f'b{res}', block)

    def forward(self, ws, **block_kwargs):
        ws = ws.to(torch.float32)
        if sg2_chain.ENABLED and not (set(block_kwargs) - {'update_emas', 'noise_mode', 'force_fp32'}):
            return self._forward_node(ws)
        x = img = None
        first = 0
        for res in self.block_resolutions:
            block = getattr(self, f'b{res}')
            n = block.num_conv + block.num_torgb
            cur = ws.unsqueeze(1).expand(-1, n, -1) if ws.ndim == 2 else ws[:, first:first + n]
            x, img = block(x, img, cur, **block_kwargs)
            first += block.num_conv
        return img.permute(0, 3, 1, 2)


    def _forward_node(self, ws):
        blocks, tensors = [], []
        first = 0
        for res in self.block_resolutions:
            block = getattr(self, f'b{res}')
            n = block.num_conv + block.num_torgb
            w_iter = iter([ws] * n if ws.ndim == 2 else ws[:, first:first + n].unbind(dim=1))
            layers = ([block.conv0] if block.in_channels != 0 else []) + [block.conv1]
            for layer in layers:
                styles = layer.affine(next(w_iter))
                tensors += [layer.weight, layer.bias, styles, modconv.demod_coefs(layer.weight, styles)]
            tensors += [block.torgb.weight, block.torgb.bias, block.torgb.affine(next(w_iter)) * float(block.torgb.weight_gain)]
            gains = (float(block.conv0.act_gain) if block.in_channels != 0 else None, float(block.conv1.act_gain))
            params = {'conv1': (block.conv1.weight, block.conv1.bias), 'torgb': (block.torgb.weight, block.torgb.bias)}
            if block.in_channels != 0:
                params['conv0'] = (block.conv0.weight, block.conv0.bias)
            blocks.append(sg2_chain.Block(block.in_channels != 0, gains, params))
            first += block.num_conv
        b4 = getattr(self, f'b{self.block_resolutions[0]}')
        img = sg2_chain.run(blocks, b4.const, b4.resample_filter, tensors)
        return img.permute(0, 3, 1, 2)


class DecoderMappingNetwork(torch.nn.Module):
    def __init__(self, z_dim, w_dim, num_ws, num_layers=8, layer_features=None, activation='lrelu', lr_multiplier=0.01,
                 w_avg_beta=0.998):
        super().__init__()
        self.z_dim = z_dim
        self.w_dim = w_dim
        self.num_ws = num_ws
        self.num_layers = num_layers
        self.w_avg_beta = w_avg_beta
        if layer_features is None:
            layer_features = w_dim
        features_list = [z_dim] + [layer_features] * (num_layers - 1) + [w_dim]
        for idx in range(num_layers):
            layer = FullyConnectedLayer(features_list[idx], features_list[idx + 1], activation=activation, lr_multiplier=lr_multiplier)
            setattr(self, f'fc{idx}', layer)
        if num_ws is not None and w_avg_beta is not None:
            self.register_buffer('w_avg', torch.zeros([w_dim]))

    def forward(self, z, truncation_psi=1, truncation_cutoff=None, update_emas=False, broadcast=True):
        w = z.to(torch.float32)
        for idx in range(self.num_layers):
            w = getattr(self, f'fc{idx}')(w)
        if update_emas and self.w_avg_beta is not None:
            self.w_avg.copy_(torch.lerp(w.detach().mean(dim=0), self.w_avg, self.w_avg_beta))
        per_layer = truncation_psi != 1 and self.num_ws is not None and truncation_cutoff is not None
        if truncation_psi != 1 and not per_layer:
            assert self.w_avg_beta is not None
            w = torch.lerp(self.w_avg, w, truncation_psi)
        if self.num_ws is None or (not broadcast and not per_layer):
            return w
        ws = w.unsqueeze(1).repeat([1, self.num_ws, 1])
        if per_layer:
            assert self.w_avg_beta is not None
            head = torch.lerp(self.w_avg, ws[:, :truncation_cutoff], truncation_psi)
            ws = torch.cat([head, ws[:, truncation_cutoff:]], dim=1)
        return ws


class Decoder(torch.nn.Module):
    def __init__(self, z_dim, w_dim, img_resolution, img_channels, use_noise, mapping_kwargs={}, **synthesis_kwargs):
        super().__init__()
        self.z_dim = z_dim
        self.w_dim = w_dim
        self.img_resolution = img_resolution
        self.img_channels = img_channels
        self.synthesis = SynthesisNetwork(w_dim=w_dim, img_resolution=img_resolution, img_channels=img_channels, use_noise=use_noise,
                                          **synthesis_kwargs)
        self.num_ws = self.synthesis.num_ws
        self.mapping = DecoderMappingNetwork(z_dim=z_dim, w_dim=w_dim, num_ws=self.num_ws, **mapping_kwargs)

    def forward(self, z, truncation_psi=1, truncation_cutoff=None, update_emas=False, **synthesis_kwargs):
        ws = self.mapping(z, truncation_psi=truncation_psi, truncation_cutoff=truncation_cutoff, update_emas=update_emas, broadcast=False)
        return self.synthesis(ws, update_emas=update_emas, **synthesis_kwargs)
```

Before: 500.4.

## Batch StyleGAN2 side computations into grouped affine, demod and gemm launches

Moves the per-layer style affine, demodulation coefficient computation and their backward passes into the synthesis chain node. These run as grouped kernels covering all layers in a single launch: a grouped small GEMM for the affines, grouped demod fwd/bwd, and a fused affine backward into the latent gradient. The aim is to cut many tiny kernel launches and the Python autograd overhead per layer. In exchange it adds complexity around gradient accumulation into flat grad buffers, and it only applies for 2D ws with linear affines and small batch.

```diff
diff --git a/include/ldetr_hip.h b/include/ldetr_hip.h
--- a/include/ldetr_hip.h
+++ b/include/ldetr_hip.h
@@ -69,6 +69,9 @@
 int ldetr_gemm_pair_f32(const ldetr_gemm_desc* g0, const ldetr_gemm_desc* g1, void* stream);
 int ldetr_gemm_pair_is_single_launch(const ldetr_gemm_desc* g0, const ldetr_gemm_desc* g1);
 
+#define LDETR_GEMM_GROUP_MAX 32
+int ldetr_gemm_small_group_f32(const ldetr_gemm_desc* g, const float* post_scale, int n, void* stream);
+
 int ldetr_conv2d_fwd_f32(const float* x, const ldetr_tensor4* xt, const float* w, int Cout, int KH, int KW, int stride,
                          int pad, float* y, int64_t ldy, int OH, int OW, const float* in_scale, int64_t in_scale_ld,
                          const ldetr_epilogue* ep, void* stream);
@@ -182,6 +185,8 @@
                          int C, void* stream);
 int ldetr_torgb_fwd_f32(const float* x, const float* w, const float* styles, const float* bias, float* y,
                         int B, int64_t P, int C, void* stream);
+int ldetr_torgb_fwd_add_f32(const float* x, const float* w, const float* styles, const float* bias, const float* addend, float* y,
+                            int B, int64_t P, int C, void* stream);
 int ldetr_torgb_bwd_f32(const float* x, const float* dy, const float* w, const float* styles, float* dx, float* dws,
                         float* dbias, int B, int64_t P, int C, void* stream);
 int ldetr_sg2_handoff_f32(const float* dxs, const float* x, const float* dy_rgb, float* dv, const float* s_conv, const float* s_rgb,
@@ -228,6 +233,24 @@
 int ldetr_demod_bwd_f32(const float* weight, int64_t so, int64_t si, int64_t sh, int64_t sw, const float* styles, const float* dcoefs,
                         const float* w2, const float* grad_dcoefs, float* dweight, int accumulate_dweight, float* dstyles, int B, int O,
                         int I, int KH, int KW, void* stream);
+
+#define LDETR_DEMOD_GROUP_MAX 24
+typedef struct ldetr_demod_desc {
+    const float* weight; int64_t so, si, sh, sw;
+    const float* styles; float* dcoefs; float* w2;
+    const float* grad_dcoefs; float* dweight; float* dstyles;
+    int O, I, KH, KW;
+} ldetr_demod_desc;
+int ldetr_demod_group_fwd_f32(const ldetr_demod_desc* layers, int n, int B, float eps, void* stream);
+int ldetr_demod_group_bwd_f32(const ldetr_demod_desc* layers, int n, int B, int accumulate_dweight, int add_dstyles, void* stream);
+
+#define LDETR_AFFINE_GROUP_MAX 32
+typedef struct ldetr_affine_desc {
+    const float* ds; const float* A; float* dA; float* db;
+    int C; float scale; float post;
+} ldetr_affine_desc;
+int ldetr_sg2_affine_bwd_f32(const ldetr_affine_desc* layers, int n, const float* latent, float* dlatent, int accumulate_dlatent,
+                             float* scratch, int64_t scratch_floats, int B, int D, void* stream);
 
 int ldetr_layout_losses_f32(const float* bbox, const float* bbox_ref, const uint8_t* valid, int B, int N, float* losses,
                             float* grads, void* stream);
diff --git a/layoutdetr_amd/_lib.py b/layoutdetr_amd/_lib.py
--- a/layoutdetr_amd/_lib.py
+++ b/layoutdetr_amd/_lib.py
@@ -64,6 +64,16 @@
 class WgradDesc(Structure):
     _fields_ = [('A', c_void_p), ('lda', c_int64), ('B', c_void_p), ('ldb', c_int64), ('dW', c_void_p), ('ldw', c_int64), ('db', c_void_p),
                 ('M', c_int), ('rows', c_int), ('cols', c_int)]
+
+
+class DemodDesc(Structure):
+    _fields_ = [('weight', c_void_p), ('so', c_int64), ('si', c_int64), ('sh', c_int64), ('sw', c_int64),
+                ('styles', c_void_p), ('dcoefs', c_void_p), ('w2', c_void_p), ('grad_dcoefs', c_void_p), ('dweight', c_void_p), ('dstyles', c_void_p),
+                ('O', c_int), ('I', c_int), ('KH', c_int), ('KW', c_int)]
+
+
+class AffineDesc(Structure):
+    _fields_ = [('ds', c_void_p), ('A', c_void_p), ('dA', c_void_p), ('db', c_void_p), ('C', c_int), ('scale', c_float), ('post', c_float)]
 
 
 class LayoutRasterArgs(Structure):
@@ -174,6 +184,11 @@
     'ldetr_gemm_pair_is_single_launch': [_P, _P],
     'ldetr_demod_fwd_f32': [_P, _L, _L, _L, _L, _P, _P, _P, _I, _I, _I, _I, _I, _F, _P],
     'ldetr_demod_bwd_f32': [_P, _L, _L, _L, _L, _P, _P, _P, _P, _P, _I, _P, _I, _I, _I, _I, _I, _P],
+    'ldetr_demod_group_fwd_f32': [_P, _I, _I, _F, _P],
+    'ldetr_demod_group_bwd_f32': [_P, _I, _I, _I, _I, _P],
+    'ldetr_sg2_affine_bwd_f32': [_P, _I, _P, _P, _I, _P, _L, _I, _I, _P],
+    'ldetr_gemm_small_group_f32': [_P, _P, _I, _P],
+    'ldetr_torgb_fwd_add_f32': [_P, _P, _P, _P, _P, _P, _I, _L, _I, _P],
     'ldetr_layout_losses_f32': [_P, _P, _P, _I, _I, _P, _P, _P],
     'ldetr_layout_losses_bwd_f32': [_P, _P, _I, _I, _P, _P],
     'ldetr_layout_finish_f32': [_P, _P, _P, _P, _P, _P, _P, _P, _P, _I, _I, _I, _P],
diff --git a/layoutdetr_amd/build.py b/layoutdetr_amd/build.py
--- a/layoutdetr_amd/build.py
+++ b/layoutdetr_amd/build.py
@@ -13,12 +13,12 @@
 ARCH = 'gfx950'
 
 SOURCES = ['ldetr_core.cpp', 'bias_act.hip', 'upfirdn2d.hip', 'gemm_conv.hip', 'attention.hip', 'layernorm.hip',
-           'misc_ops.hip', 'optim.hip', 'lsap.hip', 'xent.hip', 'resample.hip', 'layout_loss.hip', 'demod.hip', 'wgrad_smallc.hip', 'stem_conv.hip', 'box_ops.hip', 'ffn_fused.hip', 'conv_c32.hip', 'mha_small.hip', 'p3_engine.hip', 'bmm_strided.hip', 'layoutnet.hip', 'layoutnet_train.hip', 'layout_finish.hip', 'layout_raster.hip', 'page_filter.hip', 'patch_resize.hip', 'png_decode.hip', 'png_encode.hip', 'png_inflate.hip']
+           'misc_ops.hip', 'optim.hip', 'lsap.hip', 'xent.hip', 'resample.hip', 'layout_loss.hip', 'demod.hip', 'sg2_affine.hip', 'wgrad_smallc.hip', 'stem_conv.hip', 'box_ops.hip', 'ffn_fused.hip', 'conv_c32.hip', 'mha_small.hip', 'p3_engine.hip', 'bmm_strided.hip', 'layoutnet.hip', 'layoutnet_train.hip', 'layout_finish.hip', 'layout_raster.hip', 'page_filter.hip', 'patch_resize.hip', 'png_decode.hip', 'png_encode.hip', 'png_inflate.hip']
 HEADERS = ['ldetr_common.hpp', 'layoutnet_layers.hpp', 'pil_resample.hpp', 'png_pages.hpp', 'png_inflate_kernel.hpp', os.path.join('..', '..', 'include', 'ldetr_hip.h')]
 
 FLAGS = ([] if os.environ.get('LDETR_TILE_TRACE') else ['-DLDETR_TILE_TRACE=0']) + (['-DP3_TRACE'] if os.environ.get('LDETR_P3_TRACE') else []) + ['-O3', '-std=c++17', '-fPIC', f'--offload-arch={ARCH}', '-munsafe-fp-atomics', '-fno-gpu-rdc',
          '-Wno-unused-result', '-Rpass-analysis=kernel-resource-usage']
-NO_SCRATCH = ('wgrad_c32_3x3_kernel', 'gemm_f32_kernel', 'gemm_small_kernel', 'attn_fwd_kernel', 'attn_fwd_wide_kernel', 'attn_bwd_kernel', 'ffn_fwd_kernel', 'ffn_bwd_kernel', 'conv3x3_c32_kernel', 'mha_small_fwd_kernel', 'mha_cross_fwd_kernel', 'mha_small_bwd_kernel', 'mha_cross_bwd_kernel', 'wgrad_multi_kernel', 'ln_fwd_kernel', 'ln_bwd_kernel', 'p3_nt_kernel', 'p3_tn_kernel', 'p3_c3_kernel', 'p3_bwd_pair', 'layoutnet_features_kernel', 'layoutnet_forward_kernel', 'feature_stats_f64_kernel', 'layout_finish_kernel', 'layout_raster_kernel', 'page_blur_kernel', 'page_edge_kernel', 'patch_resize_kernel', 'sg2_handoff_kernel', 'png_gather_kernel', 'png_unfilter_kernel', 'png_enc_filter_kernel', 'png_enc_deflate_kernel', 'png_enc_assemble_kernel', 'png_inflate_kernel')
+NO_SCRATCH = ('wgrad_c32_3x3_kernel', 'gemm_f32_kernel', 'gemm_small_kernel', 'gemm_small_group_kernel', 'demod_group', 'sg2_affine_bwd', 'attn_fwd_kernel', 'attn_fwd_wide_kernel', 'attn_bwd_kernel', 'ffn_fwd_kernel', 'ffn_bwd_kernel', 'conv3x3_c32_kernel', 'mha_small_fwd_kernel', 'mha_cross_fwd_kernel', 'mha_small_bwd_kernel', 'mha_cross_bwd_kernel', 'wgrad_multi_kernel', 'ln_fwd_kernel', 'ln_bwd_kernel', 'p3_nt_kernel', 'p3_tn_kernel', 'p3_c3_kernel', 'p3_bwd_pair', 'layoutnet_features_kernel', 'layoutnet_forward_kernel', 'feature_stats_f64_kernel', 'layout_finish_kernel', 'layout_raster_kernel', 'page_blur_kernel', 'page_edge_kernel', 'patch_resize_kernel', 'sg2_handoff_kernel', 'png_gather_kernel', 'png_unfilter_kernel', 'png_enc_filter_kernel', 'png_enc_deflate_kernel', 'png_enc_assemble_kernel', 'png_inflate_kernel')
 
 
 def _hipcc():
diff --git a/layoutdetr_amd/csrc/demod.hip b/layoutdetr_amd/csrc/demod.hip
--- a/layoutdetr_amd/csrc/demod.hip
+++ b/layoutdetr_amd/csrc/demod.hip
@@ -10,16 +10,15 @@
     float* w2;
     const float* g;
     float* dw; int dw_accumulate;
-    float* ds;
+    float* ds; int ds_add;
     int B, O, I, KH, KW;
     float eps;
 };
 
 constexpr int DEMOD_MAXB = 64;
 
-__global__ __launch_bounds__(256) void demod_fwd_kernel(DemodParams p) {
+__device__ __forceinline__ void demod_fwd_body(const DemodParams& p, const int o) {
     extern __shared__ float w2row[];
-    const int o = blockIdx.x;
     for (int i = threadIdx.x; i < p.I; i += 256) {
         const float* wp = p.w + (long)o * p.so + (long)i * p.si;
         float acc = 0.f;
@@ -55,9 +54,10 @@
     }
 }
 
-__global__ __launch_bounds__(256) void demod_bwd_w_kernel(DemodParams p) {
+__global__ __launch_bounds__(256) void demod_fwd_kernel(DemodParams p) { demod_fwd_body(p, blockIdx.x); }
+
+__device__ __forceinline__ void demod_bwd_w_body(const DemodParams& p, const int o) {
     __shared__ float t[DEMOD_MAXB];
-    const int o = blockIdx.x;
     if (threadIdx.x < p.B) {
         const float dv = p.d[(long)threadIdx.x * p.O + o];
         t[threadIdx.x] = -0.5f * p.g[(long)threadIdx.x * p.O + o] * dv * dv * dv;
@@ -77,9 +77,11 @@
     }
 }
 
-__global__ __launch_bounds__(256) void demod_bwd_s_kernel(DemodParams p) {
+__global__ __launch_bounds__(256) void demod_bwd_w_kernel(DemodParams p) { demod_bwd_w_body(p, blockIdx.x); }
+
+__device__ __forceinline__ void demod_bwd_s_body(const DemodParams& p, const int bx, const int b) {
     extern __shared__ float tb[];
-    const int b = blockIdx.y, i = blockIdx.x * 64 + (threadIdx.x & 63), lane = threadIdx.x >> 6;
+    const int i = bx * 64 + (threadIdx.x & 63), lane = threadIdx.x >> 6;
     for (int o = threadIdx.x; o < p.O; o += 256) {
         const float dv = p.d[(long)b * p.O + o];
         tb[o] = -0.5f * p.g[(long)b * p.O + o] * dv * dv * dv;
@@ -95,7 +97,36 @@
     __syncthreads();
     if (lane == 0 && i < p.I) {
         acc += part[threadIdx.x + 64] + part[threadIdx.x + 128] + part[threadIdx.x + 192];
-        p.ds[(long)b * p.I + i] = 2.f * p.s[(long)b * p.I + i] * acc;
+        const float v = 2.f * p.s[(long)b * p.I + i] * acc;
+        if (p.ds_add) p.ds[(long)b * p.I + i] = __fadd_rn(p.ds[(long)b * p.I + i], v); else p.ds[(long)b * p.I + i] = v;
+    }
+}
+
+__global__ __launch_bounds__(256) void demod_bwd_s_kernel(DemodParams p) { demod_bwd_s_body(p, blockIdx.x, blockIdx.y); }
+
+struct DemodGroup { DemodParams p[LDETR_DEMOD_GROUP_MAX]; int start_w[LDETR_DEMOD_GROUP_MAX + 1]; int start_s[LDETR_DEMOD_GROUP_MAX + 1]; int n; };
+
+__device__ __forceinline__ int group_find(const int* start, const int n, const int b) {
+    int pi = 0;
+    for (int i = 1; i < n; i++) pi += (b >= start[i]) ? 1 : 0;
+    return pi;
+}
+
+__global__ __launch_bounds__(256) void demod_group_fwd_kernel(DemodGroup g) {
+    const int pi = group_find(g.start_w, g.n, (int)blockIdx.x);
+    demod_fwd_body(g.p[pi], (int)blockIdx.x - g.start_w[pi]);
+}
+
+__global__ __launch_bounds__(256) void demod_group_bwd_kernel(DemodGroup g) {
+    const int blk = (int)blockIdx.x, nw = g.start_w[g.n];
+    if (blk < nw) {
+        const int pi = group_find(g.start_w, g.n, blk);
+        if (g.p[pi].dw) demod_bwd_w_body(g.p[pi], blk - g.start_w[pi]);
+    } else {
+        const int pi = group_find(g.start_s, g.n, blk - nw);
+        const DemodParams& p = g.p[pi];
+        const int r = blk - nw - g.start_s[pi], gx = (p.I + 63) >> 6;
+        demod_bwd_s_body(p, r % gx, r / gx);
     }
 }
 
@@ -140,3 +171,43 @@
     }
     return rc;
 }
+
+static int demod_group_fill(DemodGroup& g, const ldetr_demod_desc* d, int n, int B, float eps, bool bwd, int accumulate_dweight, int add_dstyles,
+                            size_t* lds, const char* what) {
+    LDETR_CHECK(d && n >= 1 && n <= LDETR_DEMOD_GROUP_MAX, "%s: 1..%d layers", what, LDETR_DEMOD_GROUP_MAX);
+    memset(&g, 0, sizeof(g));
+    g.n = n;
+    long tw = 0, ts = 0;
+    size_t need = 0;
+    for (int l = 0; l < n; l++) {
+        DemodParams& p = g.p[l];
+        const ldetr_demod_desc& q = d[l];
+        p.w = q.weight; p.so = q.so; p.si = q.si; p.sh = q.sh; p.sw = q.sw; p.s = q.styles; p.d = q.dcoefs; p.w2 = q.w2;
+        p.g = q.grad_dcoefs; p.dw = q.dweight; p.dw_accumulate = accumulate_dweight; p.ds = q.dstyles; p.ds_add = add_dstyles;
+        p.B = B; p.O = q.O; p.I = q.I; p.KH = q.KH; p.KW = q.KW; p.eps = eps;
+        int rc = demod_check(p, what); if (rc) return rc;
+        if (bwd) LDETR_CHECK(p.g && p.ds, "%s: null pointer (layer %d)", what, l);
+        g.start_w[l] = (int)tw; g.start_s[l] = (int)ts;
+        tw += p.O; ts += (long)cdiv(p.I, 64) * B;
+        const size_t mine = bwd ? (size_t)(p.O + 256) * sizeof(float) : (size_t)p.I * sizeof(float);
+        if (mine > need) need = mine;
+    }
+    LDETR_CHECK(tw + ts < 0x7fffffffL, "%s: grid too large", what);
+    g.start_w[n] = (int)tw; g.start_s[n] = (int)ts;
+    *lds = need;
+    return LDETR_OK;
+}
+
+extern "C" int ldetr_demod_group_fwd_f32(const ldetr_demod_desc* layers, int n, int B, float eps, void* stream) {
+    DemodGroup g; size_t lds = 0;
+    int rc = demod_group_fill(g, layers, n, B, eps, false, 0, 0, &lds, "demod_group_fwd"); if (rc) return rc;
+    hipLaunchKernelGGL(demod_group_fwd_kernel, dim3((unsigned)g.start_w[n]), 256, lds, (hipStream_t)stream, g);
+    return check_launch("demod_group_fwd");
+}
+
+extern "C" int ldetr_demod_group_bwd_f32(const ldetr_demod_desc* layers, int n, int B, int accumulate_dweight, int add_dstyles, void* stream) {
+    DemodGroup g; size_t lds = 0;
+    int rc = demod_group_fill(g, layers, n, B, 0.f, true, accumulate_dweight, add_dstyles, &lds, "demod_group_bwd"); if (rc) return rc;
+    hipLaunchKernelGGL(demod_group_bwd_kernel, dim3((unsigned)(g.start_w[n] + g.start_s[n])), 256, lds, (hipStream_t)stream, g);
+    return check_launch("demod_group_bwd");
+}
diff --git a/layoutdetr_amd/csrc/gemm_conv.hip b/layoutdetr_amd/csrc/gemm_conv.hip
--- a/layoutdetr_amd/csrc/gemm_conv.hip
+++ b/layoutdetr_amd/csrc/gemm_conv.hip
@@ -1068,8 +1068,8 @@
     }
 }
 
-template <int TA, int TB, int NW, bool FAST = false>
-__device__ __forceinline__ void gemm_small_body(const GemmParams& p, const int bx, const int by, const int bz, const int sk, const int gx) {
+template <int TA, int TB, int NW, bool FAST = false, bool POST = false>
+__device__ __forceinline__ void gemm_small_body(const GemmParams& p, const int bx, const int by, const int bz, const int sk, const int gx, const float post = 1.f) {
     using f32x16 = __attribute__((__vector_size__(16 * sizeof(float)))) float;
     __shared__ float red[NW][32][33];
     const int tid = threadIdx.x, lane = tid & 63, wave = tid >> 6;
@@ -1212,6 +1212,10 @@
             if (n0 + c4 + e < p.N) v[e] = apply_epilogue(ep, v[e], m, n0 + c4 + e, samp, p.ldc, inv_keep, ep.col_scale ? ep.col_scale[n0 + c4 + e] : 1.f, ep.col_bias ? ep.col_bias[n0 + c4 + e] : 0.f,
                                                              ep.residual ? ep.residual[(long)m * ep.ldr + n0 + c4 + e] : 0.f,
                                                              ep.mask_mode ? ep.mask_src[(long)m * ep.ldm + n0 + c4 + e] : 0.f);
+        if constexpr (POST) {
+#pragma unroll
+            for (int e = 0; e < 4; e++) v[e] = __fmul_rn(v[e], post);
+        }
         if (n0 + c4 + 3 < p.N && (p.ldc & 3) == 0 && ((((uintptr_t)p.C) & 15) == 0)) {
             float4 o = make_float4(v[0], v[1], v[2], v[3]);
             if (ep.accumulate) { float4 c = *reinterpret_cast<float4*>(dst); o.x += c.x; o.y += c.y; o.z += c.z; o.w += c.w; }
@@ -1234,6 +1238,29 @@
     const int b = blockIdx.x;
     if (b < nt0 * sk0) { const int t = b % nt0; gemm_small_body<TA0, TB0, NW, FAST>(p0, t % gx0, t / gx0, b / nt0, sk0, gx0); }
     else { const int c = b - nt0 * sk0, t = c % nt1; gemm_small_body<TA1, TB1, NW, FAST>(p1, t % gx1, t / gx1, c / nt1, sk1, gx1); }
+}
+
+struct SmallGroupProblem {
+    const float* A; const float* B; float* C; const float* col_bias;
+    int lda, ldb, ldc, avec, bvec, M, N, K;
+    float alpha, post;
+};
+struct SmallGroup { SmallGroupProblem q[LDETR_GEMM_GROUP_MAX]; int start[LDETR_GEMM_GROUP_MAX + 1]; int n; GemmEpilogue ep0; };
+
+template <int NW, bool FAST>
+__global__ __launch_bounds__(NW * 64) void gemm_small_group_kernel(SmallGroup g) {
+    const int blk = (int)blockIdx.x;
+    int pi = 0;
+    for (int i = 1; i < g.n; i++) pi += (blk >= g.start[i]) ? 1 : 0;
+    const SmallGroupProblem& q = g.q[pi];
+    GemmParams p = {};
+    p.A.KW = p.A.KH = p.A.stride = p.A.C = p.A.Cr = 1; p.B.KW = p.B.KH = p.B.stride = p.B.C = p.B.Cr = 1;
+    p.A.p = q.A; p.A.ld = q.lda; p.A.vec = q.avec; p.B.p = q.B; p.B.ld = q.ldb; p.B.vec = q.bvec;
+    p.M = q.M; p.N = q.N; p.K = q.K; p.C = q.C; p.ldc = q.ldc;
+    p.splitk = 1; p.pstep = 1; p.nsamp = 1;
+    p.ep = g.ep0; p.ep.alpha = q.alpha; p.ep.col_bias = q.col_bias;
+    const int t = blk - g.start[pi], gx = (q.N + 31) >> 5;
+    gemm_small_body<0, 0, NW, FAST, true>(p, t % gx, t / gx, 0, 1, gx, q.post);
 }
 
 static inline bool al16(const void* p) { return (((uintptr_t)p) & 15) == 0; }
@@ -1755,6 +1782,63 @@
     int rc = gemm_dense(*g0, stream);
     if (rc) return rc;
     return gemm_dense(*g1, stream);
+}
+
+static int launch_small_group(const ldetr_gemm_desc* d, const float* post_scale, int n, hipStream_t st) {
+    SmallGroup g; memset(&g, 0, sizeof(g));
+    g.n = n;
+    fill_epilogue(g.ep0, nullptr);
+    long total = 0;
+    bool fast = false, w8 = false;
+    for (int i = 0; i < n; i++) {
+        const ldetr_gemm_desc& q = d[i];
+        LDETR_CHECK(q.A && q.B && q.C, "gemm_small_group: null pointer (problem %d)", i);
+        LDETR_CHECK(q.M > 0 && q.N > 0 && q.K > 0, "gemm_small_group: empty problem %d", i);
+        const ldetr_epilogue* e = q.ep;
+        const bool plain_ep = !e || (!e->col_scale && !e->samp_scale && !e->residual && e->act == 0 && e->mask_mode == 0 && e->out_scale == 1.f &&
+                                     e->p_drop == 0.f && !e->accumulate && !e->a_rowsum);
+        if (q.ta || q.tb || q.splitk != 0 || !plain_ep || !small_class(q.M, q.N, q.K)) {
+            set_error("gemm_small_group: problem %d is not a plain NN small-tile problem", i);
+            return LDETR_ERR_UNSUPPORTED;
+        }
+        const long blocks = (long)cdiv(q.N, 32) * cdiv(q.M, 32);
+        if (blocks <= 128 && q.K >= 1024) {
+            set_error("gemm_small_group: problem %d splits its reduction", i);
+            return LDETR_ERR_UNSUPPORTED;
+        }
+        ldetr_gemm_desc one = q; one.pix_per_sample = 0;
+        const GemmParams p = fill_dense(one);
+        const bool f = small_fast_ok(p, 0, 0), w = small_wants8(blocks, 1, p.K);
+        if (i == 0) { fast = f; w8 = w; }
+        else if (f != fast || w != w8) {
+            set_error("gemm_small_group: problem %d resolves to another instantiation than problem 0", i);
+            return LDETR_ERR_UNSUPPORTED;
+        }
+        SmallGroupProblem& o = g.q[i];
+        LDETR_CHECK(q.lda < 0x7fffffffL && q.ldb < 0x7fffffffL && q.ldc < 0x7fffffffL, "gemm_small_group: leading dimension above 2^31 (problem %d)", i);
+        o.A = q.A; o.B = q.B; o.C = q.C; o.col_bias = p.ep.col_bias;
+        o.lda = (int)q.lda; o.ldb = (int)q.ldb; o.ldc = (int)q.ldc; o.avec = p.A.vec; o.bvec = p.B.vec; o.M = q.M; o.N = q.N; o.K = q.K;
+        o.alpha = p.ep.alpha; o.post = post_scale ? post_scale[i] : 1.f;
+        g.start[i] = (int)total;
+        total += blocks;
+    }
+    g.start[n] = (int)total;
+    const dim3 grid((unsigned)total);
+    if (fast) {
+        if (w8) hipLaunchKernelGGL((gemm_small_group_kernel<8, true>), grid, 512, 0, st, g);
+        else hipLaunchKernelGGL((gemm_small_group_kernel<4, true>), grid, 256, 0, st, g);
+    } else {
+        if (w8) hipLaunchKernelGGL((gemm_small_group_kernel<8, false>), grid, 512, 0, st, g);
+        else hipLaunchKernelGGL((gemm_small_group_kernel<4, false>), grid, 256, 0, st, g);
+    }
+    t_launches_f32++;
+    note_engine_launch(7, 32, 32, 0, w8 ? 8 : 4, fast ? 1 : 0, 0, 1, total, 0);
+    return check_launch("gemm_small_group");
+}
+
+extern "C" int ldetr_gemm_small_group_f32(const ldetr_gemm_desc* g, const float* post_scale, int n, void* stream) {
+    LDETR_CHECK(g && n >= 1 && n <= LDETR_GEMM_GROUP_MAX, "gemm_small_group: 1..%d problems", LDETR_GEMM_GROUP_MAX);
+    return launch_small_group(g, post_scale, n, (hipStream_t)stream);
 }
 
 extern "C" int ldetr_conv2d_fwd_f32(const float* x, const ldetr_tensor4* xt, const float* w, int Cout, int KH, int KW,
diff --git a/layoutdetr_amd/csrc/misc_ops.hip b/layoutdetr_amd/csrc/misc_ops.hip
--- a/layoutdetr_amd/csrc/misc_ops.hip
+++ b/layoutdetr_amd/csrc/misc_ops.hip
@@ -557,7 +557,7 @@
 }
 
 namespace ldetr {
-struct RgbFwdParams { const float* x; const float* w; const float* s; const float* bias; float* y; long P; int B, C; };
+struct RgbFwdParams { const float* x; const float* w; const float* s; const float* bias; float* y; long P; int B, C; const float* add; };
 
 template <int LPP>
 __global__ __launch_bounds__(256) void torgb_fwd_kernel(RgbFwdParams p) {
@@ -597,20 +597,25 @@
         for (int o = LPP / 2; o > 0; o >>= 1) { d0 += __shfl_xor(d0, o, 64); d1 += __shfl_xor(d1, o, 64); d2 += __shfl_xor(d2, o, 64); }
         if (lane_in == 0) {
             float* yr = p.y + ((long)b * p.P + r) * 3;
-            yr[0] = d0 + b0; yr[1] = d1 + b1; yr[2] = d2 + b2;
-        }
-    }
-}
-}
-
-extern "C" int ldetr_torgb_fwd_f32(const float* x, const float* w, const float* styles, const float* bias, float* y,
-                                   int B, int64_t P, int C, void* stream) {
+            float y0 = d0 + b0, y1 = d1 + b1, y2 = d2 + b2;
+            if (p.add) {
+                const float* ar = p.add + ((long)b * p.P + r) * 3;
+                y0 = __fadd_rn(ar[0], y0); y1 = __fadd_rn(ar[1], y1); y2 = __fadd_rn(ar[2], y2);
+            }
+            yr[0] = y0; yr[1] = y1; yr[2] = y2;
+        }
+    }
+}
+}
+
+static int torgb_fwd(const float* x, const float* w, const float* styles, const float* bias, const float* addend, float* y,
+                     int B, int64_t P, int C, void* stream) {
     LDETR_CHECK(x && w && styles && y, "torgb_fwd: null pointer");
     const int C4 = C / 4;
     LDETR_CHECK(C % 4 == 0 && C4 >= 1 && C <= 512 && (C4 & (C4 - 1)) == 0, "torgb_fwd: C must be 4 x a power of two, at most 512 (got %d)", C);
     LDETR_CHECK((((uintptr_t)x | (uintptr_t)w | (uintptr_t)styles) & 15) == 0, "torgb_fwd: buffers must be 16-byte aligned");
     if (B == 0 || P == 0) return LDETR_OK;
-    RgbFwdParams p; p.x = x; p.w = w; p.s = styles; p.bias = bias; p.y = y; p.P = P; p.B = B; p.C = C;
+    RgbFwdParams p; p.x = x; p.w = w; p.s = styles; p.bias = bias; p.y = y; p.P = P; p.B = B; p.C = C; p.add = addend;
     const int lpp = C4 < 64 ? C4 : 64;
     const long ppb = 256 / lpp;
     long gx = (P + ppb - 1) / ppb; if (gx > 4096) gx = 4096;
@@ -626,6 +631,17 @@
         default: hipLaunchKernelGGL(torgb_fwd_kernel<64>, grid, 256, 0, st, p); break;
     }
     return check_launch("torgb_fwd");
+}
+
+extern "C" int ldetr_torgb_fwd_f32(const float* x, const float* w, const float* styles, const float* bias, float* y,
+                                   int B, int64_t P, int C, void* stream) {
+    return torgb_fwd(x, w, styles, bias, nullptr, y, B, P, C, stream);
+}
+
+extern "C" int ldetr_torgb_fwd_add_f32(const float* x, const float* w, const float* styles, const float* bias, const float* addend, float* y,
+                                       int B, int64_t P, int C, void* stream) {
+    LDETR_CHECK(addend, "torgb_fwd_add: null addend");
+    return torgb_fwd(x, w, styles, bias, addend, y, B, P, C, stream);
 }
 
 extern "C" int ldetr_torgb_bwd_f32(const float* x, const float* dy, const float* w, const float* styles,
diff --git a/layoutdetr_amd/csrc/sg2_affine.hip b/layoutdetr_amd/csrc/sg2_affine.hip
--- /dev/null
+++ b/layoutdetr_amd/csrc/sg2_affine.hip
@@ -0,0 +1,118 @@
+#include "ldetr_common.hpp"
+#include "../../include/ldetr_hip.h"
+
+namespace ldetr {
+
+constexpr int AFF_MAXB = 64;
+
+struct AffineGroup { ldetr_affine_desc d[LDETR_AFFINE_GROUP_MAX]; int start[LDETR_AFFINE_GROUP_MAX + 1]; int n; };
+
+__global__ __launch_bounds__(256) void sg2_affine_bwd_kernel(AffineGroup g, const float* __restrict__ latent, float* __restrict__ part, int B, int D) {
+    extern __shared__ float lds[];
+    float* At = lds;
+    float* dsL = lds + 64 * 64;
+    float* wL = dsL + B * 64;
+    const int gx = (D + 63) >> 6;
+    const int ci = (int)blockIdx.x / gx, cgp = (int)blockIdx.x - ci * gx;
+    int pi = 0;
+    for (int i = 1; i < g.n; i++) pi += (ci >= g.start[i]) ? 1 : 0;
+    const ldetr_affine_desc& d = g.d[pi];
+    const int C = d.C, c0 = (ci - g.start[pi]) * 64, col0 = cgp * 64;
+    const int tid = threadIdx.x, cc = tid & 63, grp = tid >> 6;
+    const int col = col0 + cc;
+    for (int idx = tid; idx < 64 * 64; idx += 256) {
+        const int c = idx >> 6;
+        At[idx] = (c0 + c < C && col < D) ? d.A[(long)(c0 + c) * D + col] : 0.f;
+    }
+    for (int idx = tid; idx < B * 64; idx += 256) {
+        const int b = idx >> 6;
+        dsL[idx] = (c0 + cc < C) ? d.ds[(long)b * C + c0 + cc] : 0.f;
+        wL[idx] = (col < D) ? latent[(long)b * D + col] : 0.f;
+    }
+    __syncthreads();
+    {
+        float acc[16];
+#pragma unroll
+        for (int u = 0; u < 16; u++) acc[u] = 0.f;
+        for (int c = 0; c < 64; c++) {
+            const float av = At[c * 64 + cc];
+#pragma unroll
+            for (int u = 0; u < 16; u++)
+                if (grp + 4 * u < B) acc[u] += dsL[(grp + 4 * u) * 64 + c] * av;
+        }
+        if (col < D) {
+#pragma unroll
+            for (int u = 0; u < 16; u++)
+                if (grp + 4 * u < B) part[((long)ci * B + grp + 4 * u) * D + col] = d.scale * acc[u];
+        }
+    }
+    if (d.dA && col < D) {
+        for (int j = 0; j < 16; j++) {
+            const int c = grp * 16 + j;
+            if (c0 + c >= C) break;
+            float v = 0.f;
+            for (int b = 0; b < B; b++) v += dsL[b * 64 + c] * wL[b * 64 + cc];
+            float* dst = d.dA + (long)(c0 + c) * D + col;
+            *dst += d.scale * v;
+        }
+    }
+    if (d.db && cgp == 0 && tid < 64 && c0 + tid < C) {
+        float v = 0.f;
+        for (int b = 0; b < B; b++) v += dsL[b * 64 + tid];
+        d.db[c0 + tid] += d.post * v;
+    }
+}
+
+__global__ __launch_bounds__(256) void sg2_affine_bwd_reduce_kernel(const float* __restrict__ part, float* __restrict__ dw, int accumulate, int chunks, long BD) {
+    const long i = (long)blockIdx.x * 256 + threadIdx.x;
+    if (i >= BD) return;
+    float v = 0.f;
+    int c = 0;
+    for (; c + 8 <= chunks; c += 8) {
+        float t[8];
+#pragma unroll
+        for (int u = 0; u < 8; u++) t[u] = part[(long)(c + u) * BD + i];
+#pragma unroll
+        for (int u = 0; u < 8; u++) v += t[u];
+    }
+    for (; c < chunks; c++) v += part[(long)c * BD + i];
+    dw[i] = accumulate ? dw[i] + v : v;
+}
+
+static int affine_fill(AffineGroup& g, const ldetr_affine_desc* d, int n, const char* what) {
+    LDETR_CHECK(d && n >= 1 && n <= LDETR_AFFINE_GROUP_MAX, "%s: 1..%d layers", what, LDETR_AFFINE_GROUP_MAX);
+    memset(&g, 0, sizeof(g));
+    g.n = n;
+    long chunks = 0;
+    for (int l = 0; l < n; l++) {
+        LDETR_CHECK(d[l].ds && d[l].A && d[l].C > 0, "%s: bad layer %d", what, l);
+        g.d[l] = d[l];
+        g.start[l] = (int)chunks;
+        chunks += cdiv(d[l].C, 64);
+    }
+    LDETR_CHECK(chunks < (1 << 20), "%s: too many channels", what);
+    g.start[n] = (int)chunks;
+    return LDETR_OK;
+}
+
+}
+
+using namespace ldetr;
+
+extern "C" int ldetr_sg2_affine_bwd_f32(const ldetr_affine_desc* layers, int n, const float* latent, float* dlatent, int accumulate_dlatent,
+                                        float* scratch, int64_t scratch_floats, int B, int D, void* stream) {
+    AffineGroup g;
+    int rc = affine_fill(g, layers, n, "sg2_affine_bwd"); if (rc) return rc;
+    LDETR_CHECK(latent && dlatent && scratch, "sg2_affine_bwd: null pointer");
+    LDETR_CHECK(B > 0 && B <= AFF_MAXB && D > 0, "sg2_affine_bwd: bad shape (batch <= %d)", AFF_MAXB);
+    const int chunks = g.start[n], gx = cdiv(D, 64);
+    LDETR_CHECK((long)chunks * gx < 0x7fffffffL, "sg2_affine_bwd: grid too large");
+    LDETR_CHECK(scratch_floats >= (int64_t)chunks * B * D, "sg2_affine_bwd: scratch too small (%lld floats needed)", (long long)chunks * B * D);
+    hipStream_t st = (hipStream_t)stream;
+    const size_t lds = (size_t)(64 + 2 * B) * 64 * sizeof(float);
+    hipLaunchKernelGGL(sg2_affine_bwd_kernel, dim3((unsigned)(chunks * gx)), 256, lds, st, g, latent, scratch, B, D);
+    rc = check_launch("sg2_affine_bwd"); if (rc) return rc;
+    const long BD = (long)B * D;
+    hipLaunchKernelGGL(sg2_affine_bwd_reduce_kernel, dim3((unsigned)((BD + 255) / 256)), 256, 0, st, scratch, dlatent, accumulate_dlatent, chunks, BD);
+    return check_launch("sg2_affine_bwd_reduce");
+}
diff --git a/layoutdetr_amd/hip/core.py b/layoutdetr_amd/hip/core.py
--- a/layoutdetr_amd/hip/core.py
+++ b/layoutdetr_amd/hip/core.py
@@ -76,7 +76,7 @@
 
 
 _P3_KINDS = {1: 'p3_nt_kernel', 2: 'p3_c3_kernel', 3: 'p3_tn_kernel', 4: 'p3_bwd_pair_nt_kernel', 5: 'p3_bwd_pair_c3_kernel'}
-_ENGINE_KINDS = {1: 'gemm_f32_kernel', 2: 'gemm_small_kernel', 3: 'gemm_small_pair_kernel', 4: 'conv3x3_c32_kernel', 5: 'wgrad_c32_3x3_kernel', 6: 'stem_conv7x7_kernel'}
+_ENGINE_KINDS = {1: 'gemm_f32_kernel', 2: 'gemm_small_kernel', 3: 'gemm_small_pair_kernel', 4: 'conv3x3_c32_kernel', 5: 'wgrad_c32_3x3_kernel', 6: 'stem_conv7x7_kernel', 7: 'gemm_small_group_kernel'}
 
 
 def launched_kernel(tag):
@@ -95,7 +95,7 @@
     name = _ENGINE_KINDS.get(kind, 'engine_?')
     if kind == 1:
         return f'{name}<{bm},{bn},{bk},{nw}w' + (',FAST' if fast else '') + (',SPLIT' if split else '') + '>' + (f' splitK={sk}' if sk > 1 else '')
-    if kind in (2, 3):
+    if kind in (2, 3, 7):
         return f'{name}<{nw}w' + (',FAST' if fast else '') + '>'
     if kind == 4:
         return 'conv3x3_c32_split_kernel' if split else name
@@ -272,6 +272,35 @@
                 nbytes=4.0 * sum(d.M * d.K + d.N * d.K + d.M * d.N for d in descs))
 
 
+GEMM_GROUP_MAX = 32
+
+
+def gemm_group(problems, post=None):
+    n = len(problems)
+    if n < 1 or n > GEMM_GROUP_MAX:
+        return False
+    descs = (_lib.GemmDesc * n)()
+    flops = nbytes = 0.0
+    for d, g in zip(descs, problems):
+        require_gpu(g['A'], g['B'], g['out'])
+        d.A = g['A'].data_ptr(); d.lda = g['A'].stride(0); d.ta = 0
+        d.B = g['B'].data_ptr(); d.ldb = g['B'].stride(0); d.tb = 0
+        d.C = g['out'].data_ptr(); d.ldc = g['out'].stride(0)
+        d.M, d.N, d.K, d.splitk = int(g['M']), int(g['N']), int(g['K']), 0
+        d.ep = ctypes.addressof(g['ep']) if g.get('ep') is not None else None
+        d.pix_per_sample = 0
+        flops += 2.0 * d.M * d.N * d.K
+        nbytes += 4.0 * (d.M * d.K + d.N * d.K + d.M * d.N)
+    scales = (ctypes.c_float * n)(*[float(v) for v in post]) if post is not None else None
+    rc = engine_call('gemm', flops, lambda: lib().ldetr_gemm_small_group_f32(descs, scales, n, stream()), nbytes=nbytes)
+    if rc == 3:
+        if PROF.enabled and PROF.records:
+            PROF.records.pop()
+        return False
+    check(rc, 'gemm_small_group')
+    return True
+
+
 def colsum(a2d, B=1):
     require_gpu(a2d)
     R, C = a2d.shape
diff --git a/layoutdetr_amd/hip/sg2_chain.py b/layoutdetr_amd/hip/sg2_chain.py
--- a/layoutdetr_amd/hip/sg2_chain.py
+++ b/layoutdetr_amd/hip/sg2_chain.py
@@ -1,20 +1,26 @@
+
 import torch
 
 from . import core, modconv
+from .. import _lib
 from .conv import weight_ohwi
 from ..torch_utils.ops import upfirdn2d as _up
 
 ENABLED = core.knob('SG2_CHAIN', 1) != 0
+SIDE = core.knob('SG2_SIDE', 1) != 0
 ACT_ALPHA = 0.2
 NODE_RUNS = [0]
+SIDE_MAX_B = 64
+DEMOD_GROUP_MAX, AFFINE_GROUP_MAX = 24, 32
 
 
 class Block(object):
 
-    def __init__(self, has_conv0, gains, params):
+    def __init__(self, has_conv0, gains, params, affines=None):
         self.has_conv0 = has_conv0
         self.gains = gains
         self.params = params
+        self.affines = affines
 
 
 def _handoff(dxs, x, dy_rgb, s_conv, rgb, bias, demod, dbias, gain):
@@ -38,61 +44,190 @@
     return torch.zeros(C, device=device, dtype=torch.float32), False
 
 
+def _views(flat, shapes):
+    out, o = [], 0
+    for shp in shapes:
+        n = shp[0] * shp[1]
+        out.append(flat[o:o + n].view(shp))
+        o += n
+    return out
+
+
+def side_styles(ws, affines):
+    B, D = ws.shape
+    dev = ws.device
+    shapes = [(B, a[0].shape[0]) for a in affines]
+    styles = _views(torch.empty(sum(b * c for b, c in shapes), device=dev, dtype=torch.float32), shapes)
+    problems = [dict(A=ws, B=a[0], M=B, N=a[0].shape[0], K=D, out=s, ep=core.epilogue(alpha=a[2], col_bias=a[1])) for a, s in zip(affines, styles)]
+    posts = [a[3] for a in affines]
+    for i in range(0, len(problems), core.GEMM_GROUP_MAX):
+        chunk, post = problems[i:i + core.GEMM_GROUP_MAX], posts[i:i + core.GEMM_GROUP_MAX]
+        if not core.gemm_group(chunk, post):
+            for g, ps in zip(chunk, post):
+                core.gemm(g['A'], g['B'], 0, 0, g['M'], g['N'], g['K'], out=g['out'], ep=g['ep'])
+                if ps != 1.0:
+                    g['out'].mul_(ps)
+    return styles
+
+
+def _demod_descs(layers, grads=None):
+    descs = (_lib.DemodDesc * len(layers))()
+    for i, (d, (w, s, dc, w2)) in enumerate(zip(descs, layers)):
+        d.weight = w.data_ptr()
+        d.so, d.si, d.sh, d.sw = w.stride()
+        d.styles, d.dcoefs, d.w2 = s.data_ptr(), dc.data_ptr(), w2.data_ptr()
+        d.O, d.I, d.KH, d.KW = w.shape
+        if grads is not None:
+            g, dw, ds = grads[i]
+            d.grad_dcoefs, d.dweight, d.dstyles = g.data_ptr(), (dw.data_ptr() if dw is not None else None), ds.data_ptr()
+    return descs
+
+
+def side_demod(weights, styles):
+    B = styles[0].shape[0]
+    dev = styles[0].device
+    dshapes = [(B, w.shape[0]) for w in weights]
+    wshapes = [(w.shape[0], w.shape[1]) for w in weights]
+    dcoefs = _views(torch.empty(sum(a * b for a, b in dshapes), device=dev, dtype=torch.float32), dshapes)
+    w2 = _views(torch.empty(sum(a * b for a, b in wshapes), device=dev, dtype=torch.float32), wshapes)
+    layers = list(zip(weights, styles, dcoefs, w2))
+    for i in range(0, len(layers), DEMOD_GROUP_MAX):
+        chunk = layers[i:i + DEMOD_GROUP_MAX]
+        core.check(core.lib().ldetr_demod_group_fwd_f32(_demod_descs(chunk), len(chunk), B, 1e-8, core.stream()), 'demod_group_fwd')
+    return dcoefs, w2
+
+
+def side_demod_bwd(layers, grads, B):
+    for i in range(0, len(layers), DEMOD_GROUP_MAX):
+        chunk = layers[i:i + DEMOD_GROUP_MAX]
+        core.check(core.lib().ldetr_demod_group_bwd_f32(_demod_descs(chunk, grads[i:i + DEMOD_GROUP_MAX]), len(chunk), B, 1, 1, core.stream()),
+                   'demod_group_bwd')
+
+
+def side_affine_bwd(ws, layers):
+    ws = core.f32c(ws)
+    B, D = ws.shape
+    dws = torch.empty((B, D), device=ws.device, dtype=torch.float32)
+    for i in range(0, len(layers), AFFINE_GROUP_MAX):
+        chunk = layers[i:i + AFFINE_GROUP_MAX]
+        descs = (_lib.AffineDesc * len(chunk))()
+        floats = 0
+        for d, (ds, A, dA, db, gain, post) in zip(descs, chunk):
+            d.ds, d.A = ds.data_ptr(), A.data_ptr()
+            d.dA, d.db = (dA.data_ptr() if dA is not None else None), (db.data_ptr() if db is not None else None)
+            d.C, d.scale, d.post = A.shape[0], gain * post, post
+            floats += (A.shape[0] + 63) // 64 * B * D
+        scratch = torch.empty(floats, device=ws.device, dtype=torch.float32)
+        core.check(core.lib().ldetr_sg2_affine_bwd_f32(descs, len(chunk), core.ptr(ws), core.ptr(dws), 1 if i else 0, core.ptr(scratch), floats, B, D,
+                                                       core.stream()), 'sg2_affine_bwd')
+    return dws
+
+
+def _torgb_fwd(x, w, s, b, img):
+    B, H, W, C = x.shape
+    c4 = C // 4
+    if img is None or not (C % 4 == 0 and C <= 512 and (c4 & (c4 - 1)) == 0 and s.stride(0) == C):
+        y = modconv.torgb_fwd(x, w, s, b)
+        return img + y if img is not None else y
+    img = img.contiguous()
+    y = torch.empty((B, H, W, 3), device=x.device, dtype=torch.float32)
+    core.check(core.lib().ldetr_torgb_fwd_add_f32(core.ptr(x), core.ptr(w), core.ptr(s), core.ptr(b), core.ptr(img), core.ptr(y), B, H * W, C, core.stream()),
+               'torgb_fwd_add')
+    return y
+
+
 class _SynthesisFn(torch.autograd.Function):
 
     @staticmethod
     def forward(ctx, blocks, const, f, *tensors):
         core.require_gpu(const, f, *tensors)
         keep = any(ctx.needs_input_grad)
+        side = blocks[0].affines is not None
+        ws = None
+        if side:
+            ws, tensors = tensors[0], tensors[1:]
+            if not (ws.dtype == torch.float32 and ws.stride(1) == 1 and ws.stride(0) >= ws.shape[1] and ws.stride(0) % 4 == 0 and ws.data_ptr() % 16 == 0):
+                ws = core.f32c(ws)
+            kinds = [k for blk in blocks for k in (('conv0',) if blk.has_conv0 else ()) + ('conv1', 'torgb')]
+            affs = [blk.affines[k] for blk in blocks for k in (('conv0',) if blk.has_conv0 else ()) + ('conv1', 'torgb')]
+            affs = [(core.f32c(tensors[4 * i + 2].detach()), core.f32c(tensors[4 * i + 3].detach()), a[2], a[3]) for i, a in enumerate(affs)]
+            styles = side_styles(ws, affs)
+            convs = [i for i, k in enumerate(kinds) if k != 'torgb']
+            wdet = [tensors[4 * i].detach() if tensors[4 * i].dtype == torch.float32 else tensors[4 * i].detach().float() for i in convs]
+            dcoefs, w2s = side_demod(wdet, [styles[i] for i in convs])
+            side_of = {i: (wdet[j], dcoefs[j], w2s[j]) for j, i in enumerate(convs)}
         it = iter(tensors)
         saved, layout = [const, f], []
         x = img = None
-        B = tensors[2].shape[0]
+        B = ws.shape[0] if side else tensors[2].shape[0]
+        li = 0
+
+        def layer(is_conv):
+            nonlocal li
+            if not side:
+                return [next(it) for _ in range(4 if is_conv else 3)] + [None]
+            w, b = next(it), next(it)
+            next(it); next(it)
+            rec = (li, side_of[li][0], side_of[li][2], affs[li][0]) if is_conv else (li, affs[li][0])
+            out = [w, b, styles[li]] + ([side_of[li][1]] if is_conv else []) + [rec]
+            li += 1
+            return out
         for blk in blocks:
             entry = {}
             if blk.has_conv0:
-                w, b, s, d = [next(it) for _ in range(4)]
+                w, b, s, d, extra = layer(True)
                 w = core.f32c(weight_ohwi(w)); b = core.f32c(b); s = core.f32c(s); d = core.f32c(d)
                 _, x0 = modconv.up_fwd(x, w, s, d, b, f, ACT_ALPHA, blk.gains[0])
                 entry['conv0'] = (w, b, s, d, x0)
+                if side:
+                    entry['side_conv0'] = extra[1:]
                 x = x0
             else:
                 x = core.f32c(const).permute(1, 2, 0).unsqueeze(0).repeat([B, 1, 1, 1])
                 entry['xin'] = (x,)
-            w, b, s, d = [next(it) for _ in range(4)]
+            w, b, s, d, extra = layer(True)
             w = core.f32c(weight_ohwi(w)); b = core.f32c(b); s = core.f32c(s); d = core.f32c(d)
             x = modconv.conv_fwd(x, w, s, d, b, w.shape[1] // 2, ACT_ALPHA, blk.gains[1])
             entry['conv1'] = (w, b, s, d, x)
+            if side:
+                entry['side_conv1'] = extra[1:]
             if img is not None:
                 img = _up._kernel_call(img.permute(0, 3, 1, 2), f, 2, 2, 1, 1, 2, 1, 2, 1, False, 4.0).permute(0, 2, 3, 1)
-            w, b, s = [next(it) for _ in range(3)]
+            w, b, s, extra = layer(False)
             ctx_wshape = w.shape
             w = core.f32c(w.reshape(w.shape[0], -1)); b = core.f32c(b); s = core.f32c(s)
             if w.shape[0] != 3:
                 raise NotImplementedError('the synthesis node is specialised for 3 colour channels')
-            y = modconv.torgb_fwd(x, w, s, b)
-            img = img + y if img is not None else y
+            if side:
+                img = _torgb_fwd(x, w, s, b, img)
+                entry['side_torgb'] = extra[1:]
+            else:
+                y = modconv.torgb_fwd(x, w, s, b)
+                img = img + y if img is not None else y
             entry['torgb'] = (w, s)
             entry['rgb_wshape'] = ctx_wshape
             if keep:
                 rec = {}
-                for k in ('conv0', 'xin', 'conv1', 'torgb'):
+                for k in ('conv0', 'xin', 'conv1', 'torgb', 'side_conv0', 'side_conv1', 'side_torgb'):
                     if k in entry:
                         rec[k] = (len(saved), len(entry[k]))
                         saved += list(entry[k])
                 rec['rgb_wshape'] = ctx_wshape
                 layout.append(rec)
         if keep:
+            if side:
+                saved.append(ws)
             ctx.save_for_backward(*saved)
-            ctx.blocks, ctx.layout = blocks, layout
+            ctx.blocks, ctx.layout, ctx.side = blocks, layout, side
         return img
 
     @staticmethod
     def backward(ctx, dimg):
         saved = ctx.saved_tensors
         const, f = saved[0], saved[1]
-        blocks, layout = ctx.blocks, ctx.layout
-        need = ctx.needs_input_grad[3:]
+        blocks, layout, side = ctx.blocks, ctx.layout, ctx.side
+        per = 4 if side else 3
+        need = ctx.needs_input_grad[(4 if side else 3):]
         get = lambda rec, k: saved[rec[k][0]:rec[k][0] + rec[k][1]]
         dimg = core.f32c(dimg)
         dev = dimg.device
@@ -100,7 +235,8 @@
         first, n = [], 0
         for blk in blocks:
             first.append(n)
-            n += 11 if blk.has_conv0 else 7
+            n += (8 if blk.has_conv0 else 4) + per
+        ds_of, dd_of = {}, {}
         dxs_next = s_next = dconst = None
         for i in reversed(range(len(blocks))):
             blk, rec = blocks[i], layout[i]
@@ -116,12 +252,12 @@
             core.check(core.lib().ldetr_torgb_bwd_finish_f32(core.ptr(dws), core.ptr(sr), core.ptr(wr), B, C, core.ptr(dw_rgb), core.ptr(ds_rgb), core.stream()),
                        'torgb_bwd_finish')
             if i + 1 < len(blocks):
-                grads[first[i + 1] + 2] = ds_next
+                ds_of[first[i + 1]] = ds_next
             grads[o + 4] = None if wr_flat else dw_rgb.reshape(rec['rgb_wshape'])
             grads[o + 5] = None if br_flat else dbias_rgb
-            grads[o + 6] = ds_rgb
+            ds_of[o + 4] = ds_rgb
             grads[o + 1] = None if b1_flat else db1
-            grads[o + 3] = dd1
+            dd_of[o] = dd1
             xin = get(rec, 'conv0')[4] if blk.has_conv0 else get(rec, 'xin')[0]
             pad = w1.shape[1] // 2
             dxs1 = modconv.conv_bwd_data(dv1, w1, d1, B, xin.shape[1], xin.shape[2], pad)
@@ -129,7 +265,7 @@
                 grads[o] = modconv.conv_bwd_weight(xin, dv1, w1, s1, d1, w1p, pad)
             if not blk.has_conv0:
                 dx, ds1 = modconv._mul_reduce(dxs1, xin, s1, B, xin.shape[1] * xin.shape[2], xin.shape[3])
-                grads[o + 2] = ds1
+                ds_of[o] = ds1
                 if ctx.needs_input_grad[1]:
                     dconst = dx.sum(0).permute(2, 0, 1)
                 break
@@ -137,9 +273,9 @@
             w0p, b0p = blk.params['conv0']
             db0, b0_flat = _bias_target(b0p, C, dev)
             dv0, ds1, _, dd0 = _handoff(dxs1, x0, None, s1, None, b0, d0, db0, blk.gains[0])
-            grads[o + 2] = ds1
+            ds_of[o] = ds1
             grads[first[i] + 1] = None if b0_flat else db0
-            grads[first[i] + 3] = dd0
+            dd_of[first[i]] = dd0
             dud = modconv.up_fir_adjoint(dv0, f)
             xprev = get(layout[i - 1], 'conv1')[4]
             dxs_next = modconv.up_bwd_data(dud, w0, d0, B, xprev.shape[1], xprev.shape[2])
@@ -147,7 +283,59 @@
             if need[first[i]]:
                 grads[first[i]] = modconv.up_bwd_weight(xprev, dud, w0, s0, d0, w0p)
             dimg = _up._kernel_call(dimg.permute(0, 3, 1, 2), f, 1, 1, 2, 2, 1, 1, 1, 1, True, 4.0).permute(0, 2, 3, 1)
-        return (None, dconst, None) + tuple(grads)
+        if not side:
+            for p, t in ds_of.items():
+                grads[p + 2] = t
+            for p, t in dd_of.items():
+                grads[p + 3] = t
+            return (None, dconst, None) + tuple(grads)
+        dws = _SynthesisFn._side_backward(ctx, saved, blocks, layout, first, need, grads, ds_of, dd_of)
+        return (None, dconst, None, dws) + tuple(grads)
+
+    @staticmethod
+    def _side_backward(ctx, saved, blocks, layout, first, need, grads, ds_of, dd_of):
+        get = lambda rec, k: saved[rec[k][0]:rec[k][0] + rec[k][1]]
+        ws = saved[-1]
+        B = ws.shape[0]
+        demod_layers, demod_grads, aff_layers, fix = [], [], [], []
+        for i, (blk, rec) in enumerate(zip(blocks, layout)):
+            names = (('conv0', first[i]),) if blk.has_conv0 else ()
+            names += (('conv1', first[i] + (4 if blk.has_conv0 else 0)), ('torgb', first[i] + (8 if blk.has_conv0 else 4)))
+            for name, p in names:
+                ds = ds_of[p]
+                extra = get(rec, 'side_' + name)
+                if name != 'torgb':
+                    wdet, w2, aw = extra
+                    _, _, s, d, _ = get(rec, name)
+                    dwt = None
+                    if need[p]:
+                        acc = core.flat_grad(blk.params[name][0])
+                        if acc is not None and acc.stride() == wdet.stride():
+                            dwt = acc
+                        else:
+                            dwt = torch.zeros_like(wdet)
+                            fix.append((p, dwt))
+                    demod_layers.append((wdet, s, d, w2))
+                    demod_grads.append((dd_of[p], dwt, ds))
+                else:
+                    aw, = extra
+                aparam, bparam, gain, post = blk.affines[name]
+                dA = db = None
+                if need[p + 2]:
+                    dA = core.flat_grad(aparam)
+                    if dA is None or not dA.is_contiguous():
+                        dA = torch.zeros_like(aw)
+                        grads[p + 2] = dA
+                if need[p + 3]:
+                    db = core.flat_grad(bparam)
+                    if db is None or not db.is_contiguous():
+                        db = torch.zeros(aw.shape[0], device=aw.device, dtype=torch.float32)
+                        grads[p + 3] = db
+                aff_layers.append((ds, aw, dA, db, gain, post))
+        side_demod_bwd(demod_layers, demod_grads, B)
+        for p, dwt in fix:
+            grads[p] = dwt if grads[p] is None else grads[p] + dwt
+        return side_affine_bwd(ws, aff_layers)
 
 
 def run(blocks, const, f, tensors):
diff --git a/layoutdetr_amd/training/networks_stylegan2.py b/layoutdetr_amd/training/networks_stylegan2.py
--- a/layoutdetr_amd/training/networks_stylegan2.py
+++ b/layoutdetr_amd/training/networks_stylegan2.py
@@ -3,7 +3,7 @@
 import numpy as np
 import torch
 
-from ..hip import core, modconv, sg2_chain
+from ..hip import composite, core, modconv, sg2_chain
 from ..hip.linear import linear
 from ..torch_utils.ops import bias_act, upfirdn2d
 
@@ -190,20 +190,38 @@
     def _forward_node(self, ws):
         blocks, tensors = [], []
         first = 0
+        side = sg2_chain.SIDE and ws.ndim == 2 and ws.is_cuda and ws.shape[0] <= sg2_chain.SIDE_MAX_B and not composite.active()
+        for res in self.block_resolutions:
+            block = getattr(self, f'b{res}')
+            for layer in ([block.conv0] if block.in_channels != 0 else []) + [block.conv1, block.torgb]:
+                a = layer.affine
+                side = side and a.activation == 'linear' and a.bias is not None and a.bias_gain == 1 and a.weight.shape[0] % 4 == 0
+        if side:
+            tensors.append(ws)
         for res in self.block_resolutions:
             block = getattr(self, f'b{res}')
             n = block.num_conv + block.num_torgb
             w_iter = iter([ws] * n if ws.ndim == 2 else ws[:, first:first + n].unbind(dim=1))
             layers = ([block.conv0] if block.in_channels != 0 else []) + [block.conv1]
-            for layer in layers:
+            names = (['conv0'] if block.in_channels != 0 else []) + ['conv1']
+            affines = {} if side else None
+            for name, layer in zip(names, layers):
+                if side:
+                    tensors += [layer.weight, layer.bias, layer.affine.weight, layer.affine.bias]
+                    affines[name] = (layer.affine.weight, layer.affine.bias, float(layer.affine.weight_gain), 1.0)
+                    continue
                 styles = layer.affine(next(w_iter))
                 tensors += [layer.weight, layer.bias, styles, modconv.demod_coefs(layer.weight, styles)]
-            tensors += [block.torgb.weight, block.torgb.bias, block.torgb.affine(next(w_iter)) * float(block.torgb.weight_gain)]
+            if side:
+                tensors += [block.torgb.weight, block.torgb.bias, block.torgb.affine.weight, block.torgb.affine.bias]
+                affines['torgb'] = (block.torgb.affine.weight, block.torgb.affine.bias, float(block.torgb.affine.weight_gain), float(block.torgb.weight_gain))
+            else:
+                tensors += [block.torgb.weight, block.torgb.bias, block.torgb.affine(next(w_iter)) * float(block.torgb.weight_gain)]
             gains = (float(block.conv0.act_gain) if block.in_channels != 0 else None, float(block.conv1.act_gain))
             params = {'conv1': (block.conv1.weight, block.conv1.bias), 'torgb': (block.torgb.weight, block.torgb.bias)}
             if block.in_channels != 0:
                 params['conv0'] = (block.conv0.weight, block.conv0.bias)
-            blocks.append(sg2_chain.Block(block.in_channels != 0, gains, params))
+            blocks.append(sg2_chain.Block(block.in_channels != 0, gains, params, affines))
             first += block.num_conv
         b4 = getattr(self, f'b{self.block_resolutions[0]}')
         img = sg2_chain.run(blocks, b4.const, b4.resample_filter, tensors)
```

New measurement: 513.6 (median of 6 runs). +2.6%, better.
